# yesint/molar

Measured on AMD Instinct MI355X. Metric: frames/sec + Matom-pairs/sec, 1M-atom PBC neighbor search + RMSD fit, higher is better.
Workload: dtype f32; 1 GPU; 1M-atom synthetic triclinic box A, per frame: PBC neighbour search rc=1.2 nm (ordered pair list in HBM) + Kabsch RMSD fit/COM/gyration of a 100k-atom selection; natoms=1000000, selection_atoms=100000, frames_per_gpu=1451, parallelism=frames sharded over 1 rank(s), no data-path collective, streams_per_gpu=2, measure_overlapped_with_search=True

## Files before the change

include/molar_hip.h:

```cpp
#ifndef MOLAR_HIP_H
#define MOLAR_HIP_H

#include <stddef.h>
#include <stdint.h>

#ifdef __cplusplus
extern "C" {
#endif

enum {
    MOLAR_HIP_OK = 0,
    MOLAR_HIP_ERR_SIZES = 1,
    MOLAR_HIP_ERR_ZERO_MASS = 2,
    MOLAR_HIP_ERR_SVD = 3,
    MOLAR_HIP_ERR_NO_PBC = 4,
    MOLAR_HIP_ERR_ZERO_LENGTH_VECTOR = 5,
    MOLAR_HIP_ERR_INVERSE_FAILED = 6,
    MOLAR_HIP_ERR_LIPID_TAIL_TOO_SHORT = 7,
    MOLAR_HIP_ERR_LIPID_NORMALS_COUNT = 8,
    MOLAR_HIP_ERR_LIPID_BOND_ORDER_COUNT = 9,
    MOLAR_HIP_ERR_ANGLE_TOO_SMALL = 10,
    MOLAR_HIP_ERR_INVALID_ARGUMENT = 50,
    MOLAR_HIP_ERR_TOO_LARGE = 51,
    MOLAR_HIP_ERR_NO_SEARCH = 52,
// ... 5 lines not shown
#define MOLAR_HIP_PBC_NONE 0u


typedef struct molar_hip_ctx molar_hip_ctx;

molar_hip_ctx *molar_hip_create(int device);
void molar_hip_destroy(molar_hip_ctx *ctx);
const char *molar_hip_last_error(void);
const char *molar_hip_version(void);
int molar_hip_device_count(void);
int molar_hip_set_stream(molar_hip_ctx *ctx, void *hip_stream);
int molar_hip_synchronize(molar_hip_ctx *ctx);

#define MOLAR_HIP_PROFILE_CLASSES 8
int molar_hip_profile_enable(molar_hip_ctx *ctx, int on);
int molar_hip_profile_read(molar_hip_ctx *ctx, float ms[MOLAR_HIP_PROFILE_CLASSES],
                           uint64_t launches[MOLAR_HIP_PROFILE_CLASSES]);

int molar_hip_copy_bandwidth(molar_hip_ctx *ctx, size_t bytes, int reps, float *gb_per_s);
int molar_hip_write_bandwidth(molar_hip_ctx *ctx, size_t bytes, int reps, float *gb_per_s);


typedef struct {
    float m[9];
    float inv[9];
    int32_t nshift;
    float shifts[26 * 3];
} molar_hip_box;

int molar_hip_box_from_matrix(const float m9[9], molar_hip_box *out);
int molar_hip_box_from_vectors_angles(float a, float b, float c, float alpha, float beta, float gamma,
                                      molar_hip_box *out);
void molar_hip_box_shortest_vector(const molar_hip_box *box, const float v[3], uint8_t pbc, float out[3]);
void molar_hip_box_lab_extents(const molar_hip_box *box, float out[3]);
void molar_hip_box_extents(const molar_hip_box *box, float out[3]);
void molar_hip_box_to_box_coords(const molar_hip_box *box, const float v[3], float out[3]);
void molar_hip_box_to_lab_coords(const molar_hip_box *box, const float v[3], float out[3]);
int molar_hip_box_is_inside(const molar_hip_box *box, const float p[3]);
void molar_hip_box_wrap_point(const molar_hip_box *box, const float p[3], float out[3]);


enum {
    MOLAR_HIP_SEARCH_SINGLE = 0,
    MOLAR_HIP_SEARCH_DOUBLE = 1,
    MOLAR_HIP_SEARCH_WITHIN = 2,
    MOLAR_HIP_SEARCH_DOUBLE_VDW = 3
};

typedef struct {
    int32_t kind;
    float cutoff;
    const float *xyz1;
    size_t natoms1;
    const uint64_t *idx1;
    size_t n1;
    const float *xyz2;
    size_t natoms2;
    const uint64_t *idx2;
    size_t n2;
    const float *vdw1;
    const float *vdw2;
    int32_t ids_local;
    const float *box9;
    uint8_t pbc;
    const float *lower3;
    const float *upper3;
} molar_hip_search_desc;

int molar_hip_search_count(molar_hip_ctx *ctx, const molar_hip_search_desc *desc, uint64_t *out_count);
int molar_hip_search_fill(molar_hip_ctx *ctx, uint32_t *pairs, float *dist);
int molar_hip_search_fill_usize(molar_hip_ctx *ctx, uint64_t *i, uint64_t *j, float *dist);
int molar_hip_search_fill_ids(molar_hip_ctx *ctx, uint64_t *ids);
int molar_hip_within_count(molar_hip_ctx *ctx, const molar_hip_search_desc *desc, uint64_t *out_count);
int molar_hip_within_fill(molar_hip_ctx *ctx, uint64_t *ids);
int molar_hip_within_hold(molar_hip_ctx *ctx, int on);
int molar_hip_search_connectivity(molar_hip_ctx *ctx, const molar_hip_search_desc *desc, uint64_t *out_rows, uint64_t *out_entries);
int molar_hip_search_connectivity_fill(molar_hip_ctx *ctx, uint64_t *offsets, uint64_t *neigh);
int molar_hip_unwrap_connectivity(molar_hip_ctx *ctx, float *xyz, size_t natoms, const uint64_t *idx, size_t n,
                                  const float *box9, float cutoff, uint8_t pbc_dims, uint64_t *group_offsets,
                                  uint64_t *group_ids, size_t *ngroups);
int molar_hip_search_grid_dims(molar_hip_ctx *ctx, uint64_t dims[3]);
int molar_hip_search_cell_kernels(molar_hip_ctx *ctx, int32_t *lanes, uint64_t occupied_cells[2]);
int molar_hip_search_slot_counts(molar_hip_ctx *ctx, uint64_t *slots, uint64_t *consecutive_slots);
int molar_hip_search_fill_device(molar_hip_ctx *ctx, const uint32_t **d_pairs, const float **d_dist);
int molar_hip_search_resident(molar_hip_ctx *ctx, const molar_hip_search_desc *desc, uint64_t *out_count,
                              const uint32_t **d_pairs, const float **d_dist);
int molar_hip_search_resident_planes(molar_hip_ctx *ctx, int want_dist);
int molar_hip_search_resident_begin(molar_hip_ctx *ctx, const molar_hip_search_desc *desc, int32_t *ticket);
int molar_hip_search_resident_end(molar_hip_ctx *ctx, int32_t ticket, uint64_t *out_count, const uint32_t **d_pairs,
                                  const float **d_dist);
int molar_hip_search_histogram(molar_hip_ctx *ctx, const molar_hip_search_desc *desc, float hmin,
                               float hmax, size_t nbins, uint64_t *bins, uint64_t *out_count);
int molar_hip_search_histogram_frames(molar_hip_ctx *ctx, const molar_hip_search_desc *desc, size_t nframes, size_t xyz1_stride,
                                      size_t xyz2_stride, const float *boxes9, float hmin, float hmax, size_t nbins,
                                      uint64_t *bins);
int molar_hip_histogram_edges(float hmin, float hmax, size_t nbins, float *edges);

typedef struct {
    const uint32_t *group1;
    size_t ngroups1;
    const uint32_t *group2;
    size_t ngroups2;
} molar_hip_contact_groups;

int molar_hip_search_contacts(molar_hip_ctx *ctx, const molar_hip_search_desc *desc, const molar_hip_contact_groups *groups ,
                              uint64_t *deg1, uint64_t *deg2, uint64_t *map, uint64_t *out_count);
int molar_hip_search_contacts_frames(molar_hip_ctx *ctx, const molar_hip_search_desc *desc, const molar_hip_contact_groups *groups,
                                     size_t nframes, size_t xyz1_stride, size_t xyz2_stride, const float *boxes9,
                                     uint64_t *deg1, uint64_t *deg2, uint64_t *map, uint32_t *occupancy);

int molar_hip_search_clusters(molar_hip_ctx *ctx, const molar_hip_search_desc *desc, const molar_hip_contact_groups *groups ,
                              uint32_t *comp_of, uint32_t *sizes, uint64_t *offsets, uint32_t *members, uint32_t *out_ncomponents);
int molar_hip_search_clusters_frames(molar_hip_ctx *ctx, const molar_hip_search_desc *desc, const molar_hip_contact_groups *groups,
                                     size_t nframes, size_t xyz1_stride, const float *boxes9, uint32_t *ncomponents, uint32_t *largest,
                                     uint64_t *size_hist, uint32_t *comp_of_frames);
int molar_hip_search_clusters_counters(molar_hip_ctx *ctx, int32_t enable, uint64_t *out4);

enum {
    MOLAR_HIP_HBOND_DHA_MIN = 0,
    MOLAR_HIP_HBOND_HDA_MAX = 1
};
int molar_hip_hbonds_count(molar_hip_ctx *ctx, const molar_hip_search_desc *desc, const uint64_t *h_offsets, const uint64_t *h_idx,
                           size_t nh, int32_t angle_kind, double angle_deg, double max_ha, uint64_t *out_count);
int molar_hip_hbonds_fill(molar_hip_ctx *ctx, uint32_t *triples, double *dist_da, double *dist_ha, double *angle_deg);
int molar_hip_hbonds_counts(molar_hip_ctx *ctx, const molar_hip_search_desc *desc, const uint64_t *h_offsets, const uint64_t *h_idx,
                            size_t nh, int32_t angle_kind, double angle_deg, double max_ha, const molar_hip_contact_groups *groups,
                            uint64_t *don_count, uint64_t *acc_count, uint64_t *map, uint64_t *out_count);
int molar_hip_hbonds_frames(molar_hip_ctx *ctx, const molar_hip_search_desc *desc, const uint64_t *h_offsets, const uint64_t *h_idx,
                            size_t nh, int32_t angle_kind, double angle_deg, double max_ha, size_t nframes, size_t xyz_stride,
                            const float *boxes9, const molar_hip_contact_groups *groups, uint64_t *per_frame, uint64_t *don_count,
                            uint64_t *acc_count, uint64_t *map, uint64_t *out_total, uint64_t *out_unique);
int molar_hip_hbonds_frames_fill(molar_hip_ctx *ctx, uint64_t *frame_offsets, uint32_t *triples, double *dist_da, double *dist_ha,
                                 double *angle_deg, uint32_t *bond_of_entry, uint32_t *table, uint32_t *occupancy);

int molar_hip_lifetimes_plan(size_t nframes, size_t nrows, size_t ngroups, int want_cont, size_t *workspace_bytes,
                             uint32_t *words_per_row);
int molar_hip_lifetimes(molar_hip_ctx *ctx, const uint64_t *frame_offsets, const uint32_t *row_of_entry, size_t nframes,
                        size_t nrows, const uint32_t *group_of_row, size_t ngroups, size_t max_lag, size_t origin_stride,
                        size_t gap, uint64_t *inter, uint64_t *cont, uint64_t *run_hist, uint32_t *events, uint32_t *longest,
                        uint32_t *present);
int molar_hip_hbonds_frames_shape(molar_hip_ctx *ctx, size_t *nframes, size_t *nrows, size_t *nentries, uint64_t *serial);
int molar_hip_hbonds_frames_lifetimes(molar_hip_ctx *ctx, const uint32_t *group_of_row, size_t ngroups, size_t max_lag,
                                      size_t origin_stride, size_t gap, uint64_t *inter, uint64_t *cont, uint64_t *run_hist,
                                      uint32_t *events, uint32_t *longest, uint32_t *present);

typedef struct {
    int32_t kind;
    double cutoff;
    const double *xyz1;
    size_t natoms1;
    const uint64_t *idx1;
    size_t n1;
    const double *xyz2;
    size_t natoms2;
    const uint64_t *idx2;
    size_t n2;
    const double *vdw1;
    const double *vdw2;
    int32_t ids_local;
    const double *box9;
    uint8_t pbc;
    const double *lower3;
    const double *upper3;
} molar_hip_search_desc_f64;
int molar_hip_search_count_f64(molar_hip_ctx *ctx, const molar_hip_search_desc_f64 *desc, uint64_t *out_count);
int molar_hip_search_fill_f64(molar_hip_ctx *ctx, uint64_t *i, uint64_t *j, double *dist);
// ... 336 lines not shown
```

molar_amd/_lib.py:

```python
from __future__ import annotations

import ctypes as C
import os

HERE = os.path.dirname(os.path.abspath(__file__))
DEFAULT_LIB = os.path.join(HERE, "libmolar_hip.so")

_lib = None


class MolarHipError(RuntimeError):

    def __init__(self, code: int, msg: str):
        super().__init__(f"[molar_hip status {code}] {msg}")
        self.code = code


class Box(C.Structure):
    _fields_ = [("m", C.c_float * 9), ("inv", C.c_float * 9), ("nshift", C.c_int32), ("shifts", C.c_float * 78)]


class SearchDesc(C.Structure):
    _fields_ = [
        ("kind", C.c_int32), ("cutoff", C.c_float),
        ("xyz1", C.c_void_p), ("natoms1", C.c_size_t), ("idx1", C.c_void_p), ("n1", C.c_size_t),
        ("xyz2", C.c_void_p), ("natoms2", C.c_size_t), ("idx2", C.c_void_p), ("n2", C.c_size_t),
        ("vdw1", C.c_void_p), ("vdw2", C.c_void_p),
        ("ids_local", C.c_int32),
        ("box9", C.c_void_p), ("pbc", C.c_uint8),
        ("lower3", C.c_void_p), ("upper3", C.c_void_p),
    ]


class ContactGroups(C.Structure):
    _fields_ = [("group1", C.c_void_p), ("ngroups1", C.c_size_t), ("group2", C.c_void_p), ("ngroups2", C.c_size_t)]


class SearchDescF64(C.Structure):
    _fields_ = [
        ("kind", C.c_int32), ("cutoff", C.c_double),
        ("xyz1", C.c_void_p), ("natoms1", C.c_size_t), ("idx1", C.c_void_p), ("n1", C.c_size_t),
        ("xyz2", C.c_void_p), ("natoms2", C.c_size_t), ("idx2", C.c_void_p), ("n2", C.c_size_t),
        ("vdw1", C.c_void_p), ("vdw2", C.c_void_p),
        ("ids_local", C.c_int32),
        ("box9", C.c_void_p), ("pbc", C.c_uint8),
        ("lower3", C.c_void_p), ("upper3", C.c_void_p),
    ]


class MembraneDesc(C.Structure):
    _fields_ = [
        ("natoms", C.c_size_t), ("nlipids", C.c_size_t),
        ("lipid_idx", C.c_void_p), ("lipid_offsets", C.c_void_p), ("marker_idx", C.c_void_p), ("marker_offsets", C.c_void_p),
        ("masses", C.c_void_p), ("ntails", C.c_size_t), ("tail_idx", C.c_void_p), ("tail_offsets", C.c_void_p),
        ("tail_lipid", C.c_void_p), ("tail_bonds", C.c_void_p),
        ("cutoff", C.c_float), ("order_type", C.c_int32), ("max_smooth_iter", C.c_int32), ("unwrap", C.c_int32),
        ("use_global_normal", C.c_int32), ("global_normal", C.c_float * 3),
    ]


MEMBRANE_ARRAYS = ("head", "mid", "tail", "patch_offsets", "patch_ids", "initial_normals", "valid", "smoothed_head", "normals",
                   "quad_coefs", "mean_curv", "gauss_curv", "princ_curvs", "princ_dirs", "area", "nvert", "neib_ids",
                   "voro_vertexes", "fitted_patch_points", "order")


class MembraneView(C.Structure):
    _fields_ = ([("nlipids", C.c_size_t), ("patch_entries", C.c_size_t), ("npairs", C.c_size_t)]
                + [(k, C.c_void_p) for k in MEMBRANE_ARRAYS] + [("norder", C.c_size_t)])


class MembraneOut(C.Structure):
    _fields_ = [(k, C.c_void_p) for k in MEMBRANE_ARRAYS]


_P, _SZ, _F, _I, _U8 = C.c_void_p, C.c_size_t, C.c_float, C.c_int, C.c_uint8
SYMBOLS = {
    "molar_hip_create": (C.c_void_p, [_I]),
    "molar_hip_destroy": (None, [_P]),
    "molar_hip_last_error": (C.c_char_p, []),
    "molar_hip_version": (C.c_char_p, []),
    "molar_hip_device_count": (_I, []),
    "molar_hip_set_stream": (_I, [_P, _P]),
    "molar_hip_synchronize": (_I, [_P]),
    "molar_hip_profile_enable": (_I, [_P, _I]),
    "molar_hip_profile_read": (_I, [_P, _P, _P]),
    "molar_hip_box_from_matrix": (_I, [_P, _P]),
    "molar_hip_box_from_vectors_angles": (_I, [_F, _F, _F, _F, _F, _F, _P]),
    "molar_hip_box_shortest_vector": (None, [_P, _P, _U8, _P]),
    "molar_hip_copy_bandwidth": (_I, [_P, _SZ, _I, _P]),
    "molar_hip_write_bandwidth": (_I, [_P, _SZ, _I, _P]),
    "molar_hip_box_lab_extents": (None, [_P, _P]),
    "molar_hip_box_extents": (None, [_P, _P]),
    "molar_hip_box_to_box_coords": (None, [_P, _P, _P]),
    "molar_hip_box_to_lab_coords": (None, [_P, _P, _P]),
    "molar_hip_box_is_inside": (_I, [_P, _P]),
    "molar_hip_box_wrap_point": (None, [_P, _P, _P]),
    "molar_hip_search_count": (_I, [_P, _P, _P]),
    "molar_hip_search_fill": (_I, [_P, _P, _P]),
    "molar_hip_search_fill_usize": (_I, [_P, _P, _P, _P]),
    "molar_hip_search_fill_ids": (_I, [_P, _P]),
    "molar_hip_within_count": (_I, [_P, _P, _P]),
    "molar_hip_within_fill": (_I, [_P, _P]),
    "molar_hip_within_hold": (_I, [_P, _I]),
    "molar_hip_search_grid_dims": (_I, [_P, _P]),
    "molar_hip_search_cell_kernels": (_I, [_P, _P, _P]),
    "molar_hip_search_slot_counts": (_I, [_P, _P, _P]),
    "molar_hip_search_count_f64": (_I, [_P, _P, _P]),
    "molar_hip_search_fill_f64": (_I, [_P, _P, _P, _P]),
    "molar_hip_search_fill_ids_f64": (_I, [_P, _P]),
    "molar_hip_search_grid_dims_f64": (_I, [_P, _P]),
    "molar_hip_search_histogram_f64": (_I, [_P, _P, C.c_double, C.c_double, _SZ, _P, _P]),
    "molar_hip_search_histogram_frames_f64": (_I, [_P, _P, _SZ, _SZ, _SZ, _P, C.c_double, C.c_double, _SZ, _P]),
    "molar_hip_histogram_edges_f64": (_I, [C.c_double, C.c_double, _SZ, _P]),
    "molar_hip_within_count_f64": (_I, [_P, _P, _P]),
    "molar_hip_within_fill_f64": (_I, [_P, _P]),
    "molar_hip_search_connectivity_f64": (_I, [_P, _P, _P, _P]),
    "molar_hip_unwrap_connectivity_f64": (_I, [_P, _P, _SZ, _P, _SZ, _P, C.c_double, _U8, _P, _P, _P]),
    "molar_hip_search_resident": (_I, [_P, _P, _P, _P, _P]),
    "molar_hip_search_fill_device": (_I, [_P, _P, _P]),
    "molar_hip_search_resident_planes": (_I, [_P, _I]),
    "molar_hip_search_resident_begin": (_I, [_P, _P, _P]),
    "molar_hip_search_resident_end": (_I, [_P, C.c_int32, _P, _P, _P]),
    "molar_hip_search_histogram": (_I, [_P, _P, _F, _F, _SZ, _P, _P]),
    "molar_hip_search_histogram_frames": (_I, [_P, _P, _SZ, _SZ, _SZ, _P, _F, _F, _SZ, _P]),
    "molar_hip_histogram_edges": (_I, [_F, _F, _SZ, _P]),
    "molar_hip_search_contacts": (_I, [_P, _P, _P, _P, _P, _P, _P]),
    "molar_hip_search_contacts_frames": (_I, [_P, _P, _P, _SZ, _SZ, _SZ, _P, _P, _P, _P, _P]),
    "molar_hip_search_clusters": (_I, [_P, _P, _P, _P, _P, _P, _P, _P]),
    "molar_hip_search_clusters_frames": (_I, [_P, _P, _P, _SZ, _SZ, _P, _P, _P, _P, _P]),
    "molar_hip_search_clusters_counters": (_I, [_P, C.c_int32, _P]),
    "molar_hip_min_max": (_I, [_P, _P, _SZ, _P, _SZ, _P, _P]),
    "molar_hip_center_of_geometry": (_I, [_P, _P, _SZ, _P, _SZ, _P]),
    "molar_hip_center_of_mass": (_I, [_P, _P, _SZ, _P, _SZ, _P, _P]),
    "molar_hip_center_of_geometry_pbc": (_I, [_P, _P, _SZ, _P, _SZ, _P, _U8, _P]),
    "molar_hip_center_of_mass_pbc": (_I, [_P, _P, _SZ, _P, _SZ, _P, _P, _U8, _P]),
    "molar_hip_gyration": (_I, [_P, _P, _SZ, _P, _SZ, _P, _P, _P]),
    "molar_hip_inertia": (_I, [_P, _P, _SZ, _P, _SZ, _P, _P, _P, _P, _P]),
    "molar_hip_rmsd": (_I, [_P, _P, _SZ, _P, _SZ, _P, _SZ, _P, _SZ, _P]),
    "molar_hip_rmsd_mw": (_I, [_P, _P, _SZ, _P, _SZ, _P, _P, _SZ, _P, _SZ, _P]),
    "molar_hip_fit_transform": (_I, [_P, _P, _SZ, _P, _SZ, _P, _P, _SZ, _P, _SZ, _P, _I, _P, _P]),
    "molar_hip_xtc_histogram": (_I, [_P, _P, _SZ, _SZ, _P, _SZ, _F, _U8, _F, _F, _SZ, _P, _I]),
    "molar_hip_xtc_histogram_double": (_I, [_P, _P, _SZ, _SZ, _P, _SZ, _P, _SZ, _F, _U8, _F, _F, _SZ, _P, _I]),
    "molar_hip_fit_stream_create": (_I, [_P, _SZ, _P, _SZ, _P, _P, _SZ, _P, _I, _P]),
    "molar_hip_fit_stream_begin": (_I, [_P, _P, _I, _P]),
    "molar_hip_fit_stream_end": (_I, [_P, C.c_int32, _P, _P, _P, _P, _P]),
    "molar_hip_fit_stream_destroy": (None, [_P]),
    "molar_hip_center_of_geometry_f64": (_I, [_P, _P, _SZ, _P, _SZ, _P]),
    "molar_hip_center_of_mass_f64": (_I, [_P, _P, _SZ, _P, _SZ, _P, _P]),
    "molar_hip_gyration_f64": (_I, [_P, _P, _SZ, _P, _SZ, _P, _P]),
    "molar_hip_rmsd_f64": (_I, [_P, _P, _SZ, _P, _SZ, _P, _SZ, _P, _SZ, _P]),
    "molar_hip_rmsd_mw_f64": (_I, [_P, _P, _SZ, _P, _SZ, _P, _P, _SZ, _P, _SZ, _P]),
    "molar_hip_fit_transform_f64": (_I, [_P, _P, _SZ, _P, _SZ, _P, _P, _SZ, _P, _SZ, _P, _I, _P, _P]),
    "molar_hip_apply_transform_f64": (_I, [_P, _P, _SZ, _P, _SZ, _P, _P]),
    "molar_hip_fit_rmsd_batch_f64": (_I, [_P, _P, _SZ, _SZ, _P, _SZ, _P, _P, _SZ, _P, _I, _P, _P, _P, _P, _P]),
    "molar_hip_center_of_geometry_pbc_f64": (_I, [_P, _P, _SZ, _P, _SZ, _P, _U8, _P]),
    "molar_hip_center_of_mass_pbc_f64": (_I, [_P, _P, _SZ, _P, _SZ, _P, _P, _U8, _P]),
    "molar_hip_gyration_pbc_f64": (_I, [_P, _P, _SZ, _P, _SZ, _P, _P, _P]),
    "molar_hip_unwrap_simple_f64": (_I, [_P, _P, _SZ, _P, _SZ, _P, _U8]),
    "molar_hip_inertia_pbc_f64": (_I, [_P, _P, _SZ, _P, _SZ, _P, _P, _P, _P, _P]),
    "molar_hip_rotate_f64": (_I, [_P, _P, _SZ, _P, _SZ, _P, C.c_double]),
    "molar_hip_principal_transform_f64": (_I, [_P, _P, _SZ, _P, _SZ, _P, _P, _P, _P]),
    "molar_hip_lipid_tail_order_f64": (_I, [_P, _P, _SZ, _P, _P, _SZ, _I, _P, _P, _P, _P]),
    "molar_hip_min_max_f64": (_I, [_P, _P, _SZ, _P, _SZ, _P, _P]),
    "molar_hip_inertia_f64": (_I, [_P, _P, _SZ, _P, _SZ, _P, _P, _P, _P]),
    "molar_hip_translate_f64": (_I, [_P, _P, _SZ, _P, _SZ, _P]),
    "molar_hip_sasa_points": (_I, [C.c_uint32, _P]),
    "molar_hip_sasa_points_f64": (_I, [C.c_uint32, _P]),
    "molar_hip_sasa": (_I, [_P, _P, _SZ, _P, _SZ, _P, _F, C.c_uint32, _P, _P, _P]),
    "molar_hip_sasa_f64": (_I, [_P, _P, _SZ, _P, _SZ, _P, C.c_double, C.c_uint32, _P, _P, _P]),
    "molar_hip_sasa_frames": (_I, [_P, _P, _SZ, _SZ, _SZ, _P, _SZ, _P, _F, C.c_uint32, _P, _P]),
    "molar_hip_sasa_vol": (_I, [_P, _P, _SZ, _P, _SZ, _P, _F, C.c_uint32, _P, _P, _P, _P, _P]),
    "molar_hip_sasa_vol_f64": (_I, [_P, _P, _SZ, _P, _SZ, _P, C.c_double, C.c_uint32, _P, _P, _P, _P, _P]),
    "molar_hip_sasa_vol_frames": (_I, [_P, _P, _SZ, _SZ, _SZ, _P, _SZ, _P, _F, C.c_uint32, _P, _P, _P, _P]),
    "molar_hip_rmsd_matrix_plan": (_I, [_SZ, _SZ, _SZ, _P, _P]),
    "molar_hip_rmsd_matrix": (_I, [_P, _P, _SZ, _SZ, _P, _SZ, _SZ, _SZ, _P, _SZ, _P, _I, _P, _SZ]),
    "molar_hip_rmsd_matrix_f64": (_I, [_P, _P, _SZ, _SZ, _P, _SZ, _SZ, _SZ, _P, _SZ, _P, _I, _P, _SZ]),
    "molar_hip_fluct_plan": (_I, [_SZ, _SZ, _I, _P, _P]),
    "molar_hip_fluct": (_I, [_P, _P, _SZ, _SZ, _SZ, _P, _SZ, _P, _P, _I, _I, _P, _P, _P, _SZ, _P]),
    "molar_hip_fluct_f64": (_I, [_P, _P, _SZ, _SZ, _SZ, _P, _SZ, _P, _P, _I, _I, _P, _P, _P, _SZ, _P]),
    "molar_hip_hbonds_count": (_I, [_P, _P, _P, _P, _SZ, C.c_int32, C.c_double, C.c_double, _P]),
    "molar_hip_hbonds_fill": (_I, [_P, _P, _P, _P, _P]),
    "molar_hip_hbonds_counts": (_I, [_P, _P, _P, _P, _SZ, C.c_int32, C.c_double, C.c_double, _P, _P, _P, _P, _P]),
    "molar_hip_hbonds_frames": (_I, [_P, _P, _P, _P, _SZ, C.c_int32, C.c_double, C.c_double, _SZ, _SZ, _P, _P, _P, _P, _P, _P, _P, _P]),
    "molar_hip_hbonds_frames_fill": (_I, [_P, _P, _P, _P, _P, _P, _P, _P, _P]),
    "molar_hip_lifetimes_plan": (_I, [_SZ, _SZ, _SZ, _I, _P, _P]),
    "molar_hip_lifetimes": (_I, [_P, _P, _P, _SZ, _SZ, _P, _SZ, _SZ, _SZ, _SZ, _P, _P, _P, _P, _P, _P]),
    "molar_hip_hbonds_frames_shape": (_I, [_P, _P, _P, _P, _P]),
    "molar_hip_hbonds_frames_lifetimes": (_I, [_P, _P, _SZ, _SZ, _SZ, _SZ, _P, _P, _P, _P, _P, _P]),
    "molar_hip_msd_plan": (_I, [_SZ, _SZ, _SZ, _SZ, _SZ, _I, _I, _P, _P, _P]),
# ... 95 lines not shown
```

molar_amd/api.py:

```python
from __future__ import annotations

import collections
import ctypes as C

import numpy as np

from . import _lib
from ._lib import (MEMBRANE_ARRAYS, Box, ContactGroups, MembraneDesc, MembraneOut, MembraneView, MolarHipError, SearchDesc, SearchDescF64,
                   check)

PBC_FULL = 7
PBC_NONE = 0

SEARCH_SINGLE, SEARCH_DOUBLE, SEARCH_WITHIN, SEARCH_DOUBLE_VDW = 0, 1, 2, 3

ERR_NO_SEARCH = 52
LIFETIME_OUTPUTS = ("inter", "cont", "run_hist", "events", "longest", "present")


def _is_torch(x) -> bool:
    return type(x).__module__.startswith("torch")


def _addr(x):
# ... 172 lines not shown

    def __del__(self):
        try:
            self.close()
        except Exception:
            pass

    def _adopt(self, plan):
        import weakref
        if not hasattr(self, "_plans"):
            self._plans = []
        self._plans = [r for r in self._plans if r() is not None] + [weakref.ref(plan)]

    def synchronize(self):
        check(self.lib.molar_hip_synchronize(self.ctx))

    PROFILE_CLASSES = ("grid_build", "pair_count", "offset_scan", "pair_fill", "measure", "search_frame")

    def profile_enable(self, on=True):
        check(self.lib.molar_hip_profile_enable(self.ctx, int(on)))

    def profile_read(self):
        ms = (C.c_float * 8)(); ln = (C.c_uint64 * 8)()
        check(self.lib.molar_hip_profile_read(self.ctx, ms, ln))
        return {name: (float(ms[k]), int(ln[k])) for k, name in enumerate(self.PROFILE_CLASSES)}

    def _search_desc(self, kind, cutoff, xyz1, idx1=None, xyz2=None, idx2=None, box=None, pbc=0, vdw1=None,
                     vdw2=None, ids_local=False, lower=None, upper=None):
        xyz1 = _f32(xyz1); xyz2 = _f32(xyz2); idx1 = _sel(idx1); idx2 = _sel(idx2)
        vdw1 = _f32(vdw1); vdw2 = _f32(vdw2)
        d = SearchDesc()
        d.kind = kind
        d.cutoff = float(cutoff) if cutoff is not None else 0.0
        keep = []
        for name, arr in (("xyz1", xyz1), ("idx1", idx1), ("xyz2", xyz2), ("idx2", idx2), ("vdw1", vdw1),
                          ("vdw2", vdw2)):
            a, k = _addr(arr)
            setattr(d, name, a)
            keep.append(k)
        d.natoms1 = 0 if xyz1 is None else xyz1.shape[0] if xyz1.ndim == 2 else xyz1.shape[0] // 3
        d.natoms2 = 0 if xyz2 is None else xyz2.shape[0] if xyz2.ndim == 2 else xyz2.shape[0] // 3
        d.n1 = 0 if idx1 is None else idx1.shape[0]
        d.n2 = 0 if idx2 is None else idx2.shape[0]
        d.ids_local = 1 if ids_local else 0
        if box is not None:
            b9 = box.colmajor9() if isinstance(box, PeriodicBox) else np.ascontiguousarray(
                np.asarray(box, np.float32).reshape(3, 3).T).reshape(9)
            keep.append(b9)
            d.box9 = b9.ctypes.data
        d.pbc = pbc_mask(pbc)
        if lower is not None:
            lo = np.ascontiguousarray(lower, np.float32); up = np.ascontiguousarray(upper, np.float32)
            keep += [lo, up]
            d.lower3 = lo.ctypes.data
            d.upper3 = up.ctypes.data
        return d, keep

    def search_count(self, kind, cutoff, xyz1, idx1=None, xyz2=None, idx2=None, box=None, pbc=0, vdw1=None,
                     vdw2=None, ids_local=False, lower=None, upper=None) -> int:
        d, keep = self._search_desc(kind, cutoff, xyz1, idx1, xyz2, idx2, box, pbc, vdw1, vdw2, ids_local, lower, upper)
        cnt = C.c_uint64(0)
        check(self.lib.molar_hip_search_count(self.ctx, C.byref(d), C.byref(cnt)))
        self._keep = keep
        return int(cnt.value)

    def make_search_desc(self, kind, cutoff, xyz1, **kw):
        return self._search_desc(kind, cutoff, xyz1, **kw)

    def search_resident_desc(self, desc):
        cnt = C.c_uint64(0); p = C.c_void_p(); dd = C.c_void_p()
        check(self.lib.molar_hip_search_resident(self.ctx, C.byref(desc), C.byref(cnt), C.byref(p), C.byref(dd)))
        return int(cnt.value), p.value, dd.value

    def search_cell_kernels(self):
        lanes = C.c_int32(-1)
        occ = (C.c_uint64 * 2)()
        check(self.lib.molar_hip_search_cell_kernels(self.ctx, C.byref(lanes), occ))
        return int(lanes.value), (int(occ[0]), int(occ[1]))

    def search_slot_counts(self):
        slots, rows = C.c_uint64(0), C.c_uint64(0)
        check(self.lib.molar_hip_search_slot_counts(self.ctx, C.byref(slots), C.byref(rows)))
        return int(slots.value), int(rows.value)

    def search_resident_planes(self, want_dist=True):
        check(self.lib.molar_hip_search_resident_planes(self.ctx, 1 if want_dist else 0))

    def search_resident_begin(self, desc):
        t = C.c_int32(-1)
        check(self.lib.molar_hip_search_resident_begin(self.ctx, C.byref(desc), C.byref(t)))
        return int(t.value)

    def search_resident_end(self, ticket):
        cnt = C.c_uint64(0); p = C.c_void_p(); dd = C.c_void_p()
        check(self.lib.molar_hip_search_resident_end(self.ctx, C.c_int32(ticket), C.byref(cnt), C.byref(p), C.byref(dd)))
        return int(cnt.value), p.value, dd.value

    def search_resident(self, kind, cutoff, xyz1, idx1=None, xyz2=None, idx2=None, box=None, pbc=0, vdw1=None,
                        vdw2=None, ids_local=False, lower=None, upper=None):
        d, keep = self._search_desc(kind, cutoff, xyz1, idx1, xyz2, idx2, box, pbc, vdw1, vdw2, ids_local, lower, upper)
        cnt = C.c_uint64(0); p = C.c_void_p(); dd = C.c_void_p()
        check(self.lib.molar_hip_search_resident(self.ctx, C.byref(d), C.byref(cnt), C.byref(p), C.byref(dd)))
        self._keep = keep
        return int(cnt.value), p.value, dd.value

    def search_fill(self, count):
        pairs = np.empty((count, 2), np.uint32)
        dist = np.empty(count, np.float32)
        check(self.lib.molar_hip_search_fill(self.ctx, pairs.ctypes.data, dist.ctypes.data))
        return pairs, dist

    def search_fill_usize(self, count):
        i = np.empty(count, np.uint64); j = np.empty(count, np.uint64); d = np.empty(count, np.float32)
        check(self.lib.molar_hip_search_fill_usize(self.ctx, i.ctypes.data, j.ctypes.data, d.ctypes.data))
        return i, j, d

    def within_set(self, cutoff, xyz1, idx1=None, xyz2=None, idx2=None, box=None, pbc=0, ids_local=False, lower=None,
                   upper=None, device_out=None):
        d, keep = self._search_desc(SEARCH_WITHIN, cutoff, xyz1, idx1, xyz2, idx2, box, pbc, None, None, ids_local, lower, upper)
        cnt = C.c_uint64(0)
        check(self.lib.molar_hip_within_count(self.ctx, C.byref(d), C.byref(cnt)))
        self._keep = keep
        n = int(cnt.value)
        if device_out is not None:
            out = device_out(n)
            if n:
                check(self.lib.molar_hip_within_fill(self.ctx, out.data_ptr()))
            return out
        ids = np.empty(n, np.uint64)
        if n:
            check(self.lib.molar_hip_within_fill(self.ctx, ids.ctypes.data))
        return ids

    def search_connectivity(self, cutoff, xyz, idx=None, box=None, pbc=0, ids_local=True):
        d, keep = self._search_desc(SEARCH_SINGLE, cutoff, xyz, idx, None, None, box, pbc, None, None, ids_local, None, None)
        rows, ent = C.c_uint64(0), C.c_uint64(0)
        check(self.lib.molar_hip_search_connectivity(self.ctx, C.byref(d), C.byref(rows), C.byref(ent)))
        self._keep = keep
        off = np.empty(rows.value + 1, np.uint64)
        nb = np.empty(max(ent.value, 1), np.uint64)
        check(self.lib.molar_hip_search_connectivity_fill(self.ctx, off.ctypes.data, nb.ctypes.data))
        return off, nb[:ent.value]

    def within_hold(self, on=True):
        check(self.lib.molar_hip_within_hold(self.ctx, 1 if on else 0))

    def search_fill_ids(self, count):
        ids = np.empty(count, np.uint64)
        check(self.lib.molar_hip_search_fill_ids(self.ctx, ids.ctypes.data))
        return ids

    def search_fill_device(self):
        p = C.c_void_p(); d = C.c_void_p()
        check(self.lib.molar_hip_search_fill_device(self.ctx, C.byref(p), C.byref(d)))
        return p.value, d.value

    def search_fill_into(self, pairs_t, dist_t):
        pa, _ = _addr(pairs_t); da, _ = _addr(dist_t)
        check(self.lib.molar_hip_search_fill(self.ctx, pa, da))

    def search_f64(self, kind, cutoff, xyz1, idx1=None, xyz2=None, idx2=None, box=None, pbc=0, vdw1=None, vdw2=None,
                   ids_local=False, lower=None, upper=None, device_out=False, out=None):
        d, keep = _search_desc_f64(kind, cutoff, xyz1, idx1, xyz2, idx2, box, pbc, vdw1, vdw2, ids_local, lower, upper)
        n = C.c_uint64()
        check(self.lib.molar_hip_search_count_f64(self.ctx, C.byref(d), C.byref(n)))
        n = int(n.value)
# ... 2102 lines not shown
```

molar_amd/csrc/common.hpp:

```cpp
#pragma once

#include <hip/hip_runtime.h>

#include <cstdarg>
#include <cstddef>
#include <cstdint>
#include <cstdio>
#include <cstring>
#include <string>
#include <utility>
#include <vector>

#include "../../include/molar_hip.h"

namespace mh {


inline std::string &last_error() {
    static thread_local std::string e;
    return e;
}

inline int fail(int code, const char *fmt, ...) {
    char buf[512];
// ... 17 lines not shown
    do {                      \
        int _rc = (expr);     \
        if (_rc) return _rc;  \
    } while (0)

#define MH_CTX(c)                                                                    \
    do {                                                                             \
        if (!(c)) return ::mh::fail(MOLAR_HIP_ERR_INVALID_ARGUMENT, "null context"); \
        MH_HIP(hipSetDevice((c)->device));                                           \
    } while (0)


struct DevBuf {
    void *p = nullptr;
    size_t cap = 0;
    DevBuf() = default;
    DevBuf(const DevBuf &) = delete;
    DevBuf &operator=(const DevBuf &) = delete;
    DevBuf(DevBuf &&o) noexcept : p(std::exchange(o.p, nullptr)), cap(std::exchange(o.cap, 0)) {}
    DevBuf &operator=(DevBuf &&o) noexcept {
        if (this != &o) {
            release();
            p = std::exchange(o.p, nullptr);
            cap = std::exchange(o.cap, 0);
        }
        return *this;
    }
    ~DevBuf() { release(); }
    int reserve(size_t bytes) {
        if (bytes <= cap) return 0;
        if (p) {
            MH_HIP(hipFree(p));
            p = nullptr;
            cap = 0;
        }
        size_t want = bytes + bytes / 8 + 256;
        MH_HIP(hipMalloc(&p, want));
        cap = want;
        return 0;
    }
    void release() {
        if (p) (void)hipFree(p);
        p = nullptr;
        cap = 0;
    }
    template <class T>
    T *as() const { return reinterpret_cast<T *>(p); }
};

inline bool is_device_ptr(const void *p) {
    if (!p) return false;
    hipPointerAttribute_t a;
    hipError_t e = hipPointerGetAttributes(&a, p);
    if (e != hipSuccess) {
        (void)hipGetLastError();
        return false;
    }
    return a.type == hipMemoryTypeDevice || a.type == hipMemoryTypeManaged || a.type == hipMemoryTypeArray;
}


struct GridSet {
    uint32_t n = 0;
    DevBuf xyz_stage;
    DevBuf idx_stage;
    DevBuf vdw_stage;
    const float *d_xyz = nullptr;
    const uint64_t *d_idx = nullptr;
    const float *d_vdw = nullptr;
    DevBuf key;
    DevBuf cell_count;
    DevBuf cnt_pad;
    DevBuf cursor;
    DevBuf tmp_key;
    DevBuf sort_buf;
    DevBuf sorted;
    DevBuf sorted_vdw;
    DevBuf aabb;
    DevBuf perm;
    DevBuf chunk_aabb;
    DevBuf h16;
    DevBuf cell_org;
    DevBuf live;
};

struct SearchShape {
    int kind = 0;
    bool use_box = false;
    uint8_t pbc = 0;
    float cutoff = 0.f;
    molar_hip_box box{};
    float lower[3]{}, upper[3]{};
    uint32_t dims[3]{1, 1, 1};
    uint64_t ntasks = 0;
    uint64_t nslots_bound = 0;
    GridSet *set = nullptr;
    uint32_t occ_use[2] = {0, 0};
};

struct HeldGrid {
    bool valid = false;
    const GridSet *set = nullptr;
    uint64_t fp = 0;
    const float *xyz = nullptr;
    const uint64_t *idx = nullptr;
    size_t natoms = 0, n = 0;
    int ids_local = 0;
    bool use_box = false;
    uint8_t pbc = 0;
    molar_hip_box box{};
    uint32_t dims[3]{0, 0, 0};
    float lower[3]{}, upper[3]{};
};

struct SearchSizes {
    unsigned long long total;
    unsigned long long mask_units;
    unsigned long long slots;
    unsigned long long occupied;
};
static_assert(sizeof(SearchSizes) == 32 && offsetof(SearchSizes, total) == 0 && offsetof(SearchSizes, mask_units) == 8 &&
                  offsetof(SearchSizes, slots) == 16 && offsetof(SearchSizes, occupied) == 24,
              "SearchSizes: total, mask_units, slots, occupied, 64 bits each, in this order");

}

struct molar_hip_search64_state;
struct molar_hip_sasa_state;
struct molar_hip_rmsd_matrix_state;
struct molar_hip_fluct_state;
struct molar_hip_msd_state;
struct molar_hip_hbonds_state;
struct molar_hip_lifetimes_state;
struct molar_hip_within_state;
struct molar_hip_connectivity_state;
struct molar_hip_contacts_state;

#ifndef MH_HIST_BATCH
#define MH_HIST_BATCH 16
#endif

struct molar_hip_ctx {
    int device = 0;
    hipStream_t stream = nullptr;
    bool own_stream = false;
    int num_cus = 256;

    void *h_pinned = nullptr;
    size_t h_pinned_cap = 0;
    molar_hip_search64_state *s64 = nullptr;
    molar_hip_sasa_state *sasa = nullptr;
    molar_hip_rmsd_matrix_state *rmsdm = nullptr;
    molar_hip_fluct_state *fluct = nullptr;
    molar_hip_msd_state *msd = nullptr;
    molar_hip_hbonds_state *hbonds = nullptr;
    molar_hip_lifetimes_state *lifetimes = nullptr;
    molar_hip_within_state *within = nullptr;
    molar_hip_connectivity_state *conn = nullptr;
    molar_hip_contacts_state *contacts = nullptr;
    void *ring[8] = {nullptr, nullptr, nullptr, nullptr, nullptr, nullptr, nullptr, nullptr};
    hipEvent_t ring_ev[8] = {nullptr, nullptr, nullptr, nullptr, nullptr, nullptr, nullptr, nullptr};

    bool have_search = false;
    mh::SearchShape cur;
    uint64_t total = 0;
    mh::GridSet set_store[2][2];
// ... 212 lines not shown
```

molar_amd/csrc/pair_kernels.hpp:

```cpp
#pragma once

#include "boxmath.hpp"
#include "common.hpp"

namespace mh {
namespace pairk {

enum { MODE_COUNT = 0, MODE_FILL = 1, MODE_HIST = 2 };

#ifndef MH_COUNT_WPE
#define MH_COUNT_WPE 6
#endif
#ifndef MH_FILL_WPE
#define MH_FILL_WPE 8
#endif
#ifndef MH_WPB
#define MH_WPB 1
#endif
constexpr int waves_per_block(int mode) { return mode == MODE_HIST ? 4 : MH_WPB; }
constexpr int KREG = 8;
constexpr int FIFO_CAP = 128;
constexpr int LIVE_GROUPS = KREG;
constexpr uint32_t SLOT_LIVE = 0x400u;
#ifndef MOLAR_HIP_NO_WIDE_FLUSH
// ... 22 lines not shown
__device__ __forceinline__ uint32_t gload_u32(const uint32_t *p, size_t i) {
    return ((const __attribute__((address_space(1))) uint32_t *)p)[i];
}
__device__ __forceinline__ void gstore_u32(uint32_t *p, size_t i, uint32_t v) {
    ((__attribute__((address_space(1))) uint32_t *)p)[i] = v;
}
__device__ __forceinline__ float uniform_f32(float v) { return __uint_as_float(__builtin_amdgcn_readfirstlane(__float_as_uint(v))); }
__device__ __forceinline__ float4 lload4(const float4 *p, uint32_t i) {
    const v4f_t v = ((const __attribute__((address_space(3))) v4f_t *)p)[i];
    return make_float4(v.x, v.y, v.z, v.w);
}

struct SearchParams {
    const float4 *sa;
    const float4 *sb;
    const uint32_t *csa;
    const uint32_t *csb;
    const float *vdwa;
    const float *vdwb;
    const float4 *aabb_b;
    const float4 *perm_b;
    const float4 *chunk_aabb_b;
    const uint4 *h16_b;
    const float4 *cell_org_b;
    uint32_t mfma_count;
    const struct TaskDesc *task_desc;
    uint32_t *maskbuf;
    const unsigned long long *task_moff;
    unsigned long long mask_cap_units;
    unsigned long long out_cap;
    uint32_t dx, dy, dz;
    uint32_t pbc;
    uint32_t use_box;
    uint32_t nblocks;
    uint32_t wrap_kind;
    uint32_t prune_wrapped;
    float prune_limit2;
    uint32_t approx_wrapped;
    float band_lo, band_hi;
    uint32_t hist_nbins;
    float hist_min, hist_max;
    unsigned long long *hist_bins;
    unsigned long long *hist_total;
    const float *hist_edges;
    float hist_scale;
    uint32_t hist_lean;
    const uint32_t *hist_nslots;
#ifdef MOLAR_HIP_DEBUG_KNOBS
    uint32_t debug_skip;
    unsigned long long *dbg;
#endif
    float cutoff2;
    uint64_t ntasks;
    molar_hip_box box;
    alignas(16) float shifts4[96];
    uint32_t hist_big;
};

struct TaskDesc {
    uint32_t a0, n1, b0, n2, cb, flags, pad0, pad1;
};

struct SlotDesc {
    uint32_t a0, n1, b0, n2;
    uint32_t cb, flags, i0, frame;
    unsigned long long moff, pad1;
};
static_assert(sizeof(SlotDesc) == 48, "SlotDesc is read with three 16-byte loads");

struct Task {
    uint32_t a0, n1, b0, n2;
    uint32_t rps;
    uint32_t cb;
    uint32_t ca;
    uint32_t wrap_b;
    uint32_t wrap;
    bool tri;
    bool valid;
};

struct SlotTask : Task {
    bool live = false;
    uint32_t lrow = 0;
};

__device__ __forceinline__ uint32_t slot_row(const SlotTask &T, uint32_t i0, uint32_t lane) { return T.live ? T.lrow : i0 + lane; }

template <int KIND, bool UNIFORM>
__device__ __forceinline__ Task decode_task(const SearchParams &P, uint64_t t) {
    Task T;
    T.valid = false;
    T.tri = false;
    T.a0 = T.b0 = T.n1 = T.n2 = 0;
    T.cb = 0;
    T.ca = 0;
    T.wrap_b = 0;
    T.rps = 64u;
    T.wrap = 0;
    uint32_t half = 0;
    uint64_t e = t;
    if (KIND != MOLAR_HIP_SEARCH_SINGLE) {
        half = (uint32_t)(t & 1ull);
        e = t >> 1;
    }
    const uint32_t m = (uint32_t)(e % 14ull);
    const uint64_t cidx = e / 14ull;
    const uint32_t z = (uint32_t)(cidx % P.dz);
    const uint64_t r = cidx / P.dz;
    const uint32_t y = (uint32_t)(r % P.dy);
    const uint32_t x = (uint32_t)(r / P.dy);
    const uint32_t dims[3] = {P.dx, P.dy, P.dz};
    uint32_t c[2][3] = {{x + MASKS[m][0], y + MASKS[m][1], z + MASKS[m][2]},
                        {x + MASKS[m][3], y + MASKS[m][4], z + MASKS[m][5]}};
    uint32_t wrap = 0, wrap_c2 = 0;
    for (int i = 0; i < 2; ++i)
        for (int d = 0; d < 3; ++d)
            if (c[i][d] == dims[d]) {
                if ((P.pbc >> d) & 1u) {
                    c[i][d] = 0;
                    wrap |= 1u << d;
                    if (i == 1) wrap_c2 |= 1u << d;
                } else {
                    return T;
                }
            }
    const uint32_t i1 = c[0][0] + c[0][1] * P.dx + c[0][2] * P.dx * P.dy;
    const uint32_t i2 = c[1][0] + c[1][1] * P.dx + c[1][2] * P.dx * P.dy;
    uint32_t ca = i1, cb = i2;
    if (KIND == MOLAR_HIP_SEARCH_SINGLE) {
        T.tri = (i1 == i2);
    } else if (half) {
        ca = i2;
        cb = i1;
    }
    T.a0 = P.csa[ca];
    T.n1 = P.csa[ca + 1] - T.a0;
    T.b0 = P.csb[cb];
    T.n2 = P.csb[cb + 1] - T.b0;
    T.wrap = wrap;
    T.wrap_b = (KIND != MOLAR_HIP_SEARCH_SINGLE && half) ? (wrap & ~wrap_c2) : wrap_c2;
    T.rps = (P.use_box && wrap == MOLAR_HIP_PBC_FULL && P.box.nshift != 0 && T.n1 <= 4096u) ? (T.n1 <= 1024u ? 2u : 8u) : 64u;
    T.cb = cb;
    T.ca = ca;
    if (UNIFORM) {
        T.cb = __builtin_amdgcn_readfirstlane(T.cb);
        T.rps = __builtin_amdgcn_readfirstlane(T.rps);
        T.a0 = __builtin_amdgcn_readfirstlane(T.a0);
        T.n1 = __builtin_amdgcn_readfirstlane(T.n1);
        T.b0 = __builtin_amdgcn_readfirstlane(T.b0);
        T.n2 = __builtin_amdgcn_readfirstlane(T.n2);
        T.wrap = __builtin_amdgcn_readfirstlane(T.wrap);
    }
    T.valid = T.n1 > 0 && T.n2 > 0 && !(T.tri && T.n1 < 2);
    return T;
}

typedef float v2f __attribute__((ext_vector_type(2)));

enum { WK_NONE = 0, WK_DIAG = 1, WK_UPPER = 2, WK_GENERAL = 3 };

__device__ __forceinline__ v2f round_away2(v2f f) { return v2f{__builtin_roundf(f.x), __builtin_roundf(f.y)}; }

struct BoxRegs {
    float I[9], M[9];
    int nshift;
};
// ... 420 lines not shown
    }
    const uint32_t ubase = (T.b0 >> 6) + T.cb;
    unsigned long long livek[NCH];
#pragma unroll
    for (int k = 0; k < NCH; ++k) {
        const float4 lo = gload4(P.chunk_aabb_b, 2u * (ubase + k)), hi = gload4(P.chunk_aabb_b, 2u * (ubase + k) + 1u);
        const bool need = lane < rows && !(aabb_d2(a.x, a.y, a.z, lo.x, lo.y, lo.z, hi.x, hi.y, hi.z) > cutoff2);
        livek[k] = __builtin_amdgcn_ballot_w64(need);
    }
    __builtin_amdgcn_wave_barrier();
    uint32_t acc = 0;
    unsigned long long live = 0ull;
#pragma unroll
    for (int k = 0; k < NCH; ++k) live |= livek[k];
    while (live) {
        const uint32_t r = (uint32_t)__builtin_ctzll(live);
        live &= ~(1ull << r);
        const float4 p = lload4(la, r);
#pragma unroll
        for (int k = 0; k < NCH; ++k) {
            if (!((livek[k] >> r) & 1ull)) continue;
            const float dx = bx[k] - p.x, dy = by[k] - p.y, dz = bz[k] - p.z;
            float d2 = (dx * dx + dy * dy) + dz * dz;
            if (TRI) d2 = (bpos[k] > i0 + r) ? d2 : INFINITY;
            asm volatile("v_cmp_ge_f32 vcc, %2, %1\n\tv_addc_co_u32 %0, vcc, 0, %0, vcc" : "+v"(acc) : "v"(d2), "s"(cutoff2) : "vcc");
        }
    }
    for (int off = 32; off > 0; off >>= 1) acc += __shfl_xor(acc, off, 64);
    return acc;
}

typedef _Float16 v8h_t __attribute__((ext_vector_type(8)));
typedef float v16f_t __attribute__((ext_vector_type(16)));

__device__ __forceinline__ uint32_t pack_h2(_Float16 a, _Float16 b) {
    return (uint32_t)__builtin_bit_cast(unsigned short, a) | ((uint32_t)__builtin_bit_cast(unsigned short, b) << 16);
}

constexpr int MFMA_TILES = 10;

__device__ __forceinline__ float mfma_error_bound(float R, float c) {
    return 2.3841858e-07f * ((16.0f * R * R + 8.0f * c) + (4.0f * R + 1.0f));
}
__device__ __forceinline__ bool mfma_bound_usable(float R, float E, float c) {
    return R < 64.0f && E < 0.02f * c && (c + R * R) < 3.0e4f;
}

template <int KIND, bool TRI>
__device__ __forceinline__ uint32_t run_count_mfma(const SearchParams &P, const SlotTask &T, uint32_t i0, float4 *la, uint4 *lh,
                                                   uint32_t lane, bool &done) {
    typedef uint32_t u4_t __attribute__((ext_vector_type(4)));
    typedef __attribute__((address_space(3))) u4_t lds_u4;
    typedef __attribute__((address_space(3))) uint32_t lds_u32;
    typedef __attribute__((address_space(1))) u4_t glb_u4;
    const float cutoff2 = P.cutoff2;
    const uint32_t rows = __builtin_amdgcn_readfirstlane(T.n1 - i0 < T.rps ? T.n1 - i0 : T.rps);
    const uint32_t kh = lane >> 5, cl = lane & 31u;
    const uint32_t nct = (T.n2 + 31u) >> 5;
    float4 a = make_float4(0.f, 0.f, 0.f, 0.f);
    if (lane < rows) a = gload4(P.sa, T.a0 + slot_row(T, i0, lane));
    const float4 org = gload4(P.cell_org_b, T.cb);
    bool need = lane < rows;
    if (!TRI && !T.live) {
        const float4 blo = gload4(P.aabb_b, 2 * T.cb), bhi = gload4(P.aabb_b, 2 * T.cb + 1);
        need = need && !(aabb_d2(a.x, a.y, a.z, blo.x, blo.y, blo.z, bhi.x, bhi.y, bhi.z) > cutoff2);
    }
    const unsigned long long live = __builtin_amdgcn_ballot_w64(need);
    const uint32_t nlive = TRI ? rows : (uint32_t)__popcll(live);
    if (!TRI && nlive == 0u) return 0u;
    const uint32_t rank = TRI ? lane : __builtin_amdgcn_mbcnt_hi((uint32_t)(live >> 32), __builtin_amdgcn_mbcnt_lo((uint32_t)live, 0u));
    u4_t bq[MFMA_TILES];
#pragma unroll
    for (int t = 0; t < MFMA_TILES; ++t) {
        const uint32_t col = (uint32_t)t * 32u + cl;
        if (32u * (uint32_t)(t + 1) <= T.n2) {
            bq[t] = ((const glb_u4 *)P.h16_b)[T.b0 + col];
        } else {
            bq[t] = u4_t{0u, 0u, 0u, 0x00007BFFu};
            if (col < T.n2) bq[t] = ((const glb_u4 *)P.h16_b)[T.b0 + col];
        }
    }
    if (TRI || need) la[rank] = a;
    const float r0 = a.x - org.x, r1 = a.y - org.y, r2 = a.z - org.z;
    float ra2 = need ? (r0 * r0 + r1 * r1) + r2 * r2 : 0.0f;
    const bool fin = ra2 == ra2;
    for (int off = 32; off > 0; off >>= 1) ra2 = fmaxf(ra2, __shfl_xor(ra2, off, 64));
    const float R = 1.0001f * __builtin_sqrtf(ra2) + org.w;
    const float E = uniform_f32(mfma_error_bound(R, cutoff2));
    if (__builtin_amdgcn_ballot_w64(!fin) != 0ull || !mfma_bound_usable(R, E, cutoff2)) {
        done = false;
        return 0u;
    }
    {
        u4_t k0 = {0u, 0u, 0u, 0x00007BFFu}, k1 = {0u, 0u, 0u, 0x3C003C00u};
        if (!TRI) {
            ((lds_u4 *)lh)[2u * lane] = k0;
            ((lds_u4 *)lh)[2u * lane + 1u] = k1;
            __builtin_amdgcn_wave_barrier();
        }
        if (need) {
            const _Float16 h0 = (_Float16)r0, h1 = (_Float16)r1, h2 = (_Float16)r2;
            const _Float16 l0 = (_Float16)(r0 - (float)h0), l1 = (_Float16)(r1 - (float)h1), l2 = (_Float16)(r2 - (float)h2);
            const float e0 = (float)h0 + (float)l0, e1 = (float)h1 + (float)l1, e2 = (float)h2 + (float)l2;
            const float na = ((e0 * e0 + e1 * e1) + e2 * e2) - cutoff2;
            const _Float16 nh = (_Float16)na, nl = (_Float16)(na - (float)nh);
            const _Float16 m2 = (_Float16)-2.0f;
            const _Float16 g0 = m2 * h0, g1 = m2 * h1, g2 = m2 * h2, s0 = m2 * l0, s1 = m2 * l1, s2 = m2 * l2;
            k0 = u4_t{pack_h2(g0, g1), pack_h2(g2, g0), pack_h2(g1, g2), pack_h2(nh, nl)};
            k1 = u4_t{pack_h2(s0, s1), pack_h2(s2, s0), pack_h2(s1, s2), 0x3C003C00u};
        }
        if (TRI || need) {
            ((lds_u4 *)lh)[2u * rank] = k0;
            ((lds_u4 *)lh)[2u * rank + 1u] = k1;
        }
    }
    __builtin_amdgcn_wave_barrier();
    const u4_t a0q = ((const lds_u4 *)lh)[2u * cl + kh], a1q = ((const lds_u4 *)lh)[2u * (32u + cl) + kh];
    const v8h_t A0 = __builtin_bit_cast(v8h_t, a0q), A1 = __builtin_bit_cast(v8h_t, a1q);
    __builtin_amdgcn_wave_barrier();
    lds_u32 *todo = (lds_u32 *)lh;
    uint32_t ntodo = 0;
    uint32_t cnt = 0;
#pragma unroll
    for (int t = 0; t < MFMA_TILES; ++t) {
        if ((uint32_t)t < nct) {
            u4_t bt = bq[t];
            if (kh == 0u) bt.w = 0x3C003C00u;
            const v8h_t B = __builtin_bit_cast(v8h_t, bt);
#pragma unroll
            for (int rt = 0; rt < 2; ++rt) {
                bool diag = false;
                if (32u * (uint32_t)rt >= nlive) continue;
                if (TRI) {
                    const uint32_t row0 = i0 + 32u * (uint32_t)rt;
                    if (32u * (uint32_t)t + 31u <= row0) continue;
                    diag = 32u * (uint32_t)t <= row0 + 31u;
                }
                v16f_t acc = {0.f, 0.f, 0.f, 0.f, 0.f, 0.f, 0.f, 0.f, 0.f, 0.f, 0.f, 0.f, 0.f, 0.f, 0.f, 0.f};
                acc = __builtin_amdgcn_mfma_f32_32x32x16_f16(rt == 0 ? A0 : A1, B, acc, 0, 0, 0);
                if (TRI && diag) {
                    const int tv = (int)(32u * (uint32_t)t + cl) - (int)(i0 + 32u * (uint32_t)rt + 4u * kh);
#pragma unroll
                    for (int i = 0; i < 16; ++i) acc[i] = (tv > 8 * (i / 4) + (i % 4)) ? acc[i] : 1.0e30f;
                }
                uint32_t h = 0u;
                float m = INFINITY;
#pragma unroll
                for (int i = 0; i < 16; ++i) {
                    h = __builtin_amdgcn_alignbit(h, __float_as_uint(acc[i]), 31);
                    m = __builtin_fminf(m, __builtin_fabsf(acc[i]));
                }
                if (__builtin_amdgcn_ballot_w64(m < E) == 0ull) {
                    cnt += (uint32_t)__popc(h);
                } else {
                    if (lane == 0) todo[ntodo] = (uint32_t)(2 * t + rt);
                    ++ntodo;
                }
            }
        }
    }
    if (ntodo) {
        __builtin_amdgcn_wave_barrier();
        for (uint32_t q = 0; q < ntodo; ++q) {
            const uint32_t id = __builtin_amdgcn_readfirstlane(todo[q]);
            const uint32_t ct = id >> 1, rt = id & 1u;
            const uint32_t col = ct * 32u + cl;
            float4 b = make_float4(3.0e38f, 3.0e38f, 3.0e38f, 0.f);
            if (col < T.n2) b = gload4(P.sb, T.b0 + col);
            for (uint32_t r = 0; r < 16u; ++r) {
// ... 589 lines not shown

template <int KIND>
__device__ __forceinline__ bool hist_lean_slot(const SearchParams &P, uint32_t flags, uint32_t n2) {
    if (KIND != MOLAR_HIP_SEARCH_SINGLE && KIND != MOLAR_HIP_SEARCH_DOUBLE) return false;
    if (((n2 + 63u) >> 6) > (uint32_t)KREG && !P.hist_big) return false;
    const uint32_t wrap = flags & 7u;
    if (!(P.use_box && wrap != 0u)) return true;
    if (flags & 0x100u) return false;
    return P.approx_wrapped != 0u && !(P.box.nshift != 0 && wrap == MOLAR_HIP_PBC_FULL);
}

template <int KIND, int MODE, int WPE = 0, bool LIVE = false>
__global__ void __launch_bounds__(64 * waves_per_block(MODE))
__attribute__((amdgpu_waves_per_eu(WPE ? WPE : (MODE == MODE_HIST ? 4 : (MODE == MODE_COUNT ? MH_COUNT_WPE : MH_FILL_WPE))))) pair_kernel(const SearchParams *__restrict__ Pp,
                                                     const SlotDesc *__restrict__ slot_desc,
                                                     const uint32_t nslots_arg,
                                                     uint32_t *__restrict__ slot_cnt,
                                                     const unsigned long long *__restrict__ slot_base,
                                                     uint2 *__restrict__ out_pairs, float *__restrict__ out_dist,
                                                     uint32_t *__restrict__ out_ids) {
    constexpr int WAVES_PER_BLOCK = waves_per_block(MODE), BLOCK = 64 * WAVES_PER_BLOCK;
    constexpr int PLANE = MODE != MODE_COUNT ? FIFO_WIDE : FIFO_CAP;
    static_assert(FIFO_CAP * 16 <= 2 * FIFO_WIDE * 4, "the replay queue fits in two planes");
    __shared__ __attribute__((aligned(16))) uint32_t lds[WAVES_PER_BLOCK][3][PLANE];
    __shared__ float4 lds_a[WAVES_PER_BLOCK][64];
    __shared__ uint4 lds_h[MODE == MODE_COUNT ? WAVES_PER_BLOCK : 1][MODE == MODE_COUNT ? 128 : 1];
    constexpr bool FILL = MODE != MODE_COUNT;
    static_assert(!LIVE || (WPE == 0 && MODE != MODE_HIST && (KIND == MOLAR_HIP_SEARCH_SINGLE || KIND == MOLAR_HIP_SEARCH_DOUBLE)),
                  "live-ranked slots: regular count / fill instances of the fixed-cutoff kinds");
    constexpr bool LIVE_SLOTS = LIVE;
    extern __shared__ uint32_t lds_hist[];
    const SearchParams &P0 = *Pp;
#ifdef MH_SLOT_LOOP
    uint32_t lane_var = threadIdx.x & 63u;
    const uint32_t &lane = lane_var;
#else
    const uint32_t lane = threadIdx.x & 63u;
#endif
    uint32_t nslots = nslots_arg;
    if (MODE == MODE_HIST && P0.hist_nslots) {
        const uint32_t real = __builtin_amdgcn_readfirstlane(P0.hist_nslots[0]);
        nslots = real < nslots_arg ? real : nslots_arg;
    }
    const uint32_t wave = WAVES_PER_BLOCK == 1 ? 0u : __builtin_amdgcn_readfirstlane(threadIdx.x >> 6);
    constexpr bool hist = MODE == MODE_HIST;
    if (hist) {
        for (uint32_t b = threadIdx.x; b < P0.hist_nbins; b += BLOCK) lds_hist[b] = 0u;
        __syncthreads();
    }
    unsigned long long wave_total = 0;
    auto process_slot = [&](uint32_t w) __attribute__((always_inline)) {
        uint32_t wr = w;
        {
            const uint32_t x = w & 7u, q = w >> 3;
            const uint32_t full = (nslots / (8u * XCD_RUN)) * (8u * XCD_RUN);
            if (w < full) wr = ((q / XCD_RUN) * 8u + x) * XCD_RUN + (q % XCD_RUN);
        }
        const uint32_t slot = nslots - 1u - wr;
        SlotTask T;
        uint32_t i0;
        unsigned long long moff;
        uint32_t frame = 0u;
        {
            const uint4 lo = reinterpret_cast<const uint4 *>(slot_desc + slot)[0];
            const uint4 hi = reinterpret_cast<const uint4 *>(slot_desc + slot)[1];
            const uint2 mo = reinterpret_cast<const uint2 *>(slot_desc + slot)[4];
            const uint32_t fl = __builtin_amdgcn_readfirstlane(hi.y);
            if (!(fl & 0x200u)) return;
            if (MODE == MODE_HIST) frame = __builtin_amdgcn_readfirstlane(hi.w);
            T.a0 = __builtin_amdgcn_readfirstlane(lo.x);
            T.n1 = __builtin_amdgcn_readfirstlane(lo.y);
            T.b0 = __builtin_amdgcn_readfirstlane(lo.z);
            T.n2 = __builtin_amdgcn_readfirstlane(lo.w);
            T.cb = __builtin_amdgcn_readfirstlane(hi.x);
            i0 = __builtin_amdgcn_readfirstlane(hi.z);
            moff = ((unsigned long long)__builtin_amdgcn_readfirstlane(mo.y) << 32) | __builtin_amdgcn_readfirstlane(mo.x);
            T.wrap = fl & 7u;
            T.tri = (fl & 0x100u) != 0u;
            T.valid = true;
            T.wrap_b = (fl >> 12) & 7u;
            T.rps = fl >> 16;
            if constexpr (LIVE_SLOTS) {
                if (fl & SLOT_LIVE) {
                    typedef __attribute__((address_space(1))) unsigned long long glb_u64;
                    const uint2 mp = reinterpret_cast<const uint2 *>(slot_desc + slot)[5];
                    const glb_u64 *mk = (const glb_u64 *)(((unsigned long long)(uint32_t)__builtin_amdgcn_readfirstlane(mp.y) << 32) |
                                                          (unsigned long long)(uint32_t)__builtin_amdgcn_readfirstlane(mp.x));
                    unsigned long long mw = 0ull;
                    if (lane < (uint32_t)LIVE_GROUPS) mw = mk[lane];
                    uint32_t *scr = lds[wave][0];
                    uint32_t before = 0u;
#pragma unroll
                    for (int g = 0; g < LIVE_GROUPS; ++g) {
                        const uint32_t wlo = __builtin_amdgcn_readlane((uint32_t)mw, g), whi = __builtin_amdgcn_readlane((uint32_t)(mw >> 32), g);
                        const uint32_t n = (uint32_t)__popc(wlo) + (uint32_t)__popc(whi);
                        if (n != 0u && before + n > i0 && before < i0 + 64u) {
                            const uint32_t rank = before + __builtin_amdgcn_mbcnt_hi(whi, __builtin_amdgcn_mbcnt_lo(wlo, 0u)) - i0;
                            const bool bit = (((lane < 32u ? wlo : whi) >> (lane & 31u)) & 1u) != 0u;
                            if (bit && rank < 64u) scr[rank] = 64u * (uint32_t)g + lane;
                        }
                        before += n;
                    }
                    __builtin_amdgcn_wave_barrier();
                    T.lrow = scr[lane];
                    __builtin_amdgcn_wave_barrier();
                    T.live = true;
                    T.n1 = before;
                }
            }
        }
        const SearchParams &P = MODE == MODE_HIST ? Pp[frame] : P0;
        Fifo F;
        F.fi = lds[wave][0];
        F.fj = lds[wave][1];
        F.fd = lds[wave][2];
        F.head = F.tail = 0;
        F.quota = 64u;
        F.has_pairs = out_pairs != nullptr;
        F.has_dist = out_dist != nullptr;
        F.pairs = nullptr;
        F.dist = nullptr;
        F.ids = nullptr;
        F.base = 0;
        F.room = 0xFFFFFFFFu;
        F.hist = hist ? lds_hist : nullptr;
        F.recompute = 0u;
        F.la = lds_a[wave];
        F.fq = nullptr;
        F.fq_store = MODE == MODE_FILL ? reinterpret_cast<float4 *>(lds[wave][0]) : nullptr;
        F.lh = MODE == MODE_COUNT ? lds_h[wave] : nullptr;
        F.wrap = 0;
        F.hmin = P.hist_min;
        F.hmax = P.hist_max;
        F.hn = (float)P.hist_nbins;
        if (FILL && !hist) {
            F.base = slot_base[slot];
            F.quota = 64u - ((uint32_t)F.base & 63u);
            const unsigned long long end = slot_base[slot + 1];
            if (end == F.base || end > P.out_cap) return;
            F.room = end - F.base < 0xFFFFFFFFull ? (uint32_t)(end - F.base) : 0xFFFFFFFFu;
            if (out_pairs) F.pairs = out_pairs + F.base + lane;
            if (out_dist) F.dist = out_dist + F.base + lane;
            if (out_ids) F.ids = out_ids + F.base + lane;
        }
        uint32_t total = 0;
        const uint32_t wk = (P.use_box && T.wrap != 0) ? P.wrap_kind : (uint32_t)WK_NONE;
        if (hist && P.hist_lean && !P.hist_nslots && hist_lean_slot<KIND>(P, (T.tri ? 0x100u : 0u) | T.wrap, T.n2)) return;
#ifdef MOLAR_HIP_DEBUG_KNOBS
        if (P.debug_skip) {
            const uint32_t kind_bit = T.tri ? 4u : (wk != WK_NONE ? (T.rps == 8u ? 8u : 2u) : 1u);
            if (P.debug_skip & kind_bit) return;
        }
#endif
        constexpr bool MASKED = MODE != MODE_HIST;
        uint32_t *mwords = nullptr;
        if (MASKED) {
            const uint32_t nch = (T.n2 + 63u) >> 6;
            if (moff + 2u * nch <= P.mask_cap_units) mwords = P.maskbuf + moff * 64u;
        }
        constexpr int KMAX = (WPE == 2 || WPE == 3) ? KMAX_HUGE : (WPE ? KMAX_WIDE : KREG);
        switch (wk) {
            case WK_NONE: total = run_task_nch<KIND, FILL, WK_NONE, MASKED, KMAX>(P, T, i0, F, lds_a[wave], lane, mwords); break;
            case WK_DIAG: total = run_task_nch<KIND, FILL, WK_DIAG, MASKED, KMAX>(P, T, i0, F, lds_a[wave], lane, mwords); break;
            case WK_UPPER: total = run_task_nch<KIND, FILL, WK_UPPER, MASKED, KMAX>(P, T, i0, F, lds_a[wave], lane, mwords); break;
            default: total = run_task_nch<KIND, FILL, WK_GENERAL, MASKED, KMAX>(P, T, i0, F, lds_a[wave], lane, mwords); break;
        }
        if (!FILL && lane == 0) slot_cnt[slot] = total;
        wave_total += total;
    };
    const uint32_t w0 = (blockIdx.y * gridDim.x + blockIdx.x) * WAVES_PER_BLOCK + wave;
    if (!hist) {
#ifdef MH_SLOT_LOOP
#pragma unroll 1
        for (uint32_t g = 0; g < (uint32_t)MH_SLOT_LOOP; ++g) {
            const uint32_t w = w0 + g * (gridDim.x * gridDim.y * WAVES_PER_BLOCK);
            if (w < nslots) process_slot(w);
            asm volatile("" : "+v"(lane_var));
        }
#else
        if (w0 < nslots) process_slot(w0);
#endif
    } else {
        for (uint32_t w = w0; w < nslots; w += gridDim.x * gridDim.y * WAVES_PER_BLOCK) process_slot(w);
    }
    if (hist) {
        __syncthreads();
        for (uint32_t b = threadIdx.x; b < P0.hist_nbins; b += BLOCK) {
            const uint32_t v = lds_hist[b];
            if (v) atomicAdd(&P0.hist_bins[b], (unsigned long long)v);
        }
// ... 59 lines not shown
```

molar_amd/csrc/search.hip:

```cpp
#include <cstdlib>

#include "boxmath.hpp"
#include "common.hpp"
#include "csr_kernels.hpp"
#include "hoststream.hpp"
#include <algorithm>

#include "pair_kernels.hpp"
#include "search_core.hpp"
#include "search_shape.hpp"
#include "stages.hpp"

namespace mh {
void launch_pair_small(int mode, int lanes_per_slot, hipStream_t stream, const pairk::SearchParams *dP, const pairk::SlotDesc *slot_desc,
                       uint32_t nslots, uint32_t *slot_cnt, const unsigned long long *slot_base, uint2 *pairs, float *dist);
}
using namespace mh;
using namespace mh::pairk;

namespace {

constexpr uint32_t DROPPED = 0xFFFFFFFFu;


// ... 478 lines not shown
    for (int q = 0; q < SCAN_ITEMS; ++q) {
        if (base + q < n) out[base + q] = run;
        run += item[q];
    }
    if (threadIdx.x == 0) block_sums[blockIdx.x] = tot;
}

constexpr unsigned long long LB_MASK = (1ull << 62) - 1ull;
constexpr uint32_t PLAN_GROUP = 128;
__device__ __forceinline__ unsigned long long lb_resolve(unsigned long long *desc, uint32_t tile, unsigned long long tot) {
    if (tile == 0) {
        __hip_atomic_store(&desc[0], (2ull << 62) | tot, __ATOMIC_RELEASE, __HIP_MEMORY_SCOPE_AGENT);
        return 0ull;
    }
    __hip_atomic_store(&desc[tile], (1ull << 62) | tot, __ATOMIC_RELEASE, __HIP_MEMORY_SCOPE_AGENT);
    unsigned long long run = 0;
    for (uint32_t t = tile - 1u;; --t) {
        unsigned long long d;
        do {
            d = __hip_atomic_load(&desc[t], __ATOMIC_ACQUIRE, __HIP_MEMORY_SCOPE_AGENT);
        } while ((d >> 62) == 0ull);
        run += d & LB_MASK;
        if ((d >> 62) == 2ull) break;
    }
    __hip_atomic_store(&desc[tile], (2ull << 62) | (run + tot), __ATOMIC_RELEASE, __HIP_MEMORY_SCOPE_AGENT);
    return run;
}

template <class TIn1, class TOut1, class TIn2, class TOut2>
__global__ void __launch_bounds__(256) scan_lookback_kernel(const TIn1 *in1, TOut1 *out1, const TIn2 *in2, TOut2 *out2, uint64_t n,
                                                            unsigned long long *state, uint32_t ntiles) {
    __shared__ uint32_t tile_s;
    __shared__ unsigned long long pre_s[2];
    if (threadIdx.x == 0) tile_s = atomicAdd(reinterpret_cast<uint32_t *>(state), 1u);
    __syncthreads();
    const uint32_t tile = tile_s;
    unsigned long long *d1 = state + 1, *d2 = state + 1 + ntiles;
    const uint64_t base = (uint64_t)tile * (blockDim.x * SCAN_ITEMS) + (uint64_t)threadIdx.x * SCAN_ITEMS;
    TOut1 a[SCAN_ITEMS];
    TOut2 b[SCAN_ITEMS];
    TOut1 sa = 0;
    TOut2 sb = 0;
    for (int q = 0; q < SCAN_ITEMS; ++q) {
        a[q] = base + q < n ? (TOut1)in1[base + q] : (TOut1)0;
        sa += a[q];
        b[q] = (in2 && base + q < n) ? (TOut2)in2[base + q] : (TOut2)0;
        sb += b[q];
    }
    TOut1 ta;
    TOut1 ra = block_exclusive_scan<TOut1>(sa, &ta);
    TOut2 tb = 0, rb = 0;
    if (in2) rb = block_exclusive_scan<TOut2>(sb, &tb);
    if (threadIdx.x == 0) pre_s[0] = lb_resolve(d1, tile, (unsigned long long)ta);
    if (threadIdx.x == (blockDim.x > 64u ? 64u : 1u) && in2) pre_s[1] = lb_resolve(d2, tile, (unsigned long long)tb);
    __syncthreads();
    ra += (TOut1)pre_s[0];
    if (in2) rb += (TOut2)pre_s[1];
    for (int q = 0; q < SCAN_ITEMS; ++q) {
        if (base + q < n) {
            out1[base + q] = ra;
            if (in2) out2[base + q] = rb;
        }
        ra += a[q];
        rb += b[q];
    }
}

inline size_t lookback_state_words(uint64_t n) { return 1 + 2 * (size_t)((n + 64 * SCAN_ITEMS - 1) / (64 * SCAN_ITEMS)); }

template <class TIn1, class TOut1, class TIn2, class TOut2>
int scan_lookback(molar_hip_ctx *c, const TIn1 *in1, TOut1 *out1, const TIn2 *in2, TOut2 *out2, uint64_t n,
                  unsigned long long *zeroed_state) {
    if (n == 0) return 0;
    const uint32_t block = 256u;
    const uint32_t ntiles = (uint32_t)((n + block * SCAN_ITEMS - 1) / (block * SCAN_ITEMS));
    hipLaunchKernelGGL((scan_lookback_kernel<TIn1, TOut1, TIn2, TOut2>), dim3(ntiles), dim3(block), 0, c->stream, in1, out1, in2, out2, n,
                       zeroed_state, ntiles);
    MH_HIP(hipGetLastError());
    return 0;
}

constexpr uint32_t LIVE_NONE = 0xFFFFFFFFu;
static_assert(LIVE_ROW_GROUPS == (uint32_t)LIVE_GROUPS, "the host sizes the masks the kernels index");
template <int KIND>
__global__ void __launch_bounds__(64) live_rows_kernel(SearchParams P, unsigned long long *__restrict__ masks, uint32_t *__restrict__ live_cnt) {
    const uint64_t t = (uint64_t)blockIdx.y * gridDim.x + blockIdx.x;
    if (t >= P.ntasks) return;
    const uint32_t lane = threadIdx.x;
    const Task T = decode_task<KIND, true>(P, t);
    const bool wrapped = P.use_box && T.wrap != 0u;
    const bool approx = wrapped && P.approx_wrapped != 0u && !(P.box.nshift != 0 && T.wrap == MOLAR_HIP_PBC_FULL);
    if (!T.valid || T.tri || T.rps != 64u || T.n1 > 64u * (uint32_t)LIVE_GROUPS || T.n2 > 64u * (uint32_t)KREG || (wrapped && !approx)) {
        if (lane == 0) live_cnt[t] = LIVE_NONE;
        return;
    }
    float Sx = 0.f, Sy = 0.f, Sz = 0.f;
    float limit2 = P.cutoff2;
    if (approx) {
#pragma unroll
        for (int d = 0; d < 3; ++d) {
            if (!((T.wrap >> d) & 1u)) continue;
            const float sgn = ((T.wrap_b >> d) & 1u) ? 1.0f : -1.0f;
            Sx += sgn * P.box.m[3 * d];
            Sy += sgn * P.box.m[3 * d + 1];
            Sz += sgn * P.box.m[3 * d + 2];
        }
        limit2 = P.prune_limit2;
    }
    const float4 lo = gload4(P.aabb_b, 2 * T.cb), hi = gload4(P.aabb_b, 2 * T.cb + 1);
    unsigned long long mine = 0ull;
    uint32_t nlive = 0u;
#pragma unroll
    for (int g = 0; g < LIVE_GROUPS; ++g) {
        const uint32_t row = 64u * (uint32_t)g + lane;
        if (64u * (uint32_t)g >= T.n1) break;
        bool need = false;
        if (row < T.n1) {
            const float4 a = gload4(P.sa, T.a0 + row);
            need = !(aabb_d2(a.x - Sx, a.y - Sy, a.z - Sz, lo.x, lo.y, lo.z, hi.x, hi.y, hi.z) > limit2);
        }
        const unsigned long long m = __builtin_amdgcn_ballot_w64(need);
        if (lane == (uint32_t)g) mine = m;
        nlive += (uint32_t)__popcll(m);
    }
    if (lane < (uint32_t)LIVE_GROUPS) masks[t * (uint64_t)LIVE_GROUPS + lane] = mine;
    if (lane == 0) live_cnt[t] = nlive;
}

template <int KIND>
__global__ void __launch_bounds__(256) plan_tiles_kernel(SearchParams P, uint32_t *__restrict__ local_first, TaskDesc *__restrict__ task_desc,
                                                         unsigned long long *__restrict__ local_moff, uint32_t fast_kind,
                                                         uint32_t *__restrict__ slot_cnt, uint64_t nslot_cnt,
                                                         unsigned long long *__restrict__ tile_tot, SearchParams *__restrict__ params_dst,
                                                         const uint32_t *__restrict__ live_cnt) {
    const uint64_t t = (uint64_t)blockIdx.x * 256u + threadIdx.x;
    for (uint64_t w = t; w < nslot_cnt; w += (uint64_t)gridDim.x * 256u) slot_cnt[w] = 0u;
    if (params_dst && blockIdx.x == 0) {
        const uint32_t *src = (const uint32_t *)__builtin_amdgcn_kernarg_segment_ptr();
        uint32_t *d = (uint32_t *)params_dst;
        for (uint32_t w = threadIdx.x; w < (uint32_t)(sizeof(SearchParams) / 4u); w += 256u) d[w] = src[w];
    }
    uint32_t nb = 0, nb_rows = 0;
    unsigned long long mu = 0;
    if (t < P.ntasks) {
        const Task T = decode_task<KIND, false>(P, t);
        nb = nb_rows = T.valid ? (T.n1 + T.rps - 1u) / T.rps : 0u;
        const uint32_t lc = (live_cnt && T.valid) ? live_cnt[t] : LIVE_NONE;
        if (lc != LIVE_NONE) nb = (lc + 63u) >> 6;
        const uint32_t nch = (T.n2 + 63u) >> 6;
        mu = (fast_kind && P.use_box && T.wrap != 0u && nch <= (uint32_t)KREG) ? (unsigned long long)nb * 2u * nch : 0ull;
        TaskDesc d;
        d.a0 = T.a0; d.n1 = T.n1; d.b0 = T.b0; d.n2 = T.n2; d.cb = T.cb;
        d.flags = T.wrap | (T.tri ? 0x100u : 0u) | (T.valid ? 0x200u : 0u) | (lc != LIVE_NONE ? SLOT_LIVE : 0u) | (T.wrap_b << 12) | (T.rps << 16);
        d.pad0 = nb;
        d.pad1 = 0u;
        task_desc[t] = d;
    }
    uint32_t tot_nb, tot_rows;
    const uint32_t first = block_exclusive_scan<uint32_t>(nb, &tot_nb);
    (void)block_exclusive_scan<uint32_t>(nb_rows, &tot_rows);
    unsigned long long tot_mu = 0ull, m0 = 0ull;
    if (fast_kind) m0 = block_exclusive_scan<unsigned long long>(mu, &tot_mu);
    if (t <= P.ntasks) {
        local_first[t] = first;
        if (fast_kind) local_moff[t] = m0;
    }
    if (threadIdx.x == 0) {
        tile_tot[2 * blockIdx.x] = (unsigned long long)tot_nb | ((unsigned long long)tot_rows << 32);
        tile_tot[2 * blockIdx.x + 1] = tot_mu;
    }
}

static __global__ void __launch_bounds__(64) plan_groups_kernel(uint32_t ntiles, const unsigned long long *__restrict__ tile_tot,
                                                                unsigned long long *__restrict__ group_tot) {
    unsigned long long n = 0, m = 0;
    for (uint32_t k = threadIdx.x; k < PLAN_GROUP; k += 64u) {
        const uint32_t b = blockIdx.x * PLAN_GROUP + k;
        if (b < ntiles) { n += tile_tot[2 * b]; m += tile_tot[2 * b + 1]; }
    }
    for (int off = 32; off > 0; off >>= 1) {
        n += __shfl_xor(n, off, 64);
        m += __shfl_xor(m, off, 64);
    }
    if (threadIdx.x == 0) { group_tot[2 * blockIdx.x] = n; group_tot[2 * blockIdx.x + 1] = m; }
}

constexpr uint32_t PLAN_SUB = 64;
static __global__ void __launch_bounds__(256) plan_slots_kernel(uint64_t ntasks, uint32_t ntiles, const uint32_t *__restrict__ local_first,
                                                                const unsigned long long *__restrict__ local_moff,
                                                                uint32_t *__restrict__ task_first, const TaskDesc *__restrict__ task_desc,
                                                                unsigned long long *__restrict__ task_moff,
                                                                const unsigned long long *__restrict__ tile_tot,
                                                                SlotDesc *__restrict__ slot_desc, uint64_t nslots_bound,
                                                                SearchSizes *__restrict__ sizes_host,
                                                                const unsigned long long *__restrict__ group_tot,
                                                                const unsigned long long *__restrict__ live_masks,
                                                                unsigned long long *__restrict__ slot_stat) {
    __shared__ unsigned long long part[3][4];
    const uint32_t tile = blockIdx.x / (256u / PLAN_SUB), sub = blockIdx.x % (256u / PLAN_SUB);
    unsigned long long pn = 0, pm = 0, all_n = 0;
    if (!group_tot) {
        for (uint32_t b = threadIdx.x; b < ntiles; b += 256u) {
            const unsigned long long n = tile_tot[2 * b];
            all_n += n;
            if (b < tile) {
                pn += n;
                pm += tile_tot[2 * b + 1];
            }
        }
    } else {
        const uint32_t ngroups = (ntiles + PLAN_GROUP - 1u) / PLAN_GROUP, g = tile / PLAN_GROUP;
        for (uint32_t b = threadIdx.x; b < ngroups; b += 256u) {
            const unsigned long long n = group_tot[2 * b];
            all_n += n;
            if (b < g) {
                pn += n;
                pm += group_tot[2 * b + 1];
            }
        }
        for (uint32_t b = g * PLAN_GROUP + threadIdx.x; b < tile; b += 256u) {
            pn += tile_tot[2 * b];
            pm += tile_tot[2 * b + 1];
        }
    }
    for (int off = 32; off > 0; off >>= 1) {
        pn += __shfl_xor(pn, off, 64);
        pm += __shfl_xor(pm, off, 64);
        all_n += __shfl_xor(all_n, off, 64);
    }
    if ((threadIdx.x & 63u) == 0u) { part[0][threadIdx.x >> 6] = pn; part[1][threadIdx.x >> 6] = pm; part[2][threadIdx.x >> 6] = all_n; }
    __syncthreads();
    const uint32_t base_n = (uint32_t)((part[0][0] + part[0][1]) + (part[0][2] + part[0][3]));
    const unsigned long long base_m = (part[1][0] + part[1][1]) + (part[1][2] + part[1][3]);
    const unsigned long long total2 = (part[2][0] + part[2][1]) + (part[2][2] + part[2][3]);
    const unsigned long long total = total2 & 0xFFFFFFFFull;
    __shared__ uint32_t lfirst[PLAN_SUB + 1];
    __shared__ TaskDesc ldesc[PLAN_SUB];
    __shared__ unsigned long long lm0[PLAN_SUB];
    const uint32_t tile_n = (uint32_t)tile_tot[2 * tile];
    if (threadIdx.x <= PLAN_SUB) {
        const uint64_t t = (uint64_t)tile * 256u + sub * PLAN_SUB + threadIdx.x;
        const bool inside = threadIdx.x < PLAN_SUB || sub + 1u < 256u / PLAN_SUB;
        uint32_t local = tile_n;
        unsigned long long m0 = ~0ull >> 1;
        TaskDesc d;
        d.a0 = d.n1 = d.b0 = d.n2 = d.cb = d.flags = d.pad0 = d.pad1 = 0u;
        if (inside && t <= ntasks) {
            local = local_first[t];
            if (threadIdx.x < PLAN_SUB) {
                if (task_moff) m0 = base_m + local_moff[t];
                if (t < ntasks) d = task_desc[t];
            }
        }
        lfirst[threadIdx.x] = local;
        if (threadIdx.x < PLAN_SUB) {
            ldesc[threadIdx.x] = d;
            lm0[threadIdx.x] = m0;
        }
    }
    __syncthreads();
    if (threadIdx.x < PLAN_SUB) {
        const uint64_t t = (uint64_t)tile * 256u + sub * PLAN_SUB + threadIdx.x;
        if (t <= ntasks) {
            task_first[t] = base_n + lfirst[threadIdx.x];
            if (task_moff) task_moff[t] = lm0[threadIdx.x];
            if (t == ntasks && sizes_host) {
                sizes_host->mask_units = task_moff ? lm0[threadIdx.x] : 0ull;
                sizes_host->slots = base_n + lfirst[threadIdx.x];
            }
            if (t == ntasks && slot_stat) {
                slot_stat[0] = total;
                slot_stat[1] = total2 >> 32;
            }
        }
    }
    const uint32_t s0 = lfirst[0], s1 = lfirst[PLAN_SUB];
    uint4 *out = reinterpret_cast<uint4 *>(slot_desc) + 3 * ((size_t)base_n + s0);
    for (uint32_t i = threadIdx.x; i < 3u * (s1 - s0); i += 256u) {
        const uint32_t sl = s0 + i / 3u, part3 = i % 3u;
        uint32_t lo = 0u, hi = PLAN_SUB;
        while (hi - lo > 1u) {
            const uint32_t mid = (lo + hi) >> 1;
            if (lfirst[mid] <= sl) lo = mid;
            else hi = mid;
        }
        const TaskDesc d = ldesc[lo];
        const uint32_t q = sl - lfirst[lo], rps = d.flags >> 16, nch = (d.n2 + 63u) >> 6;
        uint4 w;
        if (part3 == 0u) w = make_uint4(d.a0, d.n1, d.b0, d.n2);
        else if (part3 == 1u) w = make_uint4(d.cb, d.flags, q * rps, 0u);
        else {
            const unsigned long long mo = task_moff ? lm0[lo] + (unsigned long long)q * 2u * nch : lm0[lo];
            const unsigned long long mp = (d.flags & SLOT_LIVE) ? (unsigned long long)(live_masks + (((uint64_t)tile * 256u + sub * PLAN_SUB + lo) * (uint64_t)LIVE_GROUPS)) : 0ull;
            w = make_uint4((uint32_t)mo, (uint32_t)(mo >> 32), (uint32_t)mp, (uint32_t)(mp >> 32));
        }
        out[i] = w;
    }
    if (total <= nslots_bound) {
        uint4 *blank = reinterpret_cast<uint4 *>(slot_desc) + 3 * (size_t)total;
        const uint64_t nw = 3ull * (nslots_bound + 1ull - total);
        for (uint64_t i = (uint64_t)blockIdx.x * 256u + threadIdx.x; i < nw; i += (uint64_t)gridDim.x * 256u)
            blank[i] = (i % 3ull == 2ull) ? make_uint4(0xFFFFFFFFu, 0x7FFFFFFFu, 0u, 0u) : make_uint4(0u, 0u, 0u, 0u);
    }
}

template <class T>
__global__ void __launch_bounds__(256) scan_sums_kernel(T *sums, uint64_t nb) {
    __shared__ T carry_s;
    if (threadIdx.x == 0) carry_s = 0;
    __syncthreads();
    for (uint64_t start = 0; start < nb; start += 256) {
        const uint64_t i = start + threadIdx.x;
        const T v = i < nb ? sums[i] : (T)0;
        T tot;
        const T ex = block_exclusive_scan<T>(v, &tot);
        const T carry = carry_s;
        if (i < nb) sums[i] = carry + ex;
        __syncthreads();
        if (threadIdx.x == 0) carry_s = carry + tot;
        __syncthreads();
    }
}

template <class T>
__global__ void __launch_bounds__(256) scan_add_kernel(T *out, const T *sums, uint64_t n) {
    const uint64_t base = (uint64_t)blockIdx.x * SCAN_TILE + (uint64_t)threadIdx.x * SCAN_ITEMS;
    const T add = sums[blockIdx.x];
    for (int q = 0; q < SCAN_ITEMS; ++q)
        if (base + q < n) out[base + q] += add;
}

template <class TIn, class TOut>
__global__ void __launch_bounds__(256) scan_small_kernel(const TIn *in, TOut *out, uint32_t n) {
    __shared__ TOut carry_s;
    if (threadIdx.x == 0) carry_s = 0;
    __syncthreads();
    for (uint32_t start = 0; start < n; start += 1024u) {
        const uint32_t base = start + threadIdx.x * 4u;
        TOut item[4], sum = 0;
        for (int q = 0; q < 4; ++q) {
            item[q] = base + q < n ? (TOut)in[base + q] : (TOut)0;
            sum += item[q];
        }
        TOut tot;
        TOut run = carry_s + block_exclusive_scan<TOut>(sum, &tot);
        for (int q = 0; q < 4; ++q) {
            if (base + q < n) out[base + q] = run;
            run += item[q];
        }
        __syncthreads();
        if (threadIdx.x == 0) carry_s += tot;
        __syncthreads();
    }
}

template <class TIn, class TOut>
__global__ void __launch_bounds__(64) scan_small_wave_kernel(const TIn *in, TOut *out, uint32_t n) {
    TOut carry = 0;
    for (uint32_t start = 0; start < n; start += 512u) {
        const uint32_t base = start + threadIdx.x * 8u;
        TOut item[8], sum = 0;
        for (int q = 0; q < 8; ++q) {
            item[q] = base + q < n ? (TOut)in[base + q] : (TOut)0;
            sum += item[q];
        }
        TOut inc = sum;
        for (int off = 1; off < 64; off <<= 1) {
            const TOut o = __shfl_up(inc, off, 64);
            if ((int)threadIdx.x >= off) inc += o;
        }
        TOut run = carry + inc - sum;
        for (int q = 0; q < 8; ++q) {
            if (base + q < n) out[base + q] = run;
            run += item[q];
        }
        carry += __shfl(inc, 63, 64);
// ... 639 lines not shown
    float cutoff = q->cutoff;
    if (vdw) {
        if (cur.set[0].n == 0 || cur.set[1].n == 0) {
            cur.dims[0] = cur.dims[1] = cur.dims[2] = 1;
            cur.ntasks = 0;
            c->total = 0;
            *degenerate = true;
            return 0;
        }
        float m1, m2;
        MH_TRY(device_fmax2(c, cur.set[0].d_vdw, cur.set[0].n, cur.set[1].d_vdw, cur.set[1].n, &m1, &m2));
        cutoff = (m1 + m2) + F32_EPS;
    }
    if (!(cutoff > 0.0f)) return fail(MOLAR_HIP_ERR_INVALID_ARGUMENT, "search: cutoff must be positive (got %g)", (double)cutoff);
    cur.cutoff = cutoff;

    float ext[3];
    if (cur.use_box) {
        molar_hip_box_lab_extents(&cur.box, ext);
    } else {
        if (q->kind == MOLAR_HIP_SEARCH_WITHIN) {
            if (!q->lower3 || !q->upper3)
                return fail(MOLAR_HIP_ERR_INVALID_ARGUMENT, "non-periodic within search needs lower3/upper3");
            for (int d = 0; d < 3; ++d) {
                cur.lower[d] = q->lower3[d];
                cur.upper[d] = q->upper3[d];
            }
        } else {
            MH_TRY(c->hist.reserve(64));
            uint32_t *d_mm = c->hist.as<uint32_t>();
            uint32_t seed[6];
            for (int d = 0; d < 6; ++d) seed[d] = f2ord_host(0.0f);
            MH_HIP(hipMemcpyAsync(d_mm, seed, sizeof seed, hipMemcpyHostToDevice, c->stream));
            MH_TRY(bbox_accumulate(c, d_mm, cur.set[0]));
            if (two) MH_TRY(bbox_accumulate(c, d_mm, cur.set[1]));
            uint32_t mm[6];
            MH_TRY(read_back(c, mm, d_mm, sizeof mm));
            for (int d = 0; d < 3; ++d) {
                cur.lower[d] = ord2f(mm[d]) + (-cutoff - F32_EPS);
                cur.upper[d] = ord2f(mm[3 + d]) + (cutoff + F32_EPS);
            }
        }
        for (int d = 0; d < 3; ++d) ext[d] = cur.upper[d] - cur.lower[d];
    }
    MH_TRY(dims_from_extents(cur, ext));
    if (*reuse0 && !held_same_cells(c->held, cur)) {
        *reuse0 = false;
        c->held.valid = false;
        MH_TRY(stage_set(c, cur.set[0], q->xyz1, q->natoms1, q->idx1, q->n1, q->vdw1, vdw));
    }
    *to_hold = (may_hold && !*reuse0) ? held_remember(*q, cur, fp) : HeldGrid{};
    occ_latch(c);
    cur.ntasks = plan_entries(cur);
    cur.nslots_bound = slots_bound(cur, call.hist_plan);
    if (cur.ntasks >= 0xFFFFFFF0ull || cur.nslots_bound >= 0xFFFFFFF0ull || cur.ntasks + cur.nslots_bound >= 0xFFFFFF00ull)
        return fail(MOLAR_HIP_ERR_TOO_LARGE, "search plan too large (%llu entries)", (unsigned long long)cur.ntasks);
    return 0;
}

int reserve_plan(molar_hip_ctx *c, const SearchCall &call) {
    const SearchShape &cur = c->cur;
    MH_TRY(c->task_nb.reserve((cur.ntasks + 1) * 4));
    MH_TRY(c->task_desc.reserve((cur.ntasks + 1) * sizeof(TaskDesc)));
    MH_TRY(c->slot_desc.reserve((cur.nslots_bound + 1) * sizeof(SlotDesc)));
    if (call.hist_plan) MH_TRY(c->slot_desc_rest.reserve((cur.nslots_bound + 1) * sizeof(SlotDesc)));
    MH_TRY(c->slot_cnt.reserve((cur.nslots_bound + 1) * 4));
    MH_TRY(c->slot_base.reserve((cur.nslots_bound + 1) * 8));
    MH_TRY(c->params.reserve(sizeof(SearchParams)));
    MH_TRY(c->scan_state.reserve((lookback_state_words(cur.ntasks + 1) + lookback_state_words(cur.nslots_bound + 1)) * 8));
    MH_TRY(c->task_mu.reserve((cur.ntasks + 1) * 4));
    MH_TRY(c->task_moff.reserve((cur.ntasks + 1) * 8));
    MH_TRY(c->slot_stat.reserve(16));
    return 0;
}

bool plans_live_rows(const SearchCall &call, const SearchShape &cur) { return call.plan && call.live_rows && !call.hist_plan && live_row_slots(cur); }

int enqueue_live_rows(molar_hip_ctx *c, const SearchCall &call, const GridLane &lane) {
    const SearchShape &cur = c->cur;
    if (!plans_live_rows(call, cur)) return 0;
    MH_TRY(cur.set[0].live.reserve(live_rows_bytes(cur)));
    unsigned long long *masks = cur.set[0].live.as<unsigned long long>();
    uint32_t *cnt = reinterpret_cast<uint32_t *>(masks + live_rows_mask_words(cur));
    const SearchParams P = make_params(c, cur);
    const dim3 grid = pair_grid((unsigned)cur.ntasks);
    if (cur.kind == MOLAR_HIP_SEARCH_SINGLE) hipLaunchKernelGGL((live_rows_kernel<MOLAR_HIP_SEARCH_SINGLE>), grid, dim3(64), 0, lane.stream, P, masks, cnt);
    else hipLaunchKernelGGL((live_rows_kernel<MOLAR_HIP_SEARCH_DOUBLE>), grid, dim3(64), 0, lane.stream, P, masks, cnt);
    MH_HIP(hipGetLastError());
    return 0;
}

int build_grids(molar_hip_ctx *c, const SearchCall &call, const GridLane &lane, bool build0, int ids_local) {
    SearchShape &cur = c->cur;
    if (build0) MH_TRY(build_grid(c, call, lane, cur.set[0], ids_local));
    if (cur.kind != MOLAR_HIP_SEARCH_SINGLE) MH_TRY(build_grid(c, call, lane, cur.set[1], ids_local));
    return enqueue_live_rows(c, call, lane);
}

int enqueue_plan(molar_hip_ctx *c, const SearchCall &call) {
    Prof prof(c, 0);
    const SearchShape &cur = c->cur;
    const uint32_t fast_kind = records_hit_history(cur) ? 1u : 0u;
    const bool use_live = plans_live_rows(call, cur);
    SearchParams P = make_params(c, cur);
    SearchParams *params_dst = nullptr;
    c->params_fresh = false;
    if (!call.size_masks) {
        P.out_cap = call.out_cap;
        params_dst = c->params.as<SearchParams>();
        c->params_fresh = true;
        c->params_fresh_cap = P.out_cap;
    }
    if (cur.ntasks + 1 <= FPLAN_MAX_TASKS) {
        const uint32_t ntiles = (uint32_t)((cur.ntasks + 1 + 255) / 256);
        const uint32_t ngroups = ntiles > 1024u ? (ntiles + PLAN_GROUP - 1u) / PLAN_GROUP : 0u;
        MH_TRY(c->fplan_tiles.reserve((size_t)ntiles * 16 + (cur.ntasks + 1) * 8 + (size_t)ngroups * 16));
        unsigned long long *moff = fast_kind ? c->task_moff.as<unsigned long long>() : nullptr;
        unsigned long long *tt = c->fplan_tiles.as<unsigned long long>();
        unsigned long long *lmoff = tt + 2 * (size_t)ntiles;
        uint32_t *lfirst = c->task_mu.as<uint32_t>();
        const unsigned long long *live_masks = use_live ? cur.set[0].live.as<unsigned long long>() : nullptr;
        const uint32_t *live_cnt = use_live ? reinterpret_cast<const uint32_t *>(live_masks + live_rows_mask_words(cur)) : nullptr;
        if (cur.kind == MOLAR_HIP_SEARCH_SINGLE)
            hipLaunchKernelGGL((plan_tiles_kernel<MOLAR_HIP_SEARCH_SINGLE>), dim3(ntiles), dim3(256), 0, c->stream, P, lfirst,
                               c->task_desc.as<TaskDesc>(), lmoff, fast_kind, c->slot_cnt.as<uint32_t>(), cur.nslots_bound + 1, tt, params_dst, live_cnt);
        else
            hipLaunchKernelGGL((plan_tiles_kernel<MOLAR_HIP_SEARCH_DOUBLE>), dim3(ntiles), dim3(256), 0, c->stream, P, lfirst,
                               c->task_desc.as<TaskDesc>(), lmoff, fast_kind, c->slot_cnt.as<uint32_t>(), cur.nslots_bound + 1, tt, params_dst, live_cnt);
        unsigned long long *gt = ngroups ? lmoff + (cur.ntasks + 1) : nullptr;
        if (ngroups) hipLaunchKernelGGL(plan_groups_kernel, dim3(ngroups), dim3(64), 0, c->stream, ntiles, tt, gt);
        hipLaunchKernelGGL(plan_slots_kernel, dim3(ntiles * (256u / PLAN_SUB)), dim3(256), 0, c->stream, cur.ntasks, ntiles, lfirst, lmoff, c->task_nb.as<uint32_t>(),
                           c->task_desc.as<TaskDesc>(), moff, tt, c->slot_desc.as<SlotDesc>(), cur.nslots_bound, call.sizes_dev, gt,
                           live_masks, c->slot_stat.as<unsigned long long>());
        MH_HIP(hipGetLastError());
        c->slot_stat_valid = true;
        c->plan_live = use_live;
        return 0;
    }
    const uint64_t nstate = lookback_state_words(cur.ntasks + 1) + lookback_state_words(cur.nslots_bound + 1);
    const uint64_t nplan = std::max<uint64_t>(std::max<uint64_t>(cur.ntasks + 1, cur.nslots_bound + 1), nstate);
    const unsigned pbs = 256u;
    const unsigned nb = (unsigned)((nplan + pbs - 1) / pbs);
    switch (cur.kind) {
        case MOLAR_HIP_SEARCH_SINGLE:
            hipLaunchKernelGGL((plan_kernel<MOLAR_HIP_SEARCH_SINGLE>), dim3(nb), dim3(pbs), 0, c->stream, P, c->task_nb.as<uint32_t>(), c->task_desc.as<TaskDesc>(),
                               c->task_mu.as<uint32_t>(), fast_kind, c->slot_cnt.as<uint32_t>(), cur.nslots_bound + 1,
                               c->scan_state.as<unsigned long long>(), nstate, params_dst);
            break;
        default:
            hipLaunchKernelGGL((plan_kernel<MOLAR_HIP_SEARCH_DOUBLE>), dim3(nb), dim3(pbs), 0, c->stream, P, c->task_nb.as<uint32_t>(), c->task_desc.as<TaskDesc>(),
                               c->task_mu.as<uint32_t>(), fast_kind, c->slot_cnt.as<uint32_t>(), cur.nslots_bound + 1,
                               c->scan_state.as<unsigned long long>(), nstate, params_dst);
            break;
    }
    MH_HIP(hipGetLastError());
    return enqueue_plan_slots(c, call.sizes_dev);
}

bool takes_side_lane(const molar_hip_ctx *c, const molar_hip_search_desc *q, const SearchCall &call) {
    const SearchShape &cur = c->cur;
    const bool two = q->kind != MOLAR_HIP_SEARCH_SINGLE;
    return call.side && c->own_stream && cur.use_box && q->kind != MOLAR_HIP_SEARCH_DOUBLE_VDW && cur.set[0].d_xyz == q->xyz1 &&
           cur.set[0].d_idx == q->idx1 && (!two || (cur.set[1].d_xyz == q->xyz2 && cur.set[1].d_idx == q->idx2));
}

}

int mh::prepare_search(molar_hip_ctx *c, const molar_hip_search_desc *q, const SearchCall &call, bool *degenerate) {
    *degenerate = false;
    if (!c || !q) return fail(MOLAR_HIP_ERR_INVALID_ARGUMENT, "search: null argument");
    if (q->kind < 0 || q->kind > 3) return fail(MOLAR_HIP_ERR_INVALID_ARGUMENT, "search: unknown kind %d", q->kind);
    MH_HIP(hipSetDevice(c->device));
    c->have_search = false;
    c->slot_stat_valid = false;
    c->plan_live = false;
    bool reuse0 = false;
    HeldGrid to_hold;
    MH_TRY(describe_request(c, q, call, degenerate, &reuse0, &to_hold));
    if (*degenerate) return 0;
    MH_TRY(reserve_plan(c, call));
    const int ids_local = q->ids_local || q->kind == MOLAR_HIP_SEARCH_DOUBLE_VDW;
    if (takes_side_lane(c, q, call)) {
        MH_TRY(ensure_side_stream(c));
        if (call.side_wait) MH_HIP(hipStreamWaitEvent(c->side_stream, call.side_wait, 0));
        MH_TRY(build_grids(c, call, side_lane(c), !reuse0, ids_local));
        MH_HIP(hipEventRecord(c->grid_done, c->side_stream));
        if (c->env_host_grid_wait) MH_HIP(hipEventSynchronize(c->grid_done));
        else MH_HIP(hipStreamWaitEvent(c->stream, c->grid_done, 0));
    } else {
        MH_TRY(build_grids(c, call, main_lane(c), !reuse0, ids_local));
    }
    if (to_hold.valid) c->held = to_hold;
    if (call.plan) MH_TRY(enqueue_plan(c, call));
    c->mask_units = 0;
    if (call.size_masks && call.plan) MH_TRY(size_plan(c));
    return 0;
}

namespace {

int finish_count(molar_hip_ctx *c) {
    Prof *prof = new Prof(c, 2);
    SearchSizes *sizes = &c->h_sizes[molar_hip_ctx::SIZES_SYNC], *sizes_dev = sizes_dev_of(c, molar_hip_ctx::SIZES_SYNC);
    *sizes = SearchSizes{};
    int rc = scan_slot_counts(c, sizes_dev);
    delete prof;
    MH_TRY(rc);
    unsigned long long tot = 0;
    if (sizes_dev) {
        MH_HIP(hipStreamSynchronize(c->stream));
        tot = sizes->total;
        occ_note(c, occ_key_of(c->cur), *sizes);
    } else {
        MH_TRY(read_back(c, &tot, c->slot_base.as<unsigned long long>() + c->cur.nslots_bound, 8));
    }
    c->total = tot;
    c->have_search = true;
    return 0;
}

}

extern "C" {

int molar_hip_search_count(molar_hip_ctx *c, const molar_hip_search_desc *q, uint64_t *out_count) {
    SearchCall call;
    bool degenerate;
    MH_TRY(prepare_search(c, q, call, &degenerate));
    if (degenerate) {
        c->have_search = true;
        if (out_count) *out_count = 0;
        return MOLAR_HIP_OK;
    }
    MH_TRY(launch_pairs<false>(c, call, PairOut{}));
    MH_TRY(finish_count(c));
    if (out_count) *out_count = c->total;
    return MOLAR_HIP_OK;
}

int molar_hip_search_grid_dims(molar_hip_ctx *c, uint64_t dims[3]) {
    if (!c || !c->have_search) return fail(MOLAR_HIP_ERR_NO_SEARCH, "no cached search: call molar_hip_search_count first");
    for (int d = 0; d < 3; ++d) dims[d] = c->cur.dims[d];
    return MOLAR_HIP_OK;
}

int molar_hip_search_cell_kernels(molar_hip_ctx *c, int32_t *lanes, uint64_t occupied_cells[2]) {
    if (!c || !lanes) return fail(MOLAR_HIP_ERR_INVALID_ARGUMENT, "search_cell_kernels: null argument");
    *lanes = pair_family(c->cur);
    if (occupied_cells) {
        occupied_cells[0] = c->cur.occ_use[0];
        occupied_cells[1] = c->cur.occ_use[1];
    }
    return MOLAR_HIP_OK;
}

int molar_hip_search_slot_counts(molar_hip_ctx *c, uint64_t *slots, uint64_t *consecutive_slots) {
    if (!c || !slots || !consecutive_slots) return fail(MOLAR_HIP_ERR_INVALID_ARGUMENT, "search_slot_counts: null argument");
    if (!c->slot_stat_valid) return fail(MOLAR_HIP_ERR_NO_SEARCH, "search_slot_counts: the context's last search was not planned by plan_slots_kernel");
    MH_HIP(hipSetDevice(c->device));
    unsigned long long st[2] = {0ull, 0ull};
    MH_TRY(read_back(c, st, c->slot_stat.p, sizeof st));
    *slots = st[0];
    *consecutive_slots = st[1];
    return MOLAR_HIP_OK;
}

static int fill_common(molar_hip_ctx *c, uint2 *d_pairs, float *d_dist, uint32_t *d_ids) {
    if (!c || !c->have_search) return fail(MOLAR_HIP_ERR_NO_SEARCH, "no cached search: call molar_hip_search_count first");
    MH_HIP(hipSetDevice(c->device));
    if (c->total == 0 || c->cur.ntasks == 0) return 0;
    uint2 *p = d_pairs;
    float *d = d_dist;
    const bool via_p = p && ((uintptr_t)p & 15u) != 0, via_d = d && ((uintptr_t)d & 7u) != 0;
    if (via_p) {
        MH_TRY(c->out_pairs.reserve((size_t)c->total * 8));
        p = c->out_pairs.as<uint2>();
    }
    if (via_d) {
        MH_TRY(c->out_dist.reserve((size_t)c->total * 4));
        d = c->out_dist.as<float>();
    }
    MH_TRY(launch_pairs<true>(c, SearchCall{}, PairOut{p, d, d_ids}));
    if (via_p) MH_HIP(hipMemcpyAsync(d_pairs, p, (size_t)c->total * 8, hipMemcpyDeviceToDevice, c->stream));
    if (via_d) MH_HIP(hipMemcpyAsync(d_dist, d, (size_t)c->total * 4, hipMemcpyDeviceToDevice, c->stream));
    return 0;
}

int molar_hip_search_fill(molar_hip_ctx *c, uint32_t *pairs, float *dist) {
    if (!c || !c->have_search) return fail(MOLAR_HIP_ERR_NO_SEARCH, "no cached search: call molar_hip_search_count first");
    if (c->cur.kind == MOLAR_HIP_SEARCH_WITHIN)
        return fail(MOLAR_HIP_ERR_INVALID_ARGUMENT, "within search yields ids: use molar_hip_search_fill_ids");
    const bool pd = is_device_ptr(pairs), dd = is_device_ptr(dist);
    uint2 *dp = nullptr;
    float *ddist = nullptr;
    if (pairs) {
        if (pd) dp = reinterpret_cast<uint2 *>(pairs);
        else {
            MH_TRY(c->out_pairs.reserve((size_t)(c->total ? c->total : 1) * 8));
            dp = c->out_pairs.as<uint2>();
        }
    }
    if (dist) {
        if (dd) ddist = dist;
        else {
            MH_TRY(c->out_dist.reserve((size_t)(c->total ? c->total : 1) * 4));
            ddist = c->out_dist.as<float>();
        }
    }
    MH_TRY(fill_common(c, dp, ddist, nullptr));
    const bool hp = pairs && !pd && c->total, hd = dist && !dd && c->total;
    if (ring_pays(c->total * ((hp ? 8u : 0u) + (hd ? 4u : 0u)), hp ? pairs : nullptr, hd ? dist : nullptr)) {
        std::vector<RingJob> jobs;
        if (hp) jobs.push_back(RingJob{dp, (size_t)c->total * 8, RING_COPY, pairs, nullptr});
        if (hd) jobs.push_back(RingJob{ddist, (size_t)c->total * 4, RING_COPY, dist, nullptr});
        return ring_to_host(c, jobs);
    }
    if (hp) MH_HIP(hipMemcpyAsync(pairs, dp, c->total * 8, hipMemcpyDeviceToHost, c->stream));
    if (hd) MH_HIP(hipMemcpyAsync(dist, ddist, c->total * 4, hipMemcpyDeviceToHost, c->stream));
    if ((pairs && !pd) || (dist && !dd)) MH_HIP(hipStreamSynchronize(c->stream));
    return MOLAR_HIP_OK;
}

int molar_hip_search_fill_device(molar_hip_ctx *c, const uint32_t **d_pairs, const float **d_dist) {
    if (!c || !c->have_search) return fail(MOLAR_HIP_ERR_NO_SEARCH, "no cached search: call molar_hip_search_count first");
    if (c->cur.kind == MOLAR_HIP_SEARCH_WITHIN)
        return fail(MOLAR_HIP_ERR_INVALID_ARGUMENT, "within search yields ids: use molar_hip_search_fill_ids");
    MH_TRY(c->out_pairs.reserve((size_t)(c->total ? c->total : 1) * 8));
    MH_TRY(c->out_dist.reserve((size_t)(c->total ? c->total : 1) * 4));
    MH_TRY(fill_common(c, c->out_pairs.as<uint2>(), c->out_dist.as<float>(), nullptr));
    if (d_pairs) *d_pairs = c->out_pairs.as<uint32_t>();
    if (d_dist) *d_dist = c->out_dist.as<float>();
    return MOLAR_HIP_OK;
}

static int resident_enqueue(molar_hip_ctx *c, const molar_hip_search_desc *q, mh::DevBuf &outP, mh::DevBuf &outD, SearchSizes *sizes,
                            SearchSizes *sizes_dev, ResidentLaunch *L, bool pairs_only, bool trim = true, SearchCall call = SearchCall{}) {
    if (q && q->kind == MOLAR_HIP_SEARCH_WITHIN)
        return fail(MOLAR_HIP_ERR_INVALID_ARGUMENT, "within search yields ids: use molar_hip_search_count + fill_ids");
    const unsigned long long a = outP.cap / 8u, b = outD.cap / 4u;
    const unsigned long long cap0 = a < b ? a : b;
    call.size_masks = false;
    call.out_cap = cap0;
    call.sizes_dev = sizes_dev;
    bool degenerate;
    MH_TRY(prepare_search(c, q, call, &degenerate));
    ++c->search_serial;
// ... 598 lines not shown
```

molar_amd/csrc/search_shape.hpp:

```cpp
#pragma once

#include <algorithm>
#include <cmath>
#include <cstring>

#include "common.hpp"

namespace mh {

inline bool fixed_cutoff_kind(int kind) { return kind == MOLAR_HIP_SEARCH_SINGLE || kind == MOLAR_HIP_SEARCH_DOUBLE; }

inline uint64_t grid_cells(const SearchShape &s) { return (uint64_t)s.dims[0] * s.dims[1] * s.dims[2]; }

inline int dims_from_extents(SearchShape &s, const float ext[3]) {
    double cells = 1.0;
    for (int d = 0; d < 3; ++d) {
        const float q = std::floor(ext[d] / s.cutoff);
        uint64_t n = (q > 0.0f) ? (q >= 4.0e9f ? 4000000000ull : (uint64_t)q) : 0ull;
        if (n < 1) n = 1;
        s.dims[d] = (uint32_t)n;
        cells *= (double)n;
    }
    if (cells > 1.0e8)
        return fail(MOLAR_HIP_ERR_TOO_LARGE, "search grid %u x %u x %u has too many cells (cutoff %g)", s.dims[0],
                    s.dims[1], s.dims[2], (double)s.cutoff);
    return 0;
}

inline uint64_t judged_cells(const SearchShape &s, int set) {
    const uint64_t all = grid_cells(s);
    return s.occ_use[set] ? std::min<uint64_t>(s.occ_use[set], all) : all;
}

inline int small_cell_lanes(const SearchShape &s) {
#ifdef MH_NO_SMALL_CELLS
    return 0;
#endif
    if (!fixed_cutoff_kind(s.kind)) return 0;
    int lanes = 16;
    const int nsets = s.kind == MOLAR_HIP_SEARCH_SINGLE ? 1 : 2;
    for (int k = 0; k < nsets; ++k) {
        const uint64_t cells = judged_cells(s, k), n = s.set[k].n;
        const int l = n <= 13ull * cells ? 16 : (n <= 19ull * cells ? 32 : 0);
        lanes = (l == 0 || lanes == 0) ? 0 : std::max(lanes, l);
    }
    return lanes;
}

inline int pair_family(const SearchShape &s) {
    if (const int lanes = small_cell_lanes(s)) return lanes;
    if (!fixed_cutoff_kind(s.kind)) return 0;
    const int b = s.kind == MOLAR_HIP_SEARCH_SINGLE ? 0 : 1;
    const uint64_t cells = judged_cells(s, b), n = s.set[b].n;
    return n > 1000ull * cells ? -2 : (n > 448ull * cells ? -1 : 0);
}

inline bool records_hit_history(const SearchShape &s) { return fixed_cutoff_kind(s.kind) && small_cell_lanes(s) == 0; }

inline bool sorted_by_device_sort(uint64_t n, uint64_t ncells) { return n > 384ull * ncells; }

inline unsigned long long occ_key_of(const SearchShape &s) {
    unsigned long long h = 1469598103934665603ull;
    auto mix = [&](unsigned long long v) { h = (h ^ v) * 1099511628211ull; };
    mix((unsigned long long)s.kind + 1u); mix(s.set[0].n); mix(s.kind == MOLAR_HIP_SEARCH_SINGLE ? 0u : s.set[1].n);
    mix(s.dims[0]); mix(s.dims[1]); mix(s.dims[2]); mix(s.use_box ? 1u : 2u);
    return h ? h : 1ull;
}

inline uint64_t plan_entries(const SearchShape &s) { return grid_cells(s) * 14ull * (s.kind != MOLAR_HIP_SEARCH_SINGLE ? 2ull : 1ull); }

inline uint64_t slots_bound(const SearchShape &s, bool hist_plan) {
    const uint64_t n0 = s.set[0].n;
    uint64_t bound = (s.kind != MOLAR_HIP_SEARCH_SINGLE ? 28ull : 14ull) * ((n0 + 63ull) / 64ull) + plan_entries(s) + 28ull * 512ull;
    if (hist_plan) bound += (n0 + 31ull) / 32ull + grid_cells(s);
    return bound;
}

constexpr uint64_t FPLAN_MAX_TASKS = 1ull << 22;

constexpr uint32_t LIVE_ROW_GROUPS = 8;
inline bool live_row_slots(const SearchShape &s) {
    return fixed_cutoff_kind(s.kind) && pair_family(s) == 0 && plan_entries(s) + 1 <= FPLAN_MAX_TASKS &&
           (plan_entries(s) <= 8192ull || (uint64_t)s.set[0].n >= 96ull * grid_cells(s));
}
inline size_t live_rows_mask_words(const SearchShape &s) { return (size_t)plan_entries(s) * LIVE_ROW_GROUPS; }
inline size_t live_rows_bytes(const SearchShape &s) { return live_rows_mask_words(s) * 8u + (size_t)plan_entries(s) * 4u; }

inline uint64_t held_fingerprint(const float *xyz, size_t natoms) {
    uint64_t fp = 0xcbf29ce484222325ull;
    auto mix = [&](size_t atom) {
        uint32_t w[3];
        std::memcpy(w, xyz + 3 * atom, 12);
        for (int k = 0; k < 3; ++k) fp = (fp ^ w[k]) * 0x100000001b3ull;
    };
    const size_t n = natoms, step = n > 512 ? n / 512 : 1;
    for (size_t a = 0; a < n && a < 64; ++a) mix(a);
    for (size_t a = 0; a < n; a += step) mix(a);
    for (size_t a = n > 64 ? n - 64 : 0; a < n; ++a) mix(a);
    return fp | 1ull;
}

inline bool held_names_request(const HeldGrid &h, const molar_hip_search_desc &q, const SearchShape &s, uint64_t fp) {
    return h.valid && h.fp == fp && h.set == s.set && h.xyz == q.xyz1 && h.natoms == q.natoms1 && h.idx == q.idx1 && h.n == q.n1 &&
           h.ids_local == q.ids_local && h.use_box == s.use_box && h.pbc == s.pbc &&
           (!s.use_box || std::memcmp(&h.box, &s.box, sizeof s.box) == 0);
}

inline bool held_same_cells(const HeldGrid &h, const SearchShape &s) {
    bool same = h.dims[0] == s.dims[0] && h.dims[1] == s.dims[1] && h.dims[2] == s.dims[2];
    for (int d = 0; d < 3 && !s.use_box; ++d) same = same && h.lower[d] == s.lower[d] && h.upper[d] == s.upper[d];
    return same;
}

inline HeldGrid held_remember(const molar_hip_search_desc &q, const SearchShape &s, uint64_t fp) {
    HeldGrid h;
    h.valid = true;
    h.set = s.set;
    h.fp = fp;
    h.xyz = q.xyz1; h.idx = q.idx1; h.natoms = q.natoms1; h.n = q.n1;
    h.ids_local = q.ids_local;
    h.use_box = s.use_box; h.pbc = s.pbc; h.box = s.box;
    for (int d = 0; d < 3; ++d) { h.dims[d] = s.dims[d]; h.lower[d] = s.lower[d]; h.upper[d] = s.upper[d]; }
    return h;
}

struct WrapPolicy {
    uint32_t wrap_kind;
    uint32_t prune_wrapped;
    uint32_t approx_wrapped;
    float band_lo, band_hi;
    float prune_limit2;
};

inline WrapPolicy wrapped_pair_policy(const SearchShape &s) {
    WrapPolicy W{};
    const float cutoff2 = s.cutoff * s.cutoff;
    W.wrap_kind = 3u;
    if (s.use_box) {
        const float *m = s.box.m, *iv = s.box.inv;
        auto z = [&](int k) { return m[k] == 0.0f && iv[k] == 0.0f; };
        const bool lower_zero = z(1) && z(2) && z(5);
        const bool upper_zero = z(3) && z(6) && z(7);
        if (lower_zero && upper_zero) W.wrap_kind = 1u;
        else if (lower_zero) W.wrap_kind = 2u;
    }
    W.prune_wrapped = 0u;
    if (s.use_box) {
        bool ok = true;
        for (int d = 0; d < 3; ++d)
            if (((s.pbc >> d) & 1u) && s.dims[d] < 3u) ok = false;
        W.prune_wrapped = ok ? 1u : 0u;
    }
    W.approx_wrapped = 0u;
    W.band_lo = W.band_hi = cutoff2;
    float margin = 1.0e-3f;
    if (s.use_box) {
        bool ok = (uint64_t)s.set[0].n + (uint64_t)s.set[1].n < (1ull << 26);
        float ext[3], lmax = 0.f;
        molar_hip_box_lab_extents(&s.box, ext);
        for (int d = 0; d < 3; ++d) {
            if (((s.pbc >> d) & 1u) && s.dims[d] < 4u) ok = false;
            lmax = std::fmax(lmax, std::fabs(ext[d]));
            for (int k = 0; k < 3; ++k) lmax = std::fmax(lmax, std::fabs(s.box.m[3 * k + d]));
        }
        float lsum = 0.f;
        for (int d = 0; d < 3; ++d) {
            float row = 0.f;
            for (int k = 0; k < 3; ++k) row += std::fabs(s.box.m[3 * k + d]);
            lsum = std::fmax(lsum, row);
// ... 33 lines not shown
```

rust/molar_hip/src/ffi.rs:

```rust
#![allow(non_camel_case_types, clippy::too_many_arguments, clippy::missing_safety_doc)]

use std::os::raw::{c_char, c_int, c_void};

use crate::types::{
    MolarHipBox, MolarHipContactGroups, MolarHipCtx, MolarHipFitStream, MolarHipMembraneDesc, MolarHipMembraneOut, MolarHipMembranePatches, MolarHipMembranePlan, MolarHipMembraneState,
    MolarHipMembraneStateF64,
    MolarHipMembraneView, MolarHipSearchDesc, MolarHipSearchDescF64, MolarHipXtc,
};

pub struct MolarHipFns {
    pub create: unsafe extern "C" fn(c_int) -> *mut MolarHipCtx,
    pub destroy: unsafe extern "C" fn(*mut MolarHipCtx),
    pub last_error: unsafe extern "C" fn() -> *const c_char,
    pub version: unsafe extern "C" fn() -> *const c_char,
    pub device_count: unsafe extern "C" fn() -> c_int,
    pub set_stream: unsafe extern "C" fn(*mut MolarHipCtx, *mut c_void) -> c_int,
    pub synchronize: unsafe extern "C" fn(*mut MolarHipCtx) -> c_int,
    pub profile_enable: unsafe extern "C" fn(*mut MolarHipCtx, c_int) -> c_int,
    pub profile_read: unsafe extern "C" fn(*mut MolarHipCtx, *mut f32, *mut u64) -> c_int,
    pub copy_bandwidth: unsafe extern "C" fn(*mut MolarHipCtx, usize, c_int, *mut f32) -> c_int,
    pub write_bandwidth: unsafe extern "C" fn(*mut MolarHipCtx, usize, c_int, *mut f32) -> c_int,
    pub box_from_matrix: unsafe extern "C" fn(*const f32, *mut MolarHipBox) -> c_int,
    pub box_from_vectors_angles: unsafe extern "C" fn(f32, f32, f32, f32, f32, f32, *mut MolarHipBox) -> c_int,
    pub box_shortest_vector: unsafe extern "C" fn(*const MolarHipBox, *const f32, u8, *mut f32),
    pub box_lab_extents: unsafe extern "C" fn(*const MolarHipBox, *mut f32),
    pub box_extents: unsafe extern "C" fn(*const MolarHipBox, *mut f32),
    pub box_to_box_coords: unsafe extern "C" fn(*const MolarHipBox, *const f32, *mut f32),
    pub box_to_lab_coords: unsafe extern "C" fn(*const MolarHipBox, *const f32, *mut f32),
    pub box_is_inside: unsafe extern "C" fn(*const MolarHipBox, *const f32) -> c_int,
    pub box_wrap_point: unsafe extern "C" fn(*const MolarHipBox, *const f32, *mut f32),
    pub search_count: unsafe extern "C" fn(*mut MolarHipCtx, *const MolarHipSearchDesc, *mut u64) -> c_int,
    pub search_fill: unsafe extern "C" fn(*mut MolarHipCtx, *mut u32, *mut f32) -> c_int,
    pub search_fill_usize: unsafe extern "C" fn(*mut MolarHipCtx, *mut u64, *mut u64, *mut f32) -> c_int,
    pub search_fill_ids: unsafe extern "C" fn(*mut MolarHipCtx, *mut u64) -> c_int,
    pub within_count: unsafe extern "C" fn(*mut MolarHipCtx, *const MolarHipSearchDesc, *mut u64) -> c_int,
    pub within_fill: unsafe extern "C" fn(*mut MolarHipCtx, *mut u64) -> c_int,
    pub within_hold: unsafe extern "C" fn(*mut MolarHipCtx, c_int) -> c_int,
    pub search_connectivity: unsafe extern "C" fn(*mut MolarHipCtx, *const MolarHipSearchDesc, *mut u64, *mut u64) -> c_int,
    pub search_connectivity_fill: unsafe extern "C" fn(*mut MolarHipCtx, *mut u64, *mut u64) -> c_int,
    pub unwrap_connectivity: unsafe extern "C" fn(*mut MolarHipCtx, *mut f32, usize, *const u64, usize, *const f32, f32, u8, *mut u64, *mut u64, *mut usize) -> c_int,
    pub search_grid_dims: unsafe extern "C" fn(*mut MolarHipCtx, *mut u64) -> c_int,
    pub search_cell_kernels: unsafe extern "C" fn(*mut MolarHipCtx, *mut i32, *mut u64) -> c_int,
    pub search_slot_counts: unsafe extern "C" fn(*mut MolarHipCtx, *mut u64, *mut u64) -> c_int,
    pub search_fill_device: unsafe extern "C" fn(*mut MolarHipCtx, *mut *const u32, *mut *const f32) -> c_int,
    pub search_resident: unsafe extern "C" fn(*mut MolarHipCtx, *const MolarHipSearchDesc, *mut u64, *mut *const u32, *mut *const f32) -> c_int,
    pub search_resident_planes: unsafe extern "C" fn(*mut MolarHipCtx, c_int) -> c_int,
    pub search_resident_begin: unsafe extern "C" fn(*mut MolarHipCtx, *const MolarHipSearchDesc, *mut i32) -> c_int,
    pub search_resident_end: unsafe extern "C" fn(*mut MolarHipCtx, i32, *mut u64, *mut *const u32, *mut *const f32) -> c_int,
    pub search_histogram: unsafe extern "C" fn(*mut MolarHipCtx, *const MolarHipSearchDesc, f32, f32, usize, *mut u64, *mut u64) -> c_int,
    pub search_histogram_frames: unsafe extern "C" fn(*mut MolarHipCtx, *const MolarHipSearchDesc, usize, usize, usize, *const f32, f32, f32, usize, *mut u64) -> c_int,
    pub histogram_edges: unsafe extern "C" fn(f32, f32, usize, *mut f32) -> c_int,
    pub search_contacts: unsafe extern "C" fn(*mut MolarHipCtx, *const MolarHipSearchDesc, *const MolarHipContactGroups, *mut u64, *mut u64, *mut u64, *mut u64) -> c_int,
    pub search_contacts_frames: unsafe extern "C" fn(*mut MolarHipCtx, *const MolarHipSearchDesc, *const MolarHipContactGroups, usize, usize, usize, *const f32, *mut u64, *mut u64, *mut u64, *mut u32) -> c_int,
    pub search_clusters: unsafe extern "C" fn(*mut MolarHipCtx, *const MolarHipSearchDesc, *const MolarHipContactGroups, *mut u32, *mut u32, *mut u64, *mut u32, *mut u32) -> c_int,
    pub search_clusters_frames: unsafe extern "C" fn(*mut MolarHipCtx, *const MolarHipSearchDesc, *const MolarHipContactGroups, usize, usize, *const f32, *mut u32, *mut u32, *mut u64, *mut u32) -> c_int,
    pub search_clusters_counters: unsafe extern "C" fn(*mut MolarHipCtx, i32, *mut u64) -> c_int,
    pub hbonds_count: unsafe extern "C" fn(*mut MolarHipCtx, *const MolarHipSearchDesc, *const u64, *const u64, usize, i32, f64, f64, *mut u64) -> c_int,
    pub hbonds_fill: unsafe extern "C" fn(*mut MolarHipCtx, *mut u32, *mut f64, *mut f64, *mut f64) -> c_int,
    pub hbonds_counts: unsafe extern "C" fn(*mut MolarHipCtx, *const MolarHipSearchDesc, *const u64, *const u64, usize, i32, f64, f64, *const MolarHipContactGroups, *mut u64, *mut u64, *mut u64, *mut u64) -> c_int,
    pub hbonds_frames: unsafe extern "C" fn(*mut MolarHipCtx, *const MolarHipSearchDesc, *const u64, *const u64, usize, i32, f64, f64, usize, usize, *const f32, *const MolarHipContactGroups, *mut u64, *mut u64, *mut u64, *mut u64, *mut u64, *mut u64) -> c_int,
    pub hbonds_frames_fill: unsafe extern "C" fn(*mut MolarHipCtx, *mut u64, *mut u32, *mut f64, *mut f64, *mut f64, *mut u32, *mut u32, *mut u32) -> c_int,
    pub lifetimes_plan: unsafe extern "C" fn(usize, usize, usize, c_int, *mut usize, *mut u32) -> c_int,
    pub lifetimes: unsafe extern "C" fn(*mut MolarHipCtx, *const u64, *const u32, usize, usize, *const u32, usize, usize, usize, usize, *mut u64, *mut u64, *mut u64, *mut u32, *mut u32, *mut u32) -> c_int,
    pub hbonds_frames_shape: unsafe extern "C" fn(*mut MolarHipCtx, *mut usize, *mut usize, *mut usize, *mut u64) -> c_int,
    pub hbonds_frames_lifetimes: unsafe extern "C" fn(*mut MolarHipCtx, *const u32, usize, usize, usize, usize, *mut u64, *mut u64, *mut u64, *mut u32, *mut u32, *mut u32) -> c_int,
    pub search_count_f64: unsafe extern "C" fn(*mut MolarHipCtx, *const MolarHipSearchDescF64, *mut u64) -> c_int,
    pub search_fill_f64: unsafe extern "C" fn(*mut MolarHipCtx, *mut u64, *mut u64, *mut f64) -> c_int,
    pub search_fill_ids_f64: unsafe extern "C" fn(*mut MolarHipCtx, *mut u64) -> c_int,
    pub search_grid_dims_f64: unsafe extern "C" fn(*mut MolarHipCtx, *mut u64) -> c_int,
    pub search_histogram_f64: unsafe extern "C" fn(*mut MolarHipCtx, *const MolarHipSearchDescF64, f64, f64, usize, *mut u64, *mut u64) -> c_int,
    pub search_histogram_frames_f64: unsafe extern "C" fn(*mut MolarHipCtx, *const MolarHipSearchDescF64, usize, usize, usize, *const f64, f64, f64, usize, *mut u64) -> c_int,
    pub histogram_edges_f64: unsafe extern "C" fn(f64, f64, usize, *mut f64) -> c_int,
    pub within_count_f64: unsafe extern "C" fn(*mut MolarHipCtx, *const MolarHipSearchDescF64, *mut u64) -> c_int,
    pub within_fill_f64: unsafe extern "C" fn(*mut MolarHipCtx, *mut u64) -> c_int,
    pub search_connectivity_f64: unsafe extern "C" fn(*mut MolarHipCtx, *const MolarHipSearchDescF64, *mut u64, *mut u64) -> c_int,
    pub unwrap_connectivity_f64: unsafe extern "C" fn(*mut MolarHipCtx, *mut f64, usize, *const u64, usize, *const f64, f64, u8, *mut u64, *mut u64, *mut usize) -> c_int,
    pub min_max: unsafe extern "C" fn(*mut MolarHipCtx, *const f32, usize, *const u64, usize, *mut f32, *mut f32) -> c_int,
    pub center_of_geometry: unsafe extern "C" fn(*mut MolarHipCtx, *const f32, usize, *const u64, usize, *mut f32) -> c_int,
    pub center_of_mass: unsafe extern "C" fn(*mut MolarHipCtx, *const f32, usize, *const u64, usize, *const f32, *mut f32) -> c_int,
    pub center_of_geometry_pbc: unsafe extern "C" fn(*mut MolarHipCtx, *const f32, usize, *const u64, usize, *const f32, u8, *mut f32) -> c_int,
    pub center_of_mass_pbc: unsafe extern "C" fn(*mut MolarHipCtx, *const f32, usize, *const u64, usize, *const f32, *const f32, u8, *mut f32) -> c_int,
    pub gyration: unsafe extern "C" fn(*mut MolarHipCtx, *const f32, usize, *const u64, usize, *const f32, *const f32, *mut f32) -> c_int,
    pub inertia: unsafe extern "C" fn(*mut MolarHipCtx, *const f32, usize, *const u64, usize, *const f32, *const f32, *mut f32, *mut f32, *mut f32) -> c_int,
    pub rmsd: unsafe extern "C" fn(*mut MolarHipCtx, *const f32, usize, *const u64, usize, *const f32, usize, *const u64, usize, *mut f32) -> c_int,
    pub rmsd_mw: unsafe extern "C" fn(*mut MolarHipCtx, *const f32, usize, *const u64, usize, *const f32, *const f32, usize, *const u64, usize, *mut f32) -> c_int,
    pub fit_transform: unsafe extern "C" fn(*mut MolarHipCtx, *const f32, usize, *const u64, usize, *const f32, *const f32, usize, *const u64, usize, *const f32, c_int, *mut f32, *mut f32) -> c_int,
    pub center_of_geometry_f64: unsafe extern "C" fn(*mut MolarHipCtx, *const f64, usize, *const u64, usize, *mut f64) -> c_int,
    pub center_of_mass_f64: unsafe extern "C" fn(*mut MolarHipCtx, *const f64, usize, *const u64, usize, *const f64, *mut f64) -> c_int,
    pub gyration_f64: unsafe extern "C" fn(*mut MolarHipCtx, *const f64, usize, *const u64, usize, *const f64, *mut f64) -> c_int,
    pub rmsd_f64: unsafe extern "C" fn(*mut MolarHipCtx, *const f64, usize, *const u64, usize, *const f64, usize, *const u64, usize, *mut f64) -> c_int,
    pub rmsd_mw_f64: unsafe extern "C" fn(*mut MolarHipCtx, *const f64, usize, *const u64, usize, *const f64, *const f64, usize, *const u64, usize, *mut f64) -> c_int,
    pub fit_transform_f64: unsafe extern "C" fn(*mut MolarHipCtx, *const f64, usize, *const u64, usize, *const f64, *const f64, usize, *const u64, usize, *const f64, c_int, *mut f64, *mut f64) -> c_int,
    pub min_max_f64: unsafe extern "C" fn(*mut MolarHipCtx, *const f64, usize, *const u64, usize, *mut f64, *mut f64) -> c_int,
    pub inertia_f64: unsafe extern "C" fn(*mut MolarHipCtx, *const f64, usize, *const u64, usize, *const f64, *mut f64, *mut f64, *mut f64) -> c_int,
    pub translate_f64: unsafe extern "C" fn(*mut MolarHipCtx, *mut f64, usize, *const u64, usize, *const f64) -> c_int,
    pub sasa_points: unsafe extern "C" fn(u32, *mut f32) -> c_int,
    pub sasa_points_f64: unsafe extern "C" fn(u32, *mut f64) -> c_int,
    pub sasa: unsafe extern "C" fn(*mut MolarHipCtx, *const f32, usize, *const u64, usize, *const f32, f32, u32, *mut f32, *mut u32, *mut f64) -> c_int,
    pub sasa_f64: unsafe extern "C" fn(*mut MolarHipCtx, *const f64, usize, *const u64, usize, *const f64, f64, u32, *mut f64, *mut u32, *mut f64) -> c_int,
    pub sasa_frames: unsafe extern "C" fn(*mut MolarHipCtx, *const f32, usize, usize, usize, *const u64, usize, *const f32, f32, u32, *mut f32, *mut f64) -> c_int,
    pub sasa_vol: unsafe extern "C" fn(*mut MolarHipCtx, *const f32, usize, *const u64, usize, *const f32, f32, u32, *mut f32, *mut u32, *mut f64, *mut f32, *mut f64) -> c_int,
    pub sasa_vol_f64: unsafe extern "C" fn(*mut MolarHipCtx, *const f64, usize, *const u64, usize, *const f64, f64, u32, *mut f64, *mut u32, *mut f64, *mut f64, *mut f64) -> c_int,
    pub sasa_vol_frames: unsafe extern "C" fn(*mut MolarHipCtx, *const f32, usize, usize, usize, *const u64, usize, *const f32, f32, u32, *mut f32, *mut f64, *mut f32, *mut f64) -> c_int,
    pub rmsd_matrix_plan: unsafe extern "C" fn(usize, usize, usize, *mut usize, *mut u32) -> c_int,
    pub rmsd_matrix: unsafe extern "C" fn(*mut MolarHipCtx, *const f32, usize, usize, *const f32, usize, usize, usize, *const u64, usize, *const f32, c_int, *mut f32, usize) -> c_int,
    pub rmsd_matrix_f64: unsafe extern "C" fn(*mut MolarHipCtx, *const f64, usize, usize, *const f64, usize, usize, usize, *const u64, usize, *const f64, c_int, *mut f64, usize) -> c_int,
    pub fluct_plan: unsafe extern "C" fn(usize, usize, c_int, *mut usize, *mut u32) -> c_int,
    pub fluct: unsafe extern "C" fn(*mut MolarHipCtx, *const f32, usize, usize, usize, *const u64, usize, *const f32, *const f32, c_int, c_int, *mut f32, *mut f32, *mut f32, usize, *mut f32) -> c_int,
    pub fluct_f64: unsafe extern "C" fn(*mut MolarHipCtx, *const f64, usize, usize, usize, *const u64, usize, *const f64, *const f64, c_int, c_int, *mut f64, *mut f64, *mut f64, usize, *mut f64) -> c_int,
    pub msd_plan: unsafe extern "C" fn(usize, usize, usize, usize, usize, c_int, c_int, *mut usize, *mut u32, *mut u32) -> c_int,
    pub msd: unsafe extern "C" fn(*mut MolarHipCtx, *const f32, usize, usize, usize, *const u64, usize, *const f32, *const f32, usize, u8, *const u64, usize, *const u64, usize, usize, usize, u32, *mut f32, *mut f32, *mut f32, usize, *mut f32) -> c_int,
    pub msd_f64: unsafe extern "C" fn(*mut MolarHipCtx, *const f64, usize, usize, usize, *const u64, usize, *const f64, *const f64, usize, u8, *const u64, usize, *const u64, usize, usize, usize, u32, *mut f64, *mut f64, *mut f64, usize, *mut f64) -> c_int,
    pub fit_rmsd_batch_f64: unsafe extern "C" fn(*mut MolarHipCtx, *mut f64, usize, usize, *const u64, usize, *const f64, *const f64, usize, *const u64, c_int, *mut f64, *mut f64, *mut f64, *mut f64, *mut f64) -> c_int,
    pub center_of_geometry_pbc_f64: unsafe extern "C" fn(*mut MolarHipCtx, *const f64, usize, *const u64, usize, *const f64, u8, *mut f64) -> c_int,
    pub center_of_mass_pbc_f64: unsafe extern "C" fn(*mut MolarHipCtx, *const f64, usize, *const u64, usize, *const f64, *const f64, u8, *mut f64) -> c_int,
    pub gyration_pbc_f64: unsafe extern "C" fn(*mut MolarHipCtx, *const f64, usize, *const u64, usize, *const f64, *const f64, *mut f64) -> c_int,
    pub unwrap_simple_f64: unsafe extern "C" fn(*mut MolarHipCtx, *mut f64, usize, *const u64, usize, *const f64, u8) -> c_int,
    pub rotate_f64: unsafe extern "C" fn(*mut MolarHipCtx, *mut f64, usize, *const u64, usize, *const f64, f64) -> c_int,
    pub principal_transform_f64: unsafe extern "C" fn(*mut MolarHipCtx, *const f64, usize, *const u64, usize, *const f64, *const f64, *mut f64, *mut f64) -> c_int,
    pub lipid_tail_order_f64: unsafe extern "C" fn(*mut MolarHipCtx, *const f64, usize, *const u64, *const u64, usize, c_int, *const f64, *const u64, *const u8, *mut f64) -> c_int,
    pub inertia_pbc_f64: unsafe extern "C" fn(*mut MolarHipCtx, *const f64, usize, *const u64, usize, *const f64, *const f64, *mut f64, *mut f64, *mut f64) -> c_int,
    pub apply_transform_f64: unsafe extern "C" fn(*mut MolarHipCtx, *mut f64, usize, *const u64, usize, *const f64, *const f64) -> c_int,
    pub center_batch: unsafe extern "C" fn(*mut MolarHipCtx, *const f32, usize, *const u64, *const u64, usize, *const f32, *mut f32) -> c_int,
    pub unwrap_simple_batch: unsafe extern "C" fn(*mut MolarHipCtx, *mut f32, usize, *const u64, *const u64, usize, *const f32, u8) -> c_int,
    pub center_batch_f64: unsafe extern "C" fn(*mut MolarHipCtx, *const f64, usize, *const u64, *const u64, usize, *const f64, *mut f64) -> c_int,
    pub unwrap_simple_batch_f64: unsafe extern "C" fn(*mut MolarHipCtx, *mut f64, usize, *const u64, *const u64, usize, *const f64, u8) -> c_int,
    pub membrane_initial_normals: unsafe extern "C" fn(usize, *const f32, *const f32, *const u64, *const u64, *const u8, *mut f32) -> c_int,
    pub membrane_patches_from_pairs: unsafe extern "C" fn(*const u32, usize, usize, *mut u64, *mut u64) -> c_int,
    pub membrane_smooth: unsafe extern "C" fn(*mut MolarHipCtx, *const MolarHipMembranePatches, *const f32, *mut MolarHipMembraneState) -> c_int,
    pub membrane_nth_shell_patches: unsafe extern "C" fn(usize, *const u8, *const u64, *const u64, *const u32, *const u64, usize, *mut u64, *mut u64, usize, *mut usize) -> c_int,
    pub membrane_smooth_curvature: unsafe extern "C" fn(usize, *const u8, *const u64, *const u32, *const u64, usize, *mut f32, *mut f32) -> c_int,
    pub membrane_smooth_f64: unsafe extern "C" fn(*mut MolarHipCtx, *const MolarHipMembranePatches, *const f64, *mut MolarHipMembraneStateF64) -> c_int,
    pub membrane_initial_normals_f64: unsafe extern "C" fn(usize, *const f64, *const f64, *const u64, *const u64, *const u8, *mut f64) -> c_int,
    pub membrane_smooth_curvature_f64: unsafe extern "C" fn(usize, *const u8, *const u64, *const u32, *const u64, usize, *mut f64, *mut f64) -> c_int,
    pub membrane_plan_create: unsafe extern "C" fn(*mut MolarHipCtx, *const MolarHipMembraneDesc, *mut *mut MolarHipMembranePlan) -> c_int,
    pub membrane_plan_destroy: unsafe extern "C" fn(*mut MolarHipMembranePlan),
    pub membrane_plan_set_valid: unsafe extern "C" fn(*mut MolarHipMembranePlan, *const u8) -> c_int,
    pub membrane_plan_set_shells: unsafe extern "C" fn(*mut MolarHipMembranePlan, usize, usize) -> c_int,
    pub membrane_frame_begin: unsafe extern "C" fn(*mut MolarHipMembranePlan, *mut f32, *const f32, *mut i32) -> c_int,
    pub membrane_frame_end: unsafe extern "C" fn(*mut MolarHipMembranePlan, i32, *mut MolarHipMembraneView) -> c_int,
    pub membrane_frame_fetch: unsafe extern "C" fn(*mut MolarHipMembranePlan, i32, *const MolarHipMembraneOut) -> c_int,
    pub membrane_frame_end_fetch: unsafe extern "C" fn(*mut MolarHipMembranePlan, i32, *mut MolarHipMembraneView, *const MolarHipMembraneOut) -> c_int,
    pub lipid_tail_order: unsafe extern "C" fn(*mut MolarHipCtx, *const f32, usize, *const u64, *const u64, usize, c_int, *const f32, *const u64, *const u8, *mut f32) -> c_int,
    pub xtc_open: unsafe extern "C" fn(*const c_char) -> *mut MolarHipXtc,
    pub xtc_open_memory: unsafe extern "C" fn(*const c_void, usize) -> *mut MolarHipXtc,
    pub xtc_close: unsafe extern "C" fn(*mut MolarHipXtc),
    pub xtc_nframes: unsafe extern "C" fn(*const MolarHipXtc) -> usize,
    pub xtc_natoms: unsafe extern "C" fn(*const MolarHipXtc) -> usize,
    pub xtc_frame_info: unsafe extern "C" fn(*const MolarHipXtc, usize, *mut i32, *mut i32, *mut f32, *mut f32, *mut f32) -> c_int,
    pub xtc_seek_time: unsafe extern "C" fn(*const MolarHipXtc, f32, *mut usize) -> c_int,
    pub xtc_read: unsafe extern "C" fn(*mut MolarHipCtx, *const MolarHipXtc, usize, usize, *mut f32, c_int) -> c_int,
    pub xtc_read_device: unsafe extern "C" fn(*mut MolarHipCtx, *const MolarHipXtc, usize, usize, *mut f32) -> c_int,
    pub xtc_histogram: unsafe extern "C" fn(*mut MolarHipCtx, *const MolarHipXtc, usize, usize, *const u64, usize, f32, u8, f32, f32, usize, *mut u64, c_int) -> c_int,
    pub xtc_histogram_double: unsafe extern "C" fn(*mut MolarHipCtx, *const MolarHipXtc, usize, usize, *const u64, usize, *const u64, usize, f32, u8, f32, f32, usize, *mut u64, c_int) -> c_int,
    pub xtc_encode_frame: unsafe extern "C" fn(*const f32, usize, *const f32, i32, f32, f32, *mut u8, usize, *mut usize) -> c_int,
    pub apply_transform: unsafe extern "C" fn(*mut MolarHipCtx, *mut f32, usize, *const u64, usize, *const f32, *const f32) -> c_int,
    pub unwrap_simple: unsafe extern "C" fn(*mut MolarHipCtx, *mut f32, usize, *const u64, usize, *const f32, u8) -> c_int,
    pub fit_rmsd_batch: unsafe extern "C" fn(*mut MolarHipCtx, *mut f32, usize, usize, *const u64, usize, *const f32, *const f32, usize, *const u64, c_int, *mut f32, *mut f32, *mut f32, *mut f32, *mut f32) -> c_int,
    pub fit_stream_create: unsafe extern "C" fn(*mut MolarHipCtx, usize, *const u64, usize, *const f32, *const f32, usize, *const u64, c_int, *mut *mut MolarHipFitStream) -> c_int,
    pub fit_stream_begin: unsafe extern "C" fn(*mut MolarHipFitStream, *mut f32, c_int, *mut i32) -> c_int,
    pub fit_stream_end: unsafe extern "C" fn(*mut MolarHipFitStream, i32, *mut f32, *mut f32, *mut f32, *mut f32, *mut f32) -> c_int,
    pub fit_stream_destroy: unsafe extern "C" fn(*mut MolarHipFitStream),
    pub gyration_batch: unsafe extern "C" fn(*mut MolarHipCtx, *const f32, usize, *const u64, *const u64, usize, *const f32, *const f32, *mut f32) -> c_int,
    pub rmsd_batch: unsafe extern "C" fn(*mut MolarHipCtx, *const f32, usize, *const u64, *const f32, usize, *const u64, *const u64, usize, *const f32, *mut f32) -> c_int,
    pub fit_batch: unsafe extern "C" fn(*mut MolarHipCtx, *mut f32, usize, *const u64, *const f32, *const f32, usize, *const u64, *const f32, *const u64, usize, c_int, *mut f32, *mut f32, *mut f32, *mut f32, *mut f32) -> c_int,
    pub translate: unsafe extern "C" fn(*mut MolarHipCtx, *mut f32, usize, *const u64, usize, *const f32) -> c_int,
    pub rotate: unsafe extern "C" fn(*mut MolarHipCtx, *mut f32, usize, *const u64, usize, *const f32, f32) -> c_int,
    pub principal_transform: unsafe extern "C" fn(*mut MolarHipCtx, *const f32, usize, *const u64, usize, *const f32, *const f32, *mut f32, *mut f32) -> c_int,
}

impl MolarHipFns {
    pub unsafe fn resolve(lib: &libloading::Library) -> Result<Self, libloading::Error> {
        unsafe {
            Ok(MolarHipFns {
                create: *lib.get::<unsafe extern "C" fn(c_int) -> *mut MolarHipCtx>(b"molar_hip_create\0")?,
                destroy: *lib.get::<unsafe extern "C" fn(*mut MolarHipCtx)>(b"molar_hip_destroy\0")?,
                last_error: *lib.get::<unsafe extern "C" fn() -> *const c_char>(b"molar_hip_last_error\0")?,
                version: *lib.get::<unsafe extern "C" fn() -> *const c_char>(b"molar_hip_version\0")?,
                device_count: *lib.get::<unsafe extern "C" fn() -> c_int>(b"molar_hip_device_count\0")?,
                set_stream: *lib.get::<unsafe extern "C" fn(*mut MolarHipCtx, *mut c_void) -> c_int>(b"molar_hip_set_stream\0")?,
                synchronize: *lib.get::<unsafe extern "C" fn(*mut MolarHipCtx) -> c_int>(b"molar_hip_synchronize\0")?,
                profile_enable: *lib.get::<unsafe extern "C" fn(*mut MolarHipCtx, c_int) -> c_int>(b"molar_hip_profile_enable\0")?,
                profile_read: *lib.get::<unsafe extern "C" fn(*mut MolarHipCtx, *mut f32, *mut u64) -> c_int>(b"molar_hip_profile_read\0")?,
                copy_bandwidth: *lib.get::<unsafe extern "C" fn(*mut MolarHipCtx, usize, c_int, *mut f32) -> c_int>(b"molar_hip_copy_bandwidth\0")?,
                write_bandwidth: *lib.get::<unsafe extern "C" fn(*mut MolarHipCtx, usize, c_int, *mut f32) -> c_int>(b"molar_hip_write_bandwidth\0")?,
                box_from_matrix: *lib.get::<unsafe extern "C" fn(*const f32, *mut MolarHipBox) -> c_int>(b"molar_hip_box_from_matrix\0")?,
                box_from_vectors_angles: *lib.get::<unsafe extern "C" fn(f32, f32, f32, f32, f32, f32, *mut MolarHipBox) -> c_int>(b"molar_hip_box_from_vectors_angles\0")?,
                box_shortest_vector: *lib.get::<unsafe extern "C" fn(*const MolarHipBox, *const f32, u8, *mut f32)>(b"molar_hip_box_shortest_vector\0")?,
                box_lab_extents: *lib.get::<unsafe extern "C" fn(*const MolarHipBox, *mut f32)>(b"molar_hip_box_lab_extents\0")?,
                box_extents: *lib.get::<unsafe extern "C" fn(*const MolarHipBox, *mut f32)>(b"molar_hip_box_extents\0")?,
                box_to_box_coords: *lib.get::<unsafe extern "C" fn(*const MolarHipBox, *const f32, *mut f32)>(b"molar_hip_box_to_box_coords\0")?,
                box_to_lab_coords: *lib.get::<unsafe extern "C" fn(*const MolarHipBox, *const f32, *mut f32)>(b"molar_hip_box_to_lab_coords\0")?,
                box_is_inside: *lib.get::<unsafe extern "C" fn(*const MolarHipBox, *const f32) -> c_int>(b"molar_hip_box_is_inside\0")?,
                box_wrap_point: *lib.get::<unsafe extern "C" fn(*const MolarHipBox, *const f32, *mut f32)>(b"molar_hip_box_wrap_point\0")?,
                search_count: *lib.get::<unsafe extern "C" fn(*mut MolarHipCtx, *const MolarHipSearchDesc, *mut u64) -> c_int>(b"molar_hip_search_count\0")?,
                search_fill: *lib.get::<unsafe extern "C" fn(*mut MolarHipCtx, *mut u32, *mut f32) -> c_int>(b"molar_hip_search_fill\0")?,
                search_fill_usize: *lib.get::<unsafe extern "C" fn(*mut MolarHipCtx, *mut u64, *mut u64, *mut f32) -> c_int>(b"molar_hip_search_fill_usize\0")?,
                search_fill_ids: *lib.get::<unsafe extern "C" fn(*mut MolarHipCtx, *mut u64) -> c_int>(b"molar_hip_search_fill_ids\0")?,
                within_count: *lib.get::<unsafe extern "C" fn(*mut MolarHipCtx, *const MolarHipSearchDesc, *mut u64) -> c_int>(b"molar_hip_within_count\0")?,
                within_fill: *lib.get::<unsafe extern "C" fn(*mut MolarHipCtx, *mut u64) -> c_int>(b"molar_hip_within_fill\0")?,
                within_hold: *lib.get::<unsafe extern "C" fn(*mut MolarHipCtx, c_int) -> c_int>(b"molar_hip_within_hold\0")?,
                search_connectivity: *lib.get::<unsafe extern "C" fn(*mut MolarHipCtx, *const MolarHipSearchDesc, *mut u64, *mut u64) -> c_int>(b"molar_hip_search_connectivity\0")?,
                search_connectivity_fill: *lib.get::<unsafe extern "C" fn(*mut MolarHipCtx, *mut u64, *mut u64) -> c_int>(b"molar_hip_search_connectivity_fill\0")?,
                unwrap_connectivity: *lib.get::<unsafe extern "C" fn(*mut MolarHipCtx, *mut f32, usize, *const u64, usize, *const f32, f32, u8, *mut u64, *mut u64, *mut usize) -> c_int>(b"molar_hip_unwrap_connectivity\0")?,
                search_grid_dims: *lib.get::<unsafe extern "C" fn(*mut MolarHipCtx, *mut u64) -> c_int>(b"molar_hip_search_grid_dims\0")?,
                search_cell_kernels: *lib.get::<unsafe extern "C" fn(*mut MolarHipCtx, *mut i32, *mut u64) -> c_int>(b"molar_hip_search_cell_kernels\0")?,
                search_slot_counts: *lib.get::<unsafe extern "C" fn(*mut MolarHipCtx, *mut u64, *mut u64) -> c_int>(b"molar_hip_search_slot_counts\0")?,
                search_fill_device: *lib.get::<unsafe extern "C" fn(*mut MolarHipCtx, *mut *const u32, *mut *const f32) -> c_int>(b"molar_hip_search_fill_device\0")?,
                search_resident: *lib.get::<unsafe extern "C" fn(*mut MolarHipCtx, *const MolarHipSearchDesc, *mut u64, *mut *const u32, *mut *const f32) -> c_int>(b"molar_hip_search_resident\0")?,
                search_resident_planes: *lib.get::<unsafe extern "C" fn(*mut MolarHipCtx, c_int) -> c_int>(b"molar_hip_search_resident_planes\0")?,
                search_resident_begin: *lib.get::<unsafe extern "C" fn(*mut MolarHipCtx, *const MolarHipSearchDesc, *mut i32) -> c_int>(b"molar_hip_search_resident_begin\0")?,
                search_resident_end: *lib.get::<unsafe extern "C" fn(*mut MolarHipCtx, i32, *mut u64, *mut *const u32, *mut *const f32) -> c_int>(b"molar_hip_search_resident_end\0")?,
                search_histogram: *lib.get::<unsafe extern "C" fn(*mut MolarHipCtx, *const MolarHipSearchDesc, f32, f32, usize, *mut u64, *mut u64) -> c_int>(b"molar_hip_search_histogram\0")?,
                search_histogram_frames: *lib.get::<unsafe extern "C" fn(*mut MolarHipCtx, *const MolarHipSearchDesc, usize, usize, usize, *const f32, f32, f32, usize, *mut u64) -> c_int>(b"molar_hip_search_histogram_frames\0")?,
                histogram_edges: *lib.get::<unsafe extern "C" fn(f32, f32, usize, *mut f32) -> c_int>(b"molar_hip_histogram_edges\0")?,
                search_contacts: *lib.get::<unsafe extern "C" fn(*mut MolarHipCtx, *const MolarHipSearchDesc, *const MolarHipContactGroups, *mut u64, *mut u64, *mut u64, *mut u64) -> c_int>(b"molar_hip_search_contacts\0")?,
                search_contacts_frames: *lib.get::<unsafe extern "C" fn(*mut MolarHipCtx, *const MolarHipSearchDesc, *const MolarHipContactGroups, usize, usize, usize, *const f32, *mut u64, *mut u64, *mut u64, *mut u32) -> c_int>(b"molar_hip_search_contacts_frames\0")?,
                search_clusters: *lib.get::<unsafe extern "C" fn(*mut MolarHipCtx, *const MolarHipSearchDesc, *const MolarHipContactGroups, *mut u32, *mut u32, *mut u64, *mut u32, *mut u32) -> c_int>(b"molar_hip_search_clusters\0")?,
                search_clusters_frames: *lib.get::<unsafe extern "C" fn(*mut MolarHipCtx, *const MolarHipSearchDesc, *const MolarHipContactGroups, usize, usize, *const f32, *mut u32, *mut u32, *mut u64, *mut u32) -> c_int>(b"molar_hip_search_clusters_frames\0")?,
                search_clusters_counters: *lib.get::<unsafe extern "C" fn(*mut MolarHipCtx, i32, *mut u64) -> c_int>(b"molar_hip_search_clusters_counters\0")?,
                hbonds_count: *lib.get::<unsafe extern "C" fn(*mut MolarHipCtx, *const MolarHipSearchDesc, *const u64, *const u64, usize, i32, f64, f64, *mut u64) -> c_int>(b"molar_hip_hbonds_count\0")?,
                hbonds_fill: *lib.get::<unsafe extern "C" fn(*mut MolarHipCtx, *mut u32, *mut f64, *mut f64, *mut f64) -> c_int>(b"molar_hip_hbonds_fill\0")?,
                hbonds_counts: *lib.get::<unsafe extern "C" fn(*mut MolarHipCtx, *const MolarHipSearchDesc, *const u64, *const u64, usize, i32, f64, f64, *const MolarHipContactGroups, *mut u64, *mut u64, *mut u64, *mut u64) -> c_int>(b"molar_hip_hbonds_counts\0")?,
                hbonds_frames: *lib.get::<unsafe extern "C" fn(*mut MolarHipCtx, *const MolarHipSearchDesc, *const u64, *const u64, usize, i32, f64, f64, usize, usize, *const f32, *const MolarHipContactGroups, *mut u64, *mut u64, *mut u64, *mut u64, *mut u64, *mut u64) -> c_int>(b"molar_hip_hbonds_frames\0")?,
                hbonds_frames_fill: *lib.get::<unsafe extern "C" fn(*mut MolarHipCtx, *mut u64, *mut u32, *mut f64, *mut f64, *mut f64, *mut u32, *mut u32, *mut u32) -> c_int>(b"molar_hip_hbonds_frames_fill\0")?,
                lifetimes_plan: *lib.get::<unsafe extern "C" fn(usize, usize, usize, c_int, *mut usize, *mut u32) -> c_int>(b"molar_hip_lifetimes_plan\0")?,
                lifetimes: *lib.get::<unsafe extern "C" fn(*mut MolarHipCtx, *const u64, *const u32, usize, usize, *const u32, usize, usize, usize, usize, *mut u64, *mut u64, *mut u64, *mut u32, *mut u32, *mut u32) -> c_int>(b"molar_hip_lifetimes\0")?,
                hbonds_frames_shape: *lib.get::<unsafe extern "C" fn(*mut MolarHipCtx, *mut usize, *mut usize, *mut usize, *mut u64) -> c_int>(b"molar_hip_hbonds_frames_shape\0")?,
                hbonds_frames_lifetimes: *lib.get::<unsafe extern "C" fn(*mut MolarHipCtx, *const u32, usize, usize, usize, usize, *mut u64, *mut u64, *mut u64, *mut u32, *mut u32, *mut u32) -> c_int>(b"molar_hip_hbonds_frames_lifetimes\0")?,
                search_count_f64: *lib.get::<unsafe extern "C" fn(*mut MolarHipCtx, *const MolarHipSearchDescF64, *mut u64) -> c_int>(b"molar_hip_search_count_f64\0")?,
                search_fill_f64: *lib.get::<unsafe extern "C" fn(*mut MolarHipCtx, *mut u64, *mut u64, *mut f64) -> c_int>(b"molar_hip_search_fill_f64\0")?,
                search_fill_ids_f64: *lib.get::<unsafe extern "C" fn(*mut MolarHipCtx, *mut u64) -> c_int>(b"molar_hip_search_fill_ids_f64\0")?,
                search_grid_dims_f64: *lib.get::<unsafe extern "C" fn(*mut MolarHipCtx, *mut u64) -> c_int>(b"molar_hip_search_grid_dims_f64\0")?,
                search_histogram_f64: *lib.get::<unsafe extern "C" fn(*mut MolarHipCtx, *const MolarHipSearchDescF64, f64, f64, usize, *mut u64, *mut u64) -> c_int>(b"molar_hip_search_histogram_f64\0")?,
                search_histogram_frames_f64: *lib.get::<unsafe extern "C" fn(*mut MolarHipCtx, *const MolarHipSearchDescF64, usize, usize, usize, *const f64, f64, f64, usize, *mut u64) -> c_int>(b"molar_hip_search_histogram_frames_f64\0")?,
                histogram_edges_f64: *lib.get::<unsafe extern "C" fn(f64, f64, usize, *mut f64) -> c_int>(b"molar_hip_histogram_edges_f64\0")?,
                within_count_f64: *lib.get::<unsafe extern "C" fn(*mut MolarHipCtx, *const MolarHipSearchDescF64, *mut u64) -> c_int>(b"molar_hip_within_count_f64\0")?,
                within_fill_f64: *lib.get::<unsafe extern "C" fn(*mut MolarHipCtx, *mut u64) -> c_int>(b"molar_hip_within_fill_f64\0")?,
                search_connectivity_f64: *lib.get::<unsafe extern "C" fn(*mut MolarHipCtx, *const MolarHipSearchDescF64, *mut u64, *mut u64) -> c_int>(b"molar_hip_search_connectivity_f64\0")?,
                unwrap_connectivity_f64: *lib.get::<unsafe extern "C" fn(*mut MolarHipCtx, *mut f64, usize, *const u64, usize, *const f64, f64, u8, *mut u64, *mut u64, *mut usize) -> c_int>(b"molar_hip_unwrap_connectivity_f64\0")?,
                min_max: *lib.get::<unsafe extern "C" fn(*mut MolarHipCtx, *const f32, usize, *const u64, usize, *mut f32, *mut f32) -> c_int>(b"molar_hip_min_max\0")?,
                center_of_geometry: *lib.get::<unsafe extern "C" fn(*mut MolarHipCtx, *const f32, usize, *const u64, usize, *mut f32) -> c_int>(b"molar_hip_center_of_geometry\0")?,
                center_of_mass: *lib.get::<unsafe extern "C" fn(*mut MolarHipCtx, *const f32, usize, *const u64, usize, *const f32, *mut f32) -> c_int>(b"molar_hip_center_of_mass\0")?,
                center_of_geometry_pbc: *lib.get::<unsafe extern "C" fn(*mut MolarHipCtx, *const f32, usize, *const u64, usize, *const f32, u8, *mut f32) -> c_int>(b"molar_hip_center_of_geometry_pbc\0")?,
                center_of_mass_pbc: *lib.get::<unsafe extern "C" fn(*mut MolarHipCtx, *const f32, usize, *const u64, usize, *const f32, *const f32, u8, *mut f32) -> c_int>(b"molar_hip_center_of_mass_pbc\0")?,
                gyration: *lib.get::<unsafe extern "C" fn(*mut MolarHipCtx, *const f32, usize, *const u64, usize, *const f32, *const f32, *mut f32) -> c_int>(b"molar_hip_gyration\0")?,
                inertia: *lib.get::<unsafe extern "C" fn(*mut MolarHipCtx, *const f32, usize, *const u64, usize, *const f32, *const f32, *mut f32, *mut f32, *mut f32) -> c_int>(b"molar_hip_inertia\0")?,
                rmsd: *lib.get::<unsafe extern "C" fn(*mut MolarHipCtx, *const f32, usize, *const u64, usize, *const f32, usize, *const u64, usize, *mut f32) -> c_int>(b"molar_hip_rmsd\0")?,
                rmsd_mw: *lib.get::<unsafe extern "C" fn(*mut MolarHipCtx, *const f32, usize, *const u64, usize, *const f32, *const f32, usize, *const u64, usize, *mut f32) -> c_int>(b"molar_hip_rmsd_mw\0")?,
                fit_transform: *lib.get::<unsafe extern "C" fn(*mut MolarHipCtx, *const f32, usize, *const u64, usize, *const f32, *const f32, usize, *const u64, usize, *const f32, c_int, *mut f32, *mut f32) -> c_int>(b"molar_hip_fit_transform\0")?,
                center_of_geometry_f64: *lib.get::<unsafe extern "C" fn(*mut MolarHipCtx, *const f64, usize, *const u64, usize, *mut f64) -> c_int>(b"molar_hip_center_of_geometry_f64\0")?,
                center_of_mass_f64: *lib.get::<unsafe extern "C" fn(*mut MolarHipCtx, *const f64, usize, *const u64, usize, *const f64, *mut f64) -> c_int>(b"molar_hip_center_of_mass_f64\0")?,
                gyration_f64: *lib.get::<unsafe extern "C" fn(*mut MolarHipCtx, *const f64, usize, *const u64, usize, *const f64, *mut f64) -> c_int>(b"molar_hip_gyration_f64\0")?,
                rmsd_f64: *lib.get::<unsafe extern "C" fn(*mut MolarHipCtx, *const f64, usize, *const u64, usize, *const f64, usize, *const u64, usize, *mut f64) -> c_int>(b"molar_hip_rmsd_f64\0")?,
                rmsd_mw_f64: *lib.get::<unsafe extern "C" fn(*mut MolarHipCtx, *const f64, usize, *const u64, usize, *const f64, *const f64, usize, *const u64, usize, *mut f64) -> c_int>(b"molar_hip_rmsd_mw_f64\0")?,
                fit_transform_f64: *lib.get::<unsafe extern "C" fn(*mut MolarHipCtx, *const f64, usize, *const u64, usize, *const f64, *const f64, usize, *const u64, usize, *const f64, c_int, *mut f64, *mut f64) -> c_int>(b"molar_hip_fit_transform_f64\0")?,
                min_max_f64: *lib.get::<unsafe extern "C" fn(*mut MolarHipCtx, *const f64, usize, *const u64, usize, *mut f64, *mut f64) -> c_int>(b"molar_hip_min_max_f64\0")?,
                inertia_f64: *lib.get::<unsafe extern "C" fn(*mut MolarHipCtx, *const f64, usize, *const u64, usize, *const f64, *mut f64, *mut f64, *mut f64) -> c_int>(b"molar_hip_inertia_f64\0")?,
                translate_f64: *lib.get::<unsafe extern "C" fn(*mut MolarHipCtx, *mut f64, usize, *const u64, usize, *const f64) -> c_int>(b"molar_hip_translate_f64\0")?,
                sasa_points: *lib.get::<unsafe extern "C" fn(u32, *mut f32) -> c_int>(b"molar_hip_sasa_points\0")?,
                sasa_points_f64: *lib.get::<unsafe extern "C" fn(u32, *mut f64) -> c_int>(b"molar_hip_sasa_points_f64\0")?,
                sasa: *lib.get::<unsafe extern "C" fn(*mut MolarHipCtx, *const f32, usize, *const u64, usize, *const f32, f32, u32, *mut f32, *mut u32, *mut f64) -> c_int>(b"molar_hip_sasa\0")?,
                sasa_f64: *lib.get::<unsafe extern "C" fn(*mut MolarHipCtx, *const f64, usize, *const u64, usize, *const f64, f64, u32, *mut f64, *mut u32, *mut f64) -> c_int>(b"molar_hip_sasa_f64\0")?,
                sasa_frames: *lib.get::<unsafe extern "C" fn(*mut MolarHipCtx, *const f32, usize, usize, usize, *const u64, usize, *const f32, f32, u32, *mut f32, *mut f64) -> c_int>(b"molar_hip_sasa_frames\0")?,
                sasa_vol: *lib.get::<unsafe extern "C" fn(*mut MolarHipCtx, *const f32, usize, *const u64, usize, *const f32, f32, u32, *mut f32, *mut u32, *mut f64, *mut f32, *mut f64) -> c_int>(b"molar_hip_sasa_vol\0")?,
                sasa_vol_f64: *lib.get::<unsafe extern "C" fn(*mut MolarHipCtx, *const f64, usize, *const u64, usize, *const f64, f64, u32, *mut f64, *mut u32, *mut f64, *mut f64, *mut f64) -> c_int>(b"molar_hip_sasa_vol_f64\0")?,
                sasa_vol_frames: *lib.get::<unsafe extern "C" fn(*mut MolarHipCtx, *const f32, usize, usize, usize, *const u64, usize, *const f32, f32, u32, *mut f32, *mut f64, *mut f32, *mut f64) -> c_int>(b"molar_hip_sasa_vol_frames\0")?,
                rmsd_matrix_plan: *lib.get::<unsafe extern "C" fn(usize, usize, usize, *mut usize, *mut u32) -> c_int>(b"molar_hip_rmsd_matrix_plan\0")?,
                rmsd_matrix: *lib.get::<unsafe extern "C" fn(*mut MolarHipCtx, *const f32, usize, usize, *const f32, usize, usize, usize, *const u64, usize, *const f32, c_int, *mut f32, usize) -> c_int>(b"molar_hip_rmsd_matrix\0")?,
                rmsd_matrix_f64: *lib.get::<unsafe extern "C" fn(*mut MolarHipCtx, *const f64, usize, usize, *const f64, usize, usize, usize, *const u64, usize, *const f64, c_int, *mut f64, usize) -> c_int>(b"molar_hip_rmsd_matrix_f64\0")?,
                fluct_plan: *lib.get::<unsafe extern "C" fn(usize, usize, c_int, *mut usize, *mut u32) -> c_int>(b"molar_hip_fluct_plan\0")?,
                fluct: *lib.get::<unsafe extern "C" fn(*mut MolarHipCtx, *const f32, usize, usize, usize, *const u64, usize, *const f32, *const f32, c_int, c_int, *mut f32, *mut f32, *mut f32, usize, *mut f32) -> c_int>(b"molar_hip_fluct\0")?,
                fluct_f64: *lib.get::<unsafe extern "C" fn(*mut MolarHipCtx, *const f64, usize, usize, usize, *const u64, usize, *const f64, *const f64, c_int, c_int, *mut f64, *mut f64, *mut f64, usize, *mut f64) -> c_int>(b"molar_hip_fluct_f64\0")?,
                msd_plan: *lib.get::<unsafe extern "C" fn(usize, usize, usize, usize, usize, c_int, c_int, *mut usize, *mut u32, *mut u32) -> c_int>(b"molar_hip_msd_plan\0")?,
                msd: *lib.get::<unsafe extern "C" fn(*mut MolarHipCtx, *const f32, usize, usize, usize, *const u64, usize, *const f32, *const f32, usize, u8, *const u64, usize, *const u64, usize, usize, usize, u32, *mut f32, *mut f32, *mut f32, usize, *mut f32) -> c_int>(b"molar_hip_msd\0")?,
                msd_f64: *lib.get::<unsafe extern "C" fn(*mut MolarHipCtx, *const f64, usize, usize, usize, *const u64, usize, *const f64, *const f64, usize, u8, *const u64, usize, *const u64, usize, usize, usize, u32, *mut f64, *mut f64, *mut f64, usize, *mut f64) -> c_int>(b"molar_hip_msd_f64\0")?,
                fit_rmsd_batch_f64: *lib.get::<unsafe extern "C" fn(*mut MolarHipCtx, *mut f64, usize, usize, *const u64, usize, *const f64, *const f64, usize, *const u64, c_int, *mut f64, *mut f64, *mut f64, *mut f64, *mut f64) -> c_int>(b"molar_hip_fit_rmsd_batch_f64\0")?,
                center_of_geometry_pbc_f64: *lib.get::<unsafe extern "C" fn(*mut MolarHipCtx, *const f64, usize, *const u64, usize, *const f64, u8, *mut f64) -> c_int>(b"molar_hip_center_of_geometry_pbc_f64\0")?,
                center_of_mass_pbc_f64: *lib.get::<unsafe extern "C" fn(*mut MolarHipCtx, *const f64, usize, *const u64, usize, *const f64, *const f64, u8, *mut f64) -> c_int>(b"molar_hip_center_of_mass_pbc_f64\0")?,
                gyration_pbc_f64: *lib.get::<unsafe extern "C" fn(*mut MolarHipCtx, *const f64, usize, *const u64, usize, *const f64, *const f64, *mut f64) -> c_int>(b"molar_hip_gyration_pbc_f64\0")?,
                unwrap_simple_f64: *lib.get::<unsafe extern "C" fn(*mut MolarHipCtx, *mut f64, usize, *const u64, usize, *const f64, u8) -> c_int>(b"molar_hip_unwrap_simple_f64\0")?,
                rotate_f64: *lib.get::<unsafe extern "C" fn(*mut MolarHipCtx, *mut f64, usize, *const u64, usize, *const f64, f64) -> c_int>(b"molar_hip_rotate_f64\0")?,
                principal_transform_f64: *lib.get::<unsafe extern "C" fn(*mut MolarHipCtx, *const f64, usize, *const u64, usize, *const f64, *const f64, *mut f64, *mut f64) -> c_int>(b"molar_hip_principal_transform_f64\0")?,
                lipid_tail_order_f64: *lib.get::<unsafe extern "C" fn(*mut MolarHipCtx, *const f64, usize, *const u64, *const u64, usize, c_int, *const f64, *const u64, *const u8, *mut f64) -> c_int>(b"molar_hip_lipid_tail_order_f64\0")?,
                inertia_pbc_f64: *lib.get::<unsafe extern "C" fn(*mut MolarHipCtx, *const f64, usize, *const u64, usize, *const f64, *const f64, *mut f64, *mut f64, *mut f64) -> c_int>(b"molar_hip_inertia_pbc_f64\0")?,
                apply_transform_f64: *lib.get::<unsafe extern "C" fn(*mut MolarHipCtx, *mut f64, usize, *const u64, usize, *const f64, *const f64) -> c_int>(b"molar_hip_apply_transform_f64\0")?,
                center_batch: *lib.get::<unsafe extern "C" fn(*mut MolarHipCtx, *const f32, usize, *const u64, *const u64, usize, *const f32, *mut f32) -> c_int>(b"molar_hip_center_batch\0")?,
                unwrap_simple_batch: *lib.get::<unsafe extern "C" fn(*mut MolarHipCtx, *mut f32, usize, *const u64, *const u64, usize, *const f32, u8) -> c_int>(b"molar_hip_unwrap_simple_batch\0")?,
                center_batch_f64: *lib.get::<unsafe extern "C" fn(*mut MolarHipCtx, *const f64, usize, *const u64, *const u64, usize, *const f64, *mut f64) -> c_int>(b"molar_hip_center_batch_f64\0")?,
                unwrap_simple_batch_f64: *lib.get::<unsafe extern "C" fn(*mut MolarHipCtx, *mut f64, usize, *const u64, *const u64, usize, *const f64, u8) -> c_int>(b"molar_hip_unwrap_simple_batch_f64\0")?,
                membrane_initial_normals: *lib.get::<unsafe extern "C" fn(usize, *const f32, *const f32, *const u64, *const u64, *const u8, *mut f32) -> c_int>(b"molar_hip_membrane_initial_normals\0")?,
                membrane_patches_from_pairs: *lib.get::<unsafe extern "C" fn(*const u32, usize, usize, *mut u64, *mut u64) -> c_int>(b"molar_hip_membrane_patches_from_pairs\0")?,
                membrane_smooth: *lib.get::<unsafe extern "C" fn(*mut MolarHipCtx, *const MolarHipMembranePatches, *const f32, *mut MolarHipMembraneState) -> c_int>(b"molar_hip_membrane_smooth\0")?,
                membrane_nth_shell_patches: *lib.get::<unsafe extern "C" fn(usize, *const u8, *const u64, *const u64, *const u32, *const u64, usize, *mut u64, *mut u64, usize, *mut usize) -> c_int>(b"molar_hip_membrane_nth_shell_patches\0")?,
                membrane_smooth_curvature: *lib.get::<unsafe extern "C" fn(usize, *const u8, *const u64, *const u32, *const u64, usize, *mut f32, *mut f32) -> c_int>(b"molar_hip_membrane_smooth_curvature\0")?,
                membrane_smooth_f64: *lib.get::<unsafe extern "C" fn(*mut MolarHipCtx, *const MolarHipMembranePatches, *const f64, *mut MolarHipMembraneStateF64) -> c_int>(b"molar_hip_membrane_smooth_f64\0")?,
                membrane_initial_normals_f64: *lib.get::<unsafe extern "C" fn(usize, *const f64, *const f64, *const u64, *const u64, *const u8, *mut f64) -> c_int>(b"molar_hip_membrane_initial_normals_f64\0")?,
                membrane_smooth_curvature_f64: *lib.get::<unsafe extern "C" fn(usize, *const u8, *const u64, *const u32, *const u64, usize, *mut f64, *mut f64) -> c_int>(b"molar_hip_membrane_smooth_curvature_f64\0")?,
                membrane_plan_create: *lib.get::<unsafe extern "C" fn(*mut MolarHipCtx, *const MolarHipMembraneDesc, *mut *mut MolarHipMembranePlan) -> c_int>(b"molar_hip_membrane_plan_create\0")?,
                membrane_plan_destroy: *lib.get::<unsafe extern "C" fn(*mut MolarHipMembranePlan)>(b"molar_hip_membrane_plan_destroy\0")?,
                membrane_plan_set_valid: *lib.get::<unsafe extern "C" fn(*mut MolarHipMembranePlan, *const u8) -> c_int>(b"molar_hip_membrane_plan_set_valid\0")?,
                membrane_plan_set_shells: *lib.get::<unsafe extern "C" fn(*mut MolarHipMembranePlan, usize, usize) -> c_int>(b"molar_hip_membrane_plan_set_shells\0")?,
                membrane_frame_begin: *lib.get::<unsafe extern "C" fn(*mut MolarHipMembranePlan, *mut f32, *const f32, *mut i32) -> c_int>(b"molar_hip_membrane_frame_begin\0")?,
                membrane_frame_end: *lib.get::<unsafe extern "C" fn(*mut MolarHipMembranePlan, i32, *mut MolarHipMembraneView) -> c_int>(b"molar_hip_membrane_frame_end\0")?,
                membrane_frame_fetch: *lib.get::<unsafe extern "C" fn(*mut MolarHipMembranePlan, i32, *const MolarHipMembraneOut) -> c_int>(b"molar_hip_membrane_frame_fetch\0")?,
                membrane_frame_end_fetch: *lib.get::<unsafe extern "C" fn(*mut MolarHipMembranePlan, i32, *mut MolarHipMembraneView, *const MolarHipMembraneOut) -> c_int>(b"molar_hip_membrane_frame_end_fetch\0")?,
                lipid_tail_order: *lib.get::<unsafe extern "C" fn(*mut MolarHipCtx, *const f32, usize, *const u64, *const u64, usize, c_int, *const f32, *const u64, *const u8, *mut f32) -> c_int>(b"molar_hip_lipid_tail_order\0")?,
                xtc_open: *lib.get::<unsafe extern "C" fn(*const c_char) -> *mut MolarHipXtc>(b"molar_hip_xtc_open\0")?,
                xtc_open_memory: *lib.get::<unsafe extern "C" fn(*const c_void, usize) -> *mut MolarHipXtc>(b"molar_hip_xtc_open_memory\0")?,
                xtc_close: *lib.get::<unsafe extern "C" fn(*mut MolarHipXtc)>(b"molar_hip_xtc_close\0")?,
                xtc_nframes: *lib.get::<unsafe extern "C" fn(*const MolarHipXtc) -> usize>(b"molar_hip_xtc_nframes\0")?,
                xtc_natoms: *lib.get::<unsafe extern "C" fn(*const MolarHipXtc) -> usize>(b"molar_hip_xtc_natoms\0")?,
                xtc_frame_info: *lib.get::<unsafe extern "C" fn(*const MolarHipXtc, usize, *mut i32, *mut i32, *mut f32, *mut f32, *mut f32) -> c_int>(b"molar_hip_xtc_frame_info\0")?,
                xtc_seek_time: *lib.get::<unsafe extern "C" fn(*const MolarHipXtc, f32, *mut usize) -> c_int>(b"molar_hip_xtc_seek_time\0")?,
                xtc_read: *lib.get::<unsafe extern "C" fn(*mut MolarHipCtx, *const MolarHipXtc, usize, usize, *mut f32, c_int) -> c_int>(b"molar_hip_xtc_read\0")?,
                xtc_read_device: *lib.get::<unsafe extern "C" fn(*mut MolarHipCtx, *const MolarHipXtc, usize, usize, *mut f32) -> c_int>(b"molar_hip_xtc_read_device\0")?,
                xtc_histogram: *lib.get::<unsafe extern "C" fn(*mut MolarHipCtx, *const MolarHipXtc, usize, usize, *const u64, usize, f32, u8, f32, f32, usize, *mut u64, c_int) -> c_int>(b"molar_hip_xtc_histogram\0")?,
                xtc_histogram_double: *lib.get::<unsafe extern "C" fn(*mut MolarHipCtx, *const MolarHipXtc, usize, usize, *const u64, usize, *const u64, usize, f32, u8, f32, f32, usize, *mut u64, c_int) -> c_int>(b"molar_hip_xtc_histogram_double\0")?,
                xtc_encode_frame: *lib.get::<unsafe extern "C" fn(*const f32, usize, *const f32, i32, f32, f32, *mut u8, usize, *mut usize) -> c_int>(b"molar_hip_xtc_encode_frame\0")?,
                apply_transform: *lib.get::<unsafe extern "C" fn(*mut MolarHipCtx, *mut f32, usize, *const u64, usize, *const f32, *const f32) -> c_int>(b"molar_hip_apply_transform\0")?,
                unwrap_simple: *lib.get::<unsafe extern "C" fn(*mut MolarHipCtx, *mut f32, usize, *const u64, usize, *const f32, u8) -> c_int>(b"molar_hip_unwrap_simple\0")?,
                fit_rmsd_batch: *lib.get::<unsafe extern "C" fn(*mut MolarHipCtx, *mut f32, usize, usize, *const u64, usize, *const f32, *const f32, usize, *const u64, c_int, *mut f32, *mut f32, *mut f32, *mut f32, *mut f32) -> c_int>(b"molar_hip_fit_rmsd_batch\0")?,
                fit_stream_create: *lib.get::<unsafe extern "C" fn(*mut MolarHipCtx, usize, *const u64, usize, *const f32, *const f32, usize, *const u64, c_int, *mut *mut MolarHipFitStream) -> c_int>(b"molar_hip_fit_stream_create\0")?,
                fit_stream_begin: *lib.get::<unsafe extern "C" fn(*mut MolarHipFitStream, *mut f32, c_int, *mut i32) -> c_int>(b"molar_hip_fit_stream_begin\0")?,
                fit_stream_end: *lib.get::<unsafe extern "C" fn(*mut MolarHipFitStream, i32, *mut f32, *mut f32, *mut f32, *mut f32, *mut f32) -> c_int>(b"molar_hip_fit_stream_end\0")?,
                fit_stream_destroy: *lib.get::<unsafe extern "C" fn(*mut MolarHipFitStream)>(b"molar_hip_fit_stream_destroy\0")?,
                gyration_batch: *lib.get::<unsafe extern "C" fn(*mut MolarHipCtx, *const f32, usize, *const u64, *const u64, usize, *const f32, *const f32, *mut f32) -> c_int>(b"molar_hip_gyration_batch\0")?,
                rmsd_batch: *lib.get::<unsafe extern "C" fn(*mut MolarHipCtx, *const f32, usize, *const u64, *const f32, usize, *const u64, *const u64, usize, *const f32, *mut f32) -> c_int>(b"molar_hip_rmsd_batch\0")?,
                fit_batch: *lib.get::<unsafe extern "C" fn(*mut MolarHipCtx, *mut f32, usize, *const u64, *const f32, *const f32, usize, *const u64, *const f32, *const u64, usize, c_int, *mut f32, *mut f32, *mut f32, *mut f32, *mut f32) -> c_int>(b"molar_hip_fit_batch\0")?,
                translate: *lib.get::<unsafe extern "C" fn(*mut MolarHipCtx, *mut f32, usize, *const u64, usize, *const f32) -> c_int>(b"molar_hip_translate\0")?,
                rotate: *lib.get::<unsafe extern "C" fn(*mut MolarHipCtx, *mut f32, usize, *const u64, usize, *const f32, f32) -> c_int>(b"molar_hip_rotate\0")?,
                principal_transform: *lib.get::<unsafe extern "C" fn(*mut MolarHipCtx, *const f32, usize, *const u64, usize, *const f32, *const f32, *mut f32, *mut f32) -> c_int>(b"molar_hip_principal_transform\0")?,
            })
        }
    }
}

pub const ENTRY_POINTS: usize = 158;
```

Baseline: 762.7 frames/s.

## Precompute compacted live-row lists and radius bounds in the live-rows pass

The live-rows prepass now writes a compacted uint16 list of live row indices and a per-task max radius bound, alongside the bitmasks. The pair kernel then reads its row directly and uses the precomputed bound, replacing the per-slot mask scan, LDS scatter and wave max-reduction. The prepass is also regrouped per home cell, split into shares, and reuses loaded atoms across tasks that share the same source cell. This adds a larger buffer of row lists per plan entry and more global writes in the prepass. A debug export entry point is added as well.

```diff
diff --git a/include/molar_hip.h b/include/molar_hip.h
--- a/include/molar_hip.h
+++ b/include/molar_hip.h
@@ -111,6 +111,8 @@
 int molar_hip_search_grid_dims(molar_hip_ctx *ctx, uint64_t dims[3]);
 int molar_hip_search_cell_kernels(molar_hip_ctx *ctx, int32_t *lanes, uint64_t occupied_cells[2]);
 int molar_hip_search_slot_counts(molar_hip_ctx *ctx, uint64_t *slots, uint64_t *consecutive_slots);
+int molar_hip_search_live_rows(molar_hip_ctx *ctx, uint64_t entries_cap, uint64_t *entries, uint64_t *masks, uint32_t *counts, uint16_t *rows,
+                               float *bounds);
 int molar_hip_search_fill_device(molar_hip_ctx *ctx, const uint32_t **d_pairs, const float **d_dist);
 int molar_hip_search_resident(molar_hip_ctx *ctx, const molar_hip_search_desc *desc, uint64_t *out_count,
                               const uint32_t **d_pairs, const float **d_dist);
diff --git a/molar_amd/_lib.py b/molar_amd/_lib.py
--- a/molar_amd/_lib.py
+++ b/molar_amd/_lib.py
@@ -105,6 +105,7 @@
     "molar_hip_search_grid_dims": (_I, [_P, _P]),
     "molar_hip_search_cell_kernels": (_I, [_P, _P, _P]),
     "molar_hip_search_slot_counts": (_I, [_P, _P, _P]),
+    "molar_hip_search_live_rows": (_I, [_P, C.c_uint64, _P, _P, _P, _P, _P]),
     "molar_hip_search_count_f64": (_I, [_P, _P, _P]),
     "molar_hip_search_fill_f64": (_I, [_P, _P, _P, _P]),
     "molar_hip_search_fill_ids_f64": (_I, [_P, _P]),
diff --git a/molar_amd/api.py b/molar_amd/api.py
--- a/molar_amd/api.py
+++ b/molar_amd/api.py
@@ -278,6 +278,16 @@
         slots, rows = C.c_uint64(0), C.c_uint64(0)
         check(self.lib.molar_hip_search_slot_counts(self.ctx, C.byref(slots), C.byref(rows)))
         return int(slots.value), int(rows.value)
+
+    def search_live_rows(self):
+        n = C.c_uint64(0)
+        check(self.lib.molar_hip_search_live_rows(self.ctx, 0, C.byref(n), None, None, None, None))
+        ne = int(n.value)
+        masks, counts = np.empty((ne, 8), np.uint64), np.empty(ne, np.uint32)
+        rows, bounds = np.empty((ne, 512), np.uint16), np.empty(ne, np.float32)
+        check(self.lib.molar_hip_search_live_rows(self.ctx, ne, C.byref(n), masks.ctypes.data, counts.ctypes.data, rows.ctypes.data,
+                                                  bounds.ctypes.data))
+        return masks, counts, rows, bounds
 
     def search_resident_planes(self, want_dist=True):
         check(self.lib.molar_hip_search_resident_planes(self.ctx, 1 if want_dist else 0))
diff --git a/molar_amd/csrc/common.hpp b/molar_amd/csrc/common.hpp
--- a/molar_amd/csrc/common.hpp
+++ b/molar_amd/csrc/common.hpp
@@ -123,6 +123,7 @@
     DevBuf h16;
     DevBuf cell_org;
     DevBuf live;
+    DevBuf live_list;
 };
 
 struct SearchShape {
diff --git a/molar_amd/csrc/pair_kernels.hpp b/molar_amd/csrc/pair_kernels.hpp
--- a/molar_amd/csrc/pair_kernels.hpp
+++ b/molar_amd/csrc/pair_kernels.hpp
@@ -128,6 +128,7 @@
 struct SlotTask : Task {
     bool live = false;
     uint32_t lrow = 0;
+    float bound2 = 0.0f;
 };
 
 __device__ __forceinline__ uint32_t slot_row(const SlotTask &T, uint32_t i0, uint32_t lane) { return T.live ? T.lrow : i0 + lane; }
@@ -714,9 +715,16 @@
     }
     if (TRI || need) la[rank] = a;
     const float r0 = a.x - org.x, r1 = a.y - org.y, r2 = a.z - org.z;
-    float ra2 = need ? (r0 * r0 + r1 * r1) + r2 * r2 : 0.0f;
-    const bool fin = ra2 == ra2;
-    for (int off = 32; off > 0; off >>= 1) ra2 = fmaxf(ra2, __shfl_xor(ra2, off, 64));
+    float ra2;
+    bool fin;
+    if (T.live) {
+        ra2 = T.bound2;
+        fin = ra2 == ra2;
+    } else {
+        ra2 = need ? (r0 * r0 + r1 * r1) + r2 * r2 : 0.0f;
+        fin = ra2 == ra2;
+        for (int off = 32; off > 0; off >>= 1) ra2 = fmaxf(ra2, __shfl_xor(ra2, off, 64));
+    }
     const float R = 1.0001f * __builtin_sqrtf(ra2) + org.w;
     const float E = uniform_f32(mfma_error_bound(R, cutoff2));
     if (__builtin_amdgcn_ballot_w64(!fin) != 0ull || !mfma_bound_usable(R, E, cutoff2)) {
@@ -1472,30 +1480,13 @@
             T.rps = fl >> 16;
             if constexpr (LIVE_SLOTS) {
                 if (fl & SLOT_LIVE) {
-                    typedef __attribute__((address_space(1))) unsigned long long glb_u64;
+                    typedef __attribute__((address_space(1))) unsigned short glb_u16;
                     const uint2 mp = reinterpret_cast<const uint2 *>(slot_desc + slot)[5];
-                    const glb_u64 *mk = (const glb_u64 *)(((unsigned long long)(uint32_t)__builtin_amdgcn_readfirstlane(mp.y) << 32) |
+                    const glb_u16 *lr = (const glb_u16 *)(((unsigned long long)(uint32_t)__builtin_amdgcn_readfirstlane(mp.y) << 32) |
                                                           (unsigned long long)(uint32_t)__builtin_amdgcn_readfirstlane(mp.x));
-                    unsigned long long mw = 0ull;
-                    if (lane < (uint32_t)LIVE_GROUPS) mw = mk[lane];
-                    uint32_t *scr = lds[wave][0];
-                    uint32_t before = 0u;
-#pragma unroll
-                    for (int g = 0; g < LIVE_GROUPS; ++g) {
-                        const uint32_t wlo = __builtin_amdgcn_readlane((uint32_t)mw, g), whi = __builtin_amdgcn_readlane((uint32_t)(mw >> 32), g);
-                        const uint32_t n = (uint32_t)__popc(wlo) + (uint32_t)__popc(whi);
-                        if (n != 0u && before + n > i0 && before < i0 + 64u) {
-                            const uint32_t rank = before + __builtin_amdgcn_mbcnt_hi(whi, __builtin_amdgcn_mbcnt_lo(wlo, 0u)) - i0;
-                            const bool bit = (((lane < 32u ? wlo : whi) >> (lane & 31u)) & 1u) != 0u;
-                            if (bit && rank < 64u) scr[rank] = 64u * (uint32_t)g + lane;
-                        }
-                        before += n;
-                    }
-                    __builtin_amdgcn_wave_barrier();
-                    T.lrow = scr[lane];
-                    __builtin_amdgcn_wave_barrier();
+                    T.lrow = (uint32_t)lr[i0 + lane];
                     T.live = true;
-                    T.n1 = before;
+                    T.bound2 = __uint_as_float((uint32_t)__builtin_amdgcn_readfirstlane(hi.w));
                 }
             }
         }
diff --git a/molar_amd/csrc/search.hip b/molar_amd/csrc/search.hip
--- a/molar_amd/csrc/search.hip
+++ b/molar_amd/csrc/search.hip
@@ -584,49 +584,92 @@
 
 constexpr uint32_t LIVE_NONE = 0xFFFFFFFFu;
 static_assert(LIVE_ROW_GROUPS == (uint32_t)LIVE_GROUPS, "the host sizes the masks the kernels index");
+#ifndef MH_LIVE_SHARES
+#define MH_LIVE_SHARES 2
+#endif
+constexpr uint32_t LIVE_SHARES = MH_LIVE_SHARES;
+static_assert(LIVE_ROW_STRIDE == 64u * (uint32_t)LIVE_GROUPS, "the host sizes the row lists the kernels index");
+static __constant__ uint8_t LIVE_ORDER_DOUBLE[28] = {0, 2, 4, 6, 8, 10, 12, 14, 1, 16, 18, 3, 27, 20, 5, 17, 25, 22, 9, 7, 19, 21, 23, 24, 11, 26, 13, 15};
 template <int KIND>
-__global__ void __launch_bounds__(64) live_rows_kernel(SearchParams P, unsigned long long *__restrict__ masks, uint32_t *__restrict__ live_cnt) {
-    const uint64_t t = (uint64_t)blockIdx.y * gridDim.x + blockIdx.x;
-    if (t >= P.ntasks) return;
+__global__ void __launch_bounds__(64) live_rows_kernel(SearchParams P, unsigned long long *__restrict__ masks, uint32_t *__restrict__ live_cnt,
+                                                       uint16_t *__restrict__ live_row, float *__restrict__ live_bound) {
+    constexpr uint32_t NE = KIND == MOLAR_HIP_SEARCH_SINGLE ? 14u : 28u;
+    constexpr uint32_t PER = (NE + LIVE_SHARES - 1u) / LIVE_SHARES;
+    const uint64_t w = (uint64_t)blockIdx.y * gridDim.x + blockIdx.x;
+    const uint64_t home = w / LIVE_SHARES;
+    const uint32_t share = (uint32_t)(w % LIVE_SHARES);
     const uint32_t lane = threadIdx.x;
-    const Task T = decode_task<KIND, true>(P, t);
-    const bool wrapped = P.use_box && T.wrap != 0u;
-    const bool approx = wrapped && P.approx_wrapped != 0u && !(P.box.nshift != 0 && T.wrap == MOLAR_HIP_PBC_FULL);
-    if (!T.valid || T.tri || T.rps != 64u || T.n1 > 64u * (uint32_t)LIVE_GROUPS || T.n2 > 64u * (uint32_t)KREG || (wrapped && !approx)) {
-        if (lane == 0) live_cnt[t] = LIVE_NONE;
-        return;
-    }
-    float Sx = 0.f, Sy = 0.f, Sz = 0.f;
-    float limit2 = P.cutoff2;
-    if (approx) {
+    float4 a[LIVE_GROUPS];
 #pragma unroll
-        for (int d = 0; d < 3; ++d) {
-            if (!((T.wrap >> d) & 1u)) continue;
-            const float sgn = ((T.wrap_b >> d) & 1u) ? 1.0f : -1.0f;
-            Sx += sgn * P.box.m[3 * d];
-            Sy += sgn * P.box.m[3 * d + 1];
-            Sz += sgn * P.box.m[3 * d + 2];
-        }
-        limit2 = P.prune_limit2;
-    }
-    const float4 lo = gload4(P.aabb_b, 2 * T.cb), hi = gload4(P.aabb_b, 2 * T.cb + 1);
-    unsigned long long mine = 0ull;
-    uint32_t nlive = 0u;
+    for (int g = 0; g < LIVE_GROUPS; ++g) a[g] = make_float4(0.f, 0.f, 0.f, 0.f);
+    uint32_t have = 0xFFFFFFFFu;
+    const uint32_t k1 = (share + 1u) * PER < NE ? (share + 1u) * PER : NE;
+#pragma unroll 1
+    for (uint32_t k = share * PER; k < k1; ++k) {
+        const uint64_t t = home * NE + (KIND == MOLAR_HIP_SEARCH_SINGLE ? k : (uint32_t)LIVE_ORDER_DOUBLE[k]);
+        if (t >= P.ntasks) continue;
+        const Task T = decode_task<KIND, true>(P, t);
+        const bool wrapped = P.use_box && T.wrap != 0u;
+        const bool approx = wrapped && P.approx_wrapped != 0u && !(P.box.nshift != 0 && T.wrap == MOLAR_HIP_PBC_FULL);
+        if (!T.valid || T.tri || T.rps != 64u || T.n1 > 64u * (uint32_t)LIVE_GROUPS || T.n2 > 64u * (uint32_t)KREG || (wrapped && !approx)) {
+            if (lane == 0) live_cnt[t] = LIVE_NONE;
+            continue;
+        }
+        const float4 lo = gload4(P.aabb_b, 2 * T.cb), hi = gload4(P.aabb_b, 2 * T.cb + 1);
+        const float4 org = gload4(P.cell_org_b, T.cb);
+        const uint32_t ca = __builtin_amdgcn_readfirstlane(T.ca);
+        if (ca != have) {
 #pragma unroll
-    for (int g = 0; g < LIVE_GROUPS; ++g) {
-        const uint32_t row = 64u * (uint32_t)g + lane;
-        if (64u * (uint32_t)g >= T.n1) break;
-        bool need = false;
-        if (row < T.n1) {
-            const float4 a = gload4(P.sa, T.a0 + row);
-            need = !(aabb_d2(a.x - Sx, a.y - Sy, a.z - Sz, lo.x, lo.y, lo.z, hi.x, hi.y, hi.z) > limit2);
-        }
-        const unsigned long long m = __builtin_amdgcn_ballot_w64(need);
-        if (lane == (uint32_t)g) mine = m;
-        nlive += (uint32_t)__popcll(m);
-    }
-    if (lane < (uint32_t)LIVE_GROUPS) masks[t * (uint64_t)LIVE_GROUPS + lane] = mine;
-    if (lane == 0) live_cnt[t] = nlive;
+            for (int g = 0; g < LIVE_GROUPS; ++g) {
+                const uint32_t row = 64u * (uint32_t)g + lane;
+                if (64u * (uint32_t)g >= T.n1) break;
+                if (row < T.n1) a[g] = gload4(P.sa, T.a0 + row);
+            }
+            have = ca;
+        }
+        float Sx = 0.f, Sy = 0.f, Sz = 0.f;
+        float limit2 = P.cutoff2;
+        if (approx) {
+#pragma unroll
+            for (int d = 0; d < 3; ++d) {
+                if (!((T.wrap >> d) & 1u)) continue;
+                const float sgn = ((T.wrap_b >> d) & 1u) ? 1.0f : -1.0f;
+                Sx += sgn * P.box.m[3 * d];
+                Sy += sgn * P.box.m[3 * d + 1];
+                Sz += sgn * P.box.m[3 * d + 2];
+            }
+            limit2 = P.prune_limit2;
+        }
+        uint16_t *list = live_row + t * (uint64_t)LIVE_ROW_STRIDE;
+        unsigned long long mine = 0ull;
+        uint32_t nlive = 0u;
+        float ra2 = 0.0f;
+        bool fin = true;
+#pragma unroll
+        for (int g = 0; g < LIVE_GROUPS; ++g) {
+            const uint32_t row = 64u * (uint32_t)g + lane;
+            if (64u * (uint32_t)g >= T.n1) break;
+            const float ax = a[g].x - Sx, ay = a[g].y - Sy, az = a[g].z - Sz;
+            const bool need = row < T.n1 && !(aabb_d2(ax, ay, az, lo.x, lo.y, lo.z, hi.x, hi.y, hi.z) > limit2);
+            const unsigned long long m = __builtin_amdgcn_ballot_w64(need);
+            if (lane == (uint32_t)g) mine = m;
+            if (need) {
+                list[nlive + __builtin_amdgcn_mbcnt_hi((uint32_t)(m >> 32), __builtin_amdgcn_mbcnt_lo((uint32_t)m, 0u))] = (uint16_t)row;
+                const float r0 = ax - org.x, r1 = ay - org.y, r2 = az - org.z;
+                const float v = (r0 * r0 + r1 * r1) + r2 * r2;
+                fin = fin && v == v;
+                ra2 = fmaxf(ra2, v);
+            }
+            nlive += (uint32_t)__popcll(m);
+        }
+        for (int off = 32; off > 0; off >>= 1) ra2 = fmaxf(ra2, __shfl_xor(ra2, off, 64));
+        if (__builtin_amdgcn_ballot_w64(!fin) != 0ull) ra2 = __builtin_nanf("");
+        if (lane < (uint32_t)LIVE_GROUPS) masks[t * (uint64_t)LIVE_GROUPS + lane] = mine;
+        if (lane == 0) {
+            live_cnt[t] = nlive;
+            live_bound[t] = ra2;
+        }
+    }
 }
 
 template <int KIND>
@@ -655,7 +698,7 @@
         d.a0 = T.a0; d.n1 = T.n1; d.b0 = T.b0; d.n2 = T.n2; d.cb = T.cb;
         d.flags = T.wrap | (T.tri ? 0x100u : 0u) | (T.valid ? 0x200u : 0u) | (lc != LIVE_NONE ? SLOT_LIVE : 0u) | (T.wrap_b << 12) | (T.rps << 16);
         d.pad0 = nb;
-        d.pad1 = 0u;
+        d.pad1 = lc != LIVE_NONE ? lc : 0u;
         task_desc[t] = d;
     }
     uint32_t tot_nb, tot_rows;
@@ -696,7 +739,8 @@
                                                                 SlotDesc *__restrict__ slot_desc, uint64_t nslots_bound,
                                                                 SearchSizes *__restrict__ sizes_host,
                                                                 const unsigned long long *__restrict__ group_tot,
-                                                                const unsigned long long *__restrict__ live_masks,
+                                                                const uint16_t *__restrict__ live_row,
+                                                                const float *__restrict__ live_bound,
                                                                 unsigned long long *__restrict__ slot_stat) {
     __shared__ unsigned long long part[3][4];
     const uint32_t tile = blockIdx.x / (256u / PLAN_SUB), sub = blockIdx.x % (256u / PLAN_SUB);
@@ -789,11 +833,13 @@
         const TaskDesc d = ldesc[lo];
         const uint32_t q = sl - lfirst[lo], rps = d.flags >> 16, nch = (d.n2 + 63u) >> 6;
         uint4 w;
-        if (part3 == 0u) w = make_uint4(d.a0, d.n1, d.b0, d.n2);
-        else if (part3 == 1u) w = make_uint4(d.cb, d.flags, q * rps, 0u);
+        const bool live = (d.flags & SLOT_LIVE) != 0u;
+        const uint64_t t = (uint64_t)tile * 256u + sub * PLAN_SUB + lo;
+        if (part3 == 0u) w = make_uint4(d.a0, live ? d.pad1 : d.n1, d.b0, d.n2);
+        else if (part3 == 1u) w = make_uint4(d.cb, d.flags, q * rps, live ? __float_as_uint(live_bound[t]) : 0u);
         else {
             const unsigned long long mo = task_moff ? lm0[lo] + (unsigned long long)q * 2u * nch : lm0[lo];
-            const unsigned long long mp = (d.flags & SLOT_LIVE) ? (unsigned long long)(live_masks + (((uint64_t)tile * 256u + sub * PLAN_SUB + lo) * (uint64_t)LIVE_GROUPS)) : 0ull;
+            const unsigned long long mp = live ? (unsigned long long)(live_row + t * (uint64_t)LIVE_ROW_STRIDE) : 0ull;
             w = make_uint4((uint32_t)mo, (uint32_t)(mo >> 32), (uint32_t)mp, (uint32_t)(mp >> 32));
         }
         out[i] = w;
@@ -1599,10 +1645,13 @@
     MH_TRY(cur.set[0].live.reserve(live_rows_bytes(cur)));
     unsigned long long *masks = cur.set[0].live.as<unsigned long long>();
     uint32_t *cnt = reinterpret_cast<uint32_t *>(masks + live_rows_mask_words(cur));
+    MH_TRY(cur.set[0].live_list.reserve(live_row_list_bytes(cur)));
+    uint16_t *rows = cur.set[0].live_list.as<uint16_t>();
+    float *bound = reinterpret_cast<float *>(rows + live_row_list_words(cur));
     const SearchParams P = make_params(c, cur);
-    const dim3 grid = pair_grid((unsigned)cur.ntasks);
-    if (cur.kind == MOLAR_HIP_SEARCH_SINGLE) hipLaunchKernelGGL((live_rows_kernel<MOLAR_HIP_SEARCH_SINGLE>), grid, dim3(64), 0, lane.stream, P, masks, cnt);
-    else hipLaunchKernelGGL((live_rows_kernel<MOLAR_HIP_SEARCH_DOUBLE>), grid, dim3(64), 0, lane.stream, P, masks, cnt);
+    const dim3 grid = pair_grid((unsigned)(grid_cells(cur) * LIVE_SHARES));
+    if (cur.kind == MOLAR_HIP_SEARCH_SINGLE) hipLaunchKernelGGL((live_rows_kernel<MOLAR_HIP_SEARCH_SINGLE>), grid, dim3(64), 0, lane.stream, P, masks, cnt, rows, bound);
+    else hipLaunchKernelGGL((live_rows_kernel<MOLAR_HIP_SEARCH_DOUBLE>), grid, dim3(64), 0, lane.stream, P, masks, cnt, rows, bound);
     MH_HIP(hipGetLastError());
     return 0;
 }
@@ -1638,6 +1687,8 @@
         uint32_t *lfirst = c->task_mu.as<uint32_t>();
         const unsigned long long *live_masks = use_live ? cur.set[0].live.as<unsigned long long>() : nullptr;
         const uint32_t *live_cnt = use_live ? reinterpret_cast<const uint32_t *>(live_masks + live_rows_mask_words(cur)) : nullptr;
+        const uint16_t *live_row = use_live ? cur.set[0].live_list.as<uint16_t>() : nullptr;
+        const float *live_bound = use_live ? reinterpret_cast<const float *>(live_row + live_row_list_words(cur)) : nullptr;
         if (cur.kind == MOLAR_HIP_SEARCH_SINGLE)
             hipLaunchKernelGGL((plan_tiles_kernel<MOLAR_HIP_SEARCH_SINGLE>), dim3(ntiles), dim3(256), 0, c->stream, P, lfirst,
                                c->task_desc.as<TaskDesc>(), lmoff, fast_kind, c->slot_cnt.as<uint32_t>(), cur.nslots_bound + 1, tt, params_dst, live_cnt);
@@ -1648,7 +1699,7 @@
         if (ngroups) hipLaunchKernelGGL(plan_groups_kernel, dim3(ngroups), dim3(64), 0, c->stream, ntiles, tt, gt);
         hipLaunchKernelGGL(plan_slots_kernel, dim3(ntiles * (256u / PLAN_SUB)), dim3(256), 0, c->stream, cur.ntasks, ntiles, lfirst, lmoff, c->task_nb.as<uint32_t>(),
                            c->task_desc.as<TaskDesc>(), moff, tt, c->slot_desc.as<SlotDesc>(), cur.nslots_bound, call.sizes_dev, gt,
-                           live_masks, c->slot_stat.as<unsigned long long>());
+                           live_row, live_bound, c->slot_stat.as<unsigned long long>());
         MH_HIP(hipGetLastError());
         c->slot_stat_valid = true;
         c->plan_live = use_live;
@@ -1779,6 +1830,28 @@
     MH_TRY(read_back(c, st, c->slot_stat.p, sizeof st));
     *slots = st[0];
     *consecutive_slots = st[1];
+    return MOLAR_HIP_OK;
+}
+
+int molar_hip_search_live_rows(molar_hip_ctx *c, uint64_t entries_cap, uint64_t *entries, uint64_t *masks, uint32_t *counts, uint16_t *rows,
+                               float *bounds) {
+    if (!c || !entries) return fail(MOLAR_HIP_ERR_INVALID_ARGUMENT, "search_live_rows: null argument");
+    if (!c->slot_stat_valid || !c->plan_live || !c->cur.set)
+        return fail(MOLAR_HIP_ERR_NO_SEARCH, "search_live_rows: the slots of the context's last search were not cut from live rows");
+    const SearchShape &cur = c->cur;
+    const size_t ne = (size_t)plan_entries(cur);
+    *entries = ne;
+    if (!masks && !counts && !rows && !bounds) return MOLAR_HIP_OK;
+    if (entries_cap < ne) return fail(MOLAR_HIP_ERR_INVALID_ARGUMENT, "search_live_rows: room for %llu entries, the plan has %llu",
+                                      (unsigned long long)entries_cap, (unsigned long long)ne);
+    MH_HIP(hipSetDevice(c->device));
+    MH_HIP(hipDeviceSynchronize());
+    const unsigned long long *dm = cur.set[0].live.as<unsigned long long>();
+    const uint16_t *dr = cur.set[0].live_list.as<uint16_t>();
+    if (masks) MH_HIP(hipMemcpy(masks, dm, ne * LIVE_ROW_GROUPS * 8u, hipMemcpyDeviceToHost));
+    if (counts) MH_HIP(hipMemcpy(counts, dm + live_rows_mask_words(cur), ne * 4u, hipMemcpyDeviceToHost));
+    if (rows) MH_HIP(hipMemcpy(rows, dr, live_row_list_words(cur) * 2u, hipMemcpyDeviceToHost));
+    if (bounds) MH_HIP(hipMemcpy(bounds, dr + live_row_list_words(cur), ne * 4u, hipMemcpyDeviceToHost));
     return MOLAR_HIP_OK;
 }
 
diff --git a/molar_amd/csrc/search_shape.hpp b/molar_amd/csrc/search_shape.hpp
--- a/molar_amd/csrc/search_shape.hpp
+++ b/molar_amd/csrc/search_shape.hpp
@@ -85,6 +85,9 @@
 }
 inline size_t live_rows_mask_words(const SearchShape &s) { return (size_t)plan_entries(s) * LIVE_ROW_GROUPS; }
 inline size_t live_rows_bytes(const SearchShape &s) { return live_rows_mask_words(s) * 8u + (size_t)plan_entries(s) * 4u; }
+constexpr uint32_t LIVE_ROW_STRIDE = LIVE_ROW_GROUPS * 64u;
+inline size_t live_row_list_words(const SearchShape &s) { return (size_t)plan_entries(s) * LIVE_ROW_STRIDE; }
+inline size_t live_row_list_bytes(const SearchShape &s) { return live_row_list_words(s) * 2u + (size_t)plan_entries(s) * 4u; }
 
 inline uint64_t held_fingerprint(const float *xyz, size_t natoms) {
     uint64_t fp = 0xcbf29ce484222325ull;
diff --git a/rust/molar_hip/src/ffi.rs b/rust/molar_hip/src/ffi.rs
--- a/rust/molar_hip/src/ffi.rs
+++ b/rust/molar_hip/src/ffi.rs
@@ -42,6 +42,7 @@
     pub search_grid_dims: unsafe extern "C" fn(*mut MolarHipCtx, *mut u64) -> c_int,
     pub search_cell_kernels: unsafe extern "C" fn(*mut MolarHipCtx, *mut i32, *mut u64) -> c_int,
     pub search_slot_counts: unsafe extern "C" fn(*mut MolarHipCtx, *mut u64, *mut u64) -> c_int,
+    pub search_live_rows: unsafe extern "C" fn(*mut MolarHipCtx, u64, *mut u64, *mut u64, *mut u32, *mut u16, *mut f32) -> c_int,
     pub search_fill_device: unsafe extern "C" fn(*mut MolarHipCtx, *mut *const u32, *mut *const f32) -> c_int,
     pub search_resident: unsafe extern "C" fn(*mut MolarHipCtx, *const MolarHipSearchDesc, *mut u64, *mut *const u32, *mut *const f32) -> c_int,
     pub search_resident_planes: unsafe extern "C" fn(*mut MolarHipCtx, c_int) -> c_int,
@@ -206,6 +207,7 @@
                 search_grid_dims: *lib.get::<unsafe extern "C" fn(*mut MolarHipCtx, *mut u64) -> c_int>(b"molar_hip_search_grid_dims\0")?,
                 search_cell_kernels: *lib.get::<unsafe extern "C" fn(*mut MolarHipCtx, *mut i32, *mut u64) -> c_int>(b"molar_hip_search_cell_kernels\0")?,
                 search_slot_counts: *lib.get::<unsafe extern "C" fn(*mut MolarHipCtx, *mut u64, *mut u64) -> c_int>(b"molar_hip_search_slot_counts\0")?,
+                search_live_rows: *lib.get::<unsafe extern "C" fn(*mut MolarHipCtx, u64, *mut u64, *mut u64, *mut u32, *mut u16, *mut f32) -> c_int>(b"molar_hip_search_live_rows\0")?,
                 search_fill_device: *lib.get::<unsafe extern "C" fn(*mut MolarHipCtx, *mut *const u32, *mut *const f32) -> c_int>(b"molar_hip_search_fill_device\0")?,
                 search_resident: *lib.get::<unsafe extern "C" fn(*mut MolarHipCtx, *const MolarHipSearchDesc, *mut u64, *mut *const u32, *mut *const f32) -> c_int>(b"molar_hip_search_resident\0")?,
                 search_resident_planes: *lib.get::<unsafe extern "C" fn(*mut MolarHipCtx, c_int) -> c_int>(b"molar_hip_search_resident_planes\0")?,
@@ -336,4 +338,4 @@
     }
 }
 
-pub const ENTRY_POINTS: usize = 158;
+pub const ENTRY_POINTS: usize = 159;
```

Result: no change. 760.8 frames/s, median of 3 (-0.3%).
